# Deam0on/deepEMIA

Hardware: AMD Instinct MI355X
Metric: EM tiles/s (2048x2048, R101-FPN) (higher is better)
Workload: dtype f16x2

## Files before the change

deepemia_amd/_lib.py:

```python
from __future__ import annotations

import ctypes as C
import os
from pathlib import Path

_HERE = Path(__file__).resolve().parent
LIB_PATH = _HERE / "csrc" / ("libdeepemia_hip_dev.so" if os.environ.get("DEEPEMIA_DEV_LIB", "0") == "1" else "libdeepemia_hip.so")

F32, BF16, F32X3, BF16X2, F16X2, P32 = 0, 1, 2, 3, 4, 5
ACT_NONE, ACT_RELU, ACT_SIGMOID = 0, 1, 2
RES_NONE, RES_SAME, RES_UP2 = 0, 1, 2
MOP = {"fill": 1, "dilate": 2, "erode": 3, "drop_multi": 4, "flag_multi": 5, "gate": 6}


class HipExtensionMissing(RuntimeError):
    pass


class HipKernelError(RuntimeError):
    pass


class ConvDesc(C.Structure):
    _fields_ = [
        ("in_", C.c_void_p), ("w", C.c_void_p), ("scale", C.c_void_p), ("bias", C.c_void_p),
        ("residual", C.c_void_p), ("out", C.c_void_p),
        ("N", C.c_int32), ("H", C.c_int32), ("W", C.c_int32), ("Cin", C.c_int32),
        ("Ho", C.c_int32), ("Wo", C.c_int32), ("Cout", C.c_int32), ("CoutPad", C.c_int32),
        ("KH", C.c_int32), ("KW", C.c_int32), ("stride", C.c_int32), ("pad", C.c_int32),
        ("dtype", C.c_int32), ("out_dtype", C.c_int32), ("act", C.c_int32), ("res_mode", C.c_int32),
        ("out_ld", C.c_int32), ("tile_hint", C.c_int32),
        ("amax_in", C.c_void_p), ("amax_out", C.c_void_p),
    ]


class ConvP32Desc(C.Structure):
    _fields_ = [
        ("in_", C.c_void_p), ("in_meta", C.c_void_p), ("w", C.c_void_p), ("scale", C.c_void_p), ("bias", C.c_void_p),
        ("residual", C.c_void_p), ("res_meta", C.c_void_p), ("out", C.c_void_p), ("out_meta", C.c_void_p),
        ("wbound", C.c_float), ("bbound", C.c_float),
        ("N", C.c_int32), ("H", C.c_int32), ("W", C.c_int32), ("Cin", C.c_int32),
        ("Ho", C.c_int32), ("Wo", C.c_int32), ("Cout", C.c_int32), ("CoutPad", C.c_int32),
        ("KH", C.c_int32), ("KW", C.c_int32), ("stride", C.c_int32), ("pad", C.c_int32),
        ("act", C.c_int32), ("res_mode", C.c_int32), ("out_f32", C.c_int32), ("out_ld", C.c_int32), ("tile_hint", C.c_int32),
        ("head_w", C.c_void_p), ("head_b", C.c_void_p), ("head_out", C.c_void_p),
        ("head_n", C.c_int32), ("head_ld", C.c_int32), ("head_act", C.c_int32),
        ("groups", C.c_int32), ("group_rows", C.c_int32), ("row0", C.c_int32), ("single", C.c_int32),
    ]


class RpnDesc(C.Structure):
    _fields_ = [
        ("head", C.c_void_p * 5), ("H", C.c_int32 * 5), ("W", C.c_int32 * 5), ("stride", C.c_int32 * 5),
        ("cell_anchors", C.c_void_p), ("head_ld", C.c_int32), ("N", C.c_int32),
        ("img_h", C.c_int32), ("img_w", C.c_int32), ("pre_topk", C.c_int32), ("post_topk", C.c_int32),
        ("nms_thresh", C.c_float), ("out_boxes", C.c_void_p), ("out_scores", C.c_void_p),
        ("out_count", C.c_void_p), ("workspace", C.c_void_p),
    ]


class RoiAlignDesc(C.Structure):
    _fields_ = [
        ("feat", C.c_void_p * 4), ("H", C.c_int32 * 4), ("W", C.c_int32 * 4),
        ("N", C.c_int32), ("R", C.c_int32), ("C", C.c_int32), ("P", C.c_int32), ("dtype", C.c_int32),
        ("boxes", C.c_void_p), ("count", C.c_void_p), ("out", C.c_void_p),
        ("meta", C.c_void_p * 4), ("out_meta", C.c_void_p), ("groups", C.c_int32), ("single", C.c_int32),
        ("order", C.c_void_p),
    ]


class DetsDesc(C.Structure):
    _fields_ = [
        ("logits", C.c_void_p), ("ld", C.c_int32), ("props", C.c_void_p), ("prop_count", C.c_void_p),
        ("N", C.c_int32), ("R", C.c_int32), ("K", C.c_int32), ("img_h", C.c_int32), ("img_w", C.c_int32),
        ("score_thresh", C.c_float), ("nms_thresh", C.c_float), ("topk", C.c_int32),
        ("det_boxes", C.c_void_p), ("det_scores", C.c_void_p), ("det_classes", C.c_void_p),
        ("det_count", C.c_void_p),
    ]


class PasteDesc(C.Structure):
    _fields_ = [
        ("mask_prob", C.c_void_p), ("ld", C.c_int32), ("det_boxes", C.c_void_p), ("det_classes", C.c_void_p),
        ("det_count", C.c_void_p), ("N", C.c_int32), ("D", C.c_int32), ("img_h", C.c_int32), ("img_w", C.c_int32),
        ("out_h", C.c_int32), ("out_w", C.c_int32), ("out_boxes", C.c_void_p), ("valid", C.c_void_p),
        ("packed", C.c_void_p), ("out_bbox", C.c_void_p), ("prev_bbox", C.c_void_p),
    ]


EXPORTS = {
    "demia_abi_version": (C.c_int, []),
    "demia_conv_f16x2_kstep": (C.c_int, []),
    "demia_last_error": (C.c_char_p, []),
    "demia_build_arch": (C.c_char_p, []),
    "demia_build_flavor": (C.c_char_p, []),
    "demia_stream_create_cu_mask": (C.c_int, [C.c_void_p, C.c_int, C.c_void_p]),
    "demia_stream_destroy": (C.c_int, [C.c_void_p]),
    "demia_conv2d_nhwc": (C.c_int, [C.POINTER(ConvDesc), C.c_void_p]),
    "demia_conv2d_p32": (C.c_int, [C.POINTER(ConvP32Desc), C.c_void_p]),
    "demia_conv2d_p32_single": (C.c_int, [C.POINTER(ConvP32Desc), C.c_void_p]),
    "demia_resize_h_u8": (C.c_int, [C.c_void_p, C.c_void_p, C.c_int, C.c_int, C.c_int, C.c_int, C.c_void_p,
                                     C.c_void_p, C.c_void_p, C.c_int, C.c_void_p]),
    "demia_resize_v_norm": (C.c_int, [C.c_void_p, C.c_void_p, C.c_int, C.c_int, C.c_int, C.c_int, C.c_int, C.c_int,
                                       C.c_void_p, C.c_void_p, C.c_void_p, C.c_int, C.POINTER(C.c_float), C.c_int,
                                       C.c_void_p]),
    "demia_resize_linear_u8": (C.c_int, [C.c_void_p, C.c_void_p, C.c_int, C.c_int, C.c_int, C.c_int, C.c_int, C.c_void_p,
                                          C.c_void_p, C.c_void_p, C.c_void_p, C.c_void_p]),
    "demia_stem_conv": (C.c_int, [C.c_void_p, C.c_void_p, C.c_void_p, C.c_void_p, C.c_void_p, C.c_int, C.c_int,
                                   C.c_int, C.c_int, C.c_void_p]),
    "demia_stem_conv_mfma": (C.c_int, [C.c_void_p, C.c_void_p, C.c_void_p, C.c_void_p, C.c_void_p, C.c_int, C.c_int, C.c_int, C.c_float,
                                        C.c_void_p]),
    "demia_stem_pool_mfma": (C.c_int, [C.c_void_p, C.c_void_p, C.c_void_p, C.c_void_p, C.c_void_p, C.c_void_p, C.c_int, C.c_int, C.c_int,
                                        C.c_float, C.c_float, C.c_int, C.c_int, C.c_void_p]),
    "demia_maxpool3x3s2": (C.c_int, [C.c_void_p, C.c_void_p, C.c_int, C.c_int, C.c_int, C.c_int, C.c_int, C.c_void_p]),
    "demia_maxpool3x3s2_p32": (C.c_int, [C.c_void_p, C.c_void_p, C.c_void_p, C.c_float, C.c_int, C.c_int, C.c_int, C.c_int, C.c_int, C.c_int,
                                          C.c_void_p]),
    "demia_subsample2": (C.c_int, [C.c_void_p, C.c_void_p, C.c_int, C.c_int, C.c_int, C.c_int, C.c_int, C.c_void_p]),
    "demia_rpn_workspace_bytes": (C.c_int64, [C.c_int]),
    "demia_rpn_proposals": (C.c_int, [C.POINTER(RpnDesc), C.c_void_p]),
    "demia_roi_align": (C.c_int, [C.POINTER(RoiAlignDesc), C.c_void_p]),
    "demia_roi_order": (C.c_int, [C.c_void_p, C.c_void_p, C.c_int, C.c_int, C.c_void_p, C.c_void_p]),
    "demia_box_detections": (C.c_int, [C.POINTER(DetsDesc), C.c_void_p]),
    "demia_paste_masks": (C.c_int, [C.POINTER(PasteDesc), C.c_void_p]),
    "demia_unpack_masks": (C.c_int, [C.c_void_p, C.c_void_p, C.c_int64, C.c_int, C.c_int, C.c_void_p]),
    "demia_mask_area_bbox": (C.c_int, [C.c_void_p, C.c_void_p, C.c_void_p, C.c_void_p, C.c_int64, C.c_int, C.c_int, C.c_void_p]),
    "demia_mask_program": (C.c_int, [C.c_void_p, C.c_void_p, C.c_void_p, C.c_void_p, C.c_uint32, C.c_int64, C.c_int, C.c_int,
                                      C.c_void_p, C.c_void_p, C.c_void_p, C.c_void_p]),
    "demia_mask_program_wl": (C.c_int, [C.c_void_p, C.c_void_p, C.c_void_p, C.c_void_p, C.c_uint32, C.c_int64, C.c_int, C.c_int,
                                         C.c_void_p, C.c_void_p, C.c_void_p, C.c_void_p, C.c_void_p]),
    "demia_mask_overlap_prefix": (C.c_int, [C.c_void_p, C.c_void_p, C.c_void_p, C.c_int64, C.c_int, C.c_int, C.c_void_p]),
    "demia_mask_column_counts": (C.c_int, [C.c_void_p, C.c_void_p, C.c_void_p, C.c_int64, C.c_int, C.c_int, C.c_void_p, C.c_void_p]),
    "demia_mask_pair_intersections": (C.c_int, [C.c_void_p, C.c_void_p, C.c_void_p, C.c_void_p, C.c_void_p, C.c_void_p,
                                                 C.c_void_p, C.c_int64, C.c_int, C.c_int, C.c_void_p]),
    "demia_mask_pair_matrix": (C.c_int, [C.c_void_p, C.c_void_p, C.c_void_p, C.c_void_p, C.c_void_p, C.c_void_p, C.c_int64, C.c_int,
                                          C.c_int, C.c_int, C.c_void_p]),
    "demia_host_greedy_keep": (C.c_int, [C.c_void_p, C.c_int, C.c_void_p, C.c_void_p, C.c_void_p, C.c_void_p, C.c_int, C.c_double,
                                          C.c_void_p]),
    "demia_host_dedup_smart": (C.c_int, [C.c_void_p, C.c_int, C.c_void_p, C.c_void_p, C.c_void_p, C.c_void_p, C.c_void_p, C.c_void_p,
                                          C.c_void_p, C.c_int, C.c_double, C.c_void_p, C.c_void_p]),
    "demia_host_repr_rows": (C.c_int64, [C.c_void_p, C.c_int64, C.c_int, C.c_void_p, C.c_int64]),
    "demia_host_rle_text": (C.c_int64, [C.c_void_p, C.c_void_p, C.c_void_p, C.c_int64, C.c_int, C.c_void_p, C.c_int64, C.c_void_p]),
    "demia_mask_place_tiles": (C.c_int, [C.c_void_p, C.c_void_p, C.c_void_p, C.c_void_p, C.c_int64, C.c_int, C.c_int,
                                          C.c_int, C.c_int, C.c_int, C.c_int, C.c_void_p]),
    "demia_mask_crop_pack": (C.c_int, [C.c_void_p, C.c_void_p, C.c_void_p, C.c_int64, C.c_int, C.c_int, C.c_void_p, C.c_void_p]),
    "demia_mask_gather_regions": (C.c_int, [C.c_void_p, C.c_void_p, C.c_void_p, C.c_int64, C.c_int, C.c_int, C.c_void_p, C.c_void_p]),
    "demia_mask_gather_regions_pooled": (C.c_int, [C.c_void_p, C.c_void_p, C.c_void_p, C.c_int64, C.c_int, C.c_int, C.c_void_p, C.c_void_p,
                                                    C.c_int, C.c_void_p]),
    "demia_mask_crop_unpack": (C.c_int, [C.c_void_p, C.c_void_p, C.c_void_p, C.c_int64, C.c_int, C.c_int, C.c_void_p, C.c_void_p]),
    "demia_crop_place_tiles": (C.c_int, [C.c_void_p, C.c_void_p, C.c_void_p, C.c_int64, C.c_int, C.c_int, C.c_int, C.c_int, C.c_int, C.c_int,
                                          C.c_void_p, C.c_void_p, C.c_void_p, C.c_void_p, C.c_void_p, C.c_void_p]),
    "demia_crop_gather": (C.c_int, [C.c_void_p, C.c_void_p, C.c_void_p, C.c_void_p, C.c_void_p, C.c_int64, C.c_void_p, C.c_void_p]),
    "demia_crop_reroom": (C.c_int, [C.c_void_p, C.c_void_p, C.c_void_p, C.c_void_p, C.c_void_p, C.c_void_p, C.c_int64, C.c_int64, C.c_void_p,
                                     C.c_void_p]),
    "demia_crop_pair_matrix": (C.c_int, [C.c_void_p, C.c_void_p, C.c_void_p, C.c_void_p, C.c_void_p, C.c_void_p, C.c_void_p, C.c_void_p,
                                          C.c_int64, C.c_int, C.c_void_p]),
    "demia_crop_pair_intersections": (C.c_int, [C.c_void_p, C.c_void_p, C.c_void_p, C.c_void_p, C.c_void_p, C.c_void_p, C.c_void_p, C.c_void_p,
                                                 C.c_void_p, C.c_void_p, C.c_void_p, C.c_int64, C.c_void_p]),
    "demia_crop_unpack_pooled": (C.c_int, [C.c_void_p, C.c_void_p, C.c_void_p, C.c_void_p, C.c_int64, C.c_int64, C.c_int, C.c_int,
                                            C.c_void_p, C.c_void_p, C.c_int, C.c_void_p]),
    "demia_crop_gray_histogram": (C.c_int, [C.c_void_p, C.c_void_p, C.c_void_p, C.c_void_p, C.c_void_p, C.c_int, C.c_int64, C.c_int, C.c_int,
                                             C.c_void_p, C.c_void_p]),
    "demia_mask_gray_histogram": (C.c_int, [C.c_void_p, C.c_void_p, C.c_void_p, C.c_int, C.c_int64, C.c_int, C.c_int, C.c_void_p, C.c_void_p]),
    "demia_contour_work_ints": (C.c_int64, [C.c_int, C.c_int, C.c_int]),
    "demia_contour_work_floats": (C.c_int64, [C.c_int, C.c_int, C.c_int]),
    "demia_contour_work_doubles": (C.c_int64, [C.c_int, C.c_int, C.c_int]),
    "demia_mask_contours": (C.c_int, [C.c_void_p, C.c_void_p, C.c_void_p, C.c_int, C.c_int, C.c_int, C.c_int, C.c_int,
                                       C.c_void_p, C.c_void_p, C.c_void_p, C.c_void_p, C.c_void_p, C.c_void_p]),
    "demia_mask_contours_wl": (C.c_int, [C.c_void_p, C.c_void_p, C.c_void_p, C.c_int, C.c_int, C.c_int, C.c_int, C.c_int,
                                          C.c_void_p, C.c_void_p, C.c_void_p, C.c_void_p, C.c_void_p, C.c_void_p, C.c_void_p]),
    "demia_crop_contour_scratch": (C.c_int64, [C.c_void_p, C.c_int64, C.c_int, C.c_int, C.c_void_p]),
    "demia_crop_contours_wl": (C.c_int, [C.c_void_p, C.c_void_p, C.c_void_p, C.c_void_p, C.c_int, C.c_int, C.c_int, C.c_int, C.c_int,
                                          C.c_void_p, C.c_void_p, C.c_void_p, C.c_void_p, C.c_void_p, C.c_void_p, C.c_void_p, C.c_void_p,
                                          C.c_void_p]),
    "demia_contour_measure": (C.c_int, [C.c_void_p, C.c_void_p, C.c_void_p, C.c_void_p, C.c_void_p, C.c_int, C.c_int, C.c_int,
                                         C.c_void_p, C.c_void_p, C.c_void_p, C.c_double, C.c_void_p, C.c_int, C.c_void_p]),
    "demia_contour_shape_work_ints": (C.c_int64, [C.c_int, C.c_int, C.c_int]),
    "demia_contour_shape": (C.c_int, [C.c_void_p, C.c_void_p, C.c_void_p, C.c_void_p, C.c_void_p, C.c_int, C.c_int, C.c_int,
                                       C.c_void_p, C.c_double, C.c_void_p, C.c_int, C.c_void_p]),
    "demia_mask_inscribed": (C.c_int, [C.c_void_p, C.c_void_p, C.c_void_p, C.c_void_p, C.c_void_p, C.c_void_p, C.c_int, C.c_int, C.c_int,
                                        C.c_int, C.c_double, C.c_void_p, C.c_int, C.c_void_p]),
    "demia_crop_inscribed": (C.c_int, [C.c_void_p, C.c_void_p, C.c_void_p, C.c_void_p, C.c_void_p, C.c_void_p, C.c_void_p, C.c_int, C.c_int,
                                        C.c_int, C.c_int, C.c_double, C.c_void_p, C.c_int, C.c_void_p, C.c_void_p, C.c_void_p]),
    "demia_mask_skeleton": (C.c_int, [C.c_void_p, C.c_void_p, C.c_void_p, C.c_void_p, C.c_void_p, C.c_void_p, C.c_int, C.c_int, C.c_int,
                                       C.c_int, C.c_double, C.c_void_p, C.c_int, C.c_void_p, C.c_void_p, C.c_void_p]),
    "demia_crop_skeleton_scratch": (C.c_int64, [C.c_void_p, C.c_int64, C.c_int, C.c_int, C.c_void_p]),
    "demia_crop_skeleton": (C.c_int, [C.c_void_p, C.c_void_p, C.c_void_p, C.c_void_p, C.c_void_p, C.c_void_p, C.c_void_p, C.c_int, C.c_int,
                                       C.c_int, C.c_int, C.c_double, C.c_void_p, C.c_int, C.c_void_p, C.c_void_p, C.c_void_p, C.c_void_p,
                                       C.c_void_p, C.c_void_p]),
    "demia_mask_neighbours": (C.c_int, [C.c_void_p, C.c_void_p, C.c_void_p, C.c_int64, C.c_int, C.c_int, C.c_int64, C.c_void_p, C.c_void_p,
                                         C.c_void_p, C.c_void_p, C.c_void_p, C.c_void_p]),
    "demia_crop_neighbours": (C.c_int, [C.c_void_p, C.c_void_p, C.c_void_p, C.c_void_p, C.c_void_p, C.c_int64, C.c_int, C.c_int, C.c_int64,
                                         C.c_void_p, C.c_void_p, C.c_void_p, C.c_void_p, C.c_void_p, C.c_void_p]),
    "demia_poly_rasterize": (C.c_int, [C.c_void_p, C.c_void_p, C.c_void_p, C.c_void_p, C.c_void_p, C.c_void_p, C.c_void_p, C.c_void_p,
                                        C.c_int64, C.c_void_p, C.c_int64, C.c_int, C.c_int, C.c_void_p, C.c_void_p, C.c_void_p,
                                        C.c_void_p]),
    "demia_mask_cross_matrix": (C.c_int, [C.c_void_p, C.c_void_p, C.c_void_p, C.c_void_p, C.c_void_p, C.c_void_p, C.c_void_p, C.c_void_p,
                                           C.c_void_p, C.c_int64, C.c_int, C.c_int, C.c_int, C.c_void_p]),
    "demia_mask_rle_colmajor": (C.c_int, [C.c_void_p, C.c_void_p, C.c_void_p, C.c_void_p, C.c_void_p, C.c_int64, C.c_int, C.c_int,
                                           C.c_void_p]),
    "demia_crop_poly_rasterize": (C.c_int, [C.c_void_p, C.c_void_p, C.c_void_p, C.c_void_p, C.c_void_p, C.c_void_p, C.c_void_p, C.c_void_p,
                                             C.c_int64, C.c_void_p, C.c_int64, C.c_int, C.c_int, C.c_void_p, C.c_void_p, C.c_int64,
                                             C.c_void_p, C.c_void_p, C.c_void_p, C.c_void_p]),
    "demia_crop_cross_matrix": (C.c_int, [C.c_void_p, C.c_void_p, C.c_void_p, C.c_void_p, C.c_void_p, C.c_void_p, C.c_void_p, C.c_void_p,
                                           C.c_void_p, C.c_void_p, C.c_void_p, C.c_void_p, C.c_void_p, C.c_int64, C.c_int, C.c_void_p]),
    "demia_crop_rle_colmajor": (C.c_int, [C.c_void_p, C.c_void_p, C.c_void_p, C.c_void_p, C.c_void_p, C.c_void_p, C.c_void_p, C.c_int64,
                                           C.c_int, C.c_int, C.c_void_p]),
    "demia_host_coco_match": (C.c_int, [C.c_int64, C.c_void_p, C.c_void_p, C.c_void_p, C.c_void_p, C.c_void_p, C.c_void_p, C.c_void_p,
                                         C.c_void_p, C.c_void_p, C.c_void_p, C.c_int, C.c_void_p, C.c_int, C.c_int, C.c_void_p,
                                         C.c_void_p, C.c_void_p, C.c_void_p]),
    "demia_host_rle_string": (C.c_int64, [C.c_void_p, C.c_void_p, C.c_int64, C.c_void_p, C.c_int64, C.c_void_p]),
}

_lib = None


def load() -> C.CDLL:
    global _lib
    if _lib is not None:
        return _lib
    if not LIB_PATH.exists():
        raise HipExtensionMissing(
            f"{LIB_PATH} not found: build it with `python -c 'import __graft_entry__ as g; g.build()'` "
            f"(or `make -C {LIB_PATH.parent}`); there is no CPU fallback for the hot path."
        )
    try:
        lib = C.CDLL(str(LIB_PATH), mode=getattr(os, "RTLD_NOW", 2))
    except OSError as e:
        raise HipExtensionMissing(f"cannot load {LIB_PATH}: {e}") from e
    for name, (res, args) in EXPORTS.items():
        try:
            fn = getattr(lib, name)
        except AttributeError as e:
            raise HipExtensionMissing(f"{LIB_PATH} does not export {name}") from e
        fn.restype = res
        fn.argtypes = args
    _lib = lib
    return lib


def is_dev_build() -> bool:
    return load().demia_build_flavor() == b"dev"


def check(status: int, what: str) -> None:
    if status != 0:
        msg = load().demia_last_error().decode(errors="replace")
        raise HipKernelError(f"{what} failed with status {status}: {msg}")


def ptr(t) -> int:
    return 0 if t is None else int(t.data_ptr())


def cu_masked_stream(device, spec: str):
    import numpy as np
    import torch

    kind, m, k = spec.split(":")
    assert kind == "mod"
    m, k = int(m), int(k)
    bits = np.zeros(256, dtype=np.uint8)
    bits[(np.arange(256) % m) < k] = 1
    words = np.packbits(bits.reshape(8, 32), axis=1, bitorder="little").view(np.uint32).reshape(8).copy()
    handle = C.c_void_p()
    with torch.cuda.device(device):
        check(load().demia_stream_create_cu_mask(words.ctypes.data, 8, C.byref(handle)), "demia_stream_create_cu_mask")
    return torch.cuda.ExternalStream(handle.value, device=device), int(bits.sum())
```

deepemia_amd/csrc/conv_p32.hip:

```cpp
#include <utility>
#include "common.h"
#ifndef P32_ABLATE
#define P32_ABLATE 0
#endif

#ifndef P32_HEAD_DIRECT
#define P32_HEAD_DIRECT 1
#endif
#ifndef P32_SINGLE
#define P32_SINGLE 0
#endif
#ifndef P32_DEV_TILES
#define P32_DEV_TILES 0
#endif
#ifndef P32_ST_AUX
#define P32_ST_AUX 0
#endif
#ifndef P32_RES_AUX
#define P32_RES_AUX 0
#endif
#ifndef P32_A_NT
#define P32_A_NT 0
#endif
#ifndef P32_FRAG_PIPE
#define P32_FRAG_PIPE 0
#endif

namespace {

struct ConvQ {
    const void* in;
    const float* in_meta;
    const void* w;
    const float* scale;
    const float* bias;
    const void* res;
    const float* res_meta;
    void* out;
    float* out_meta;
    float wbound, bbound;
    int N, H, W, Cin, Ho, Wo, Cout, CoutPad, KH, KW, stride, pad;
    int act, res_mode, out_f32, out_ld;
    int M, HoWo, ntn, nwg, ksteps, taps;
    int kloop;
    unsigned in_bytes, w_bytes;
    unsigned out_bytes, res_bytes;
    const float* head_w;
    const float* head_b;
    float* head_out;
    int head_n, head_ld, head_act;
    int groups, group_rows, row0;
    int no_hk;
    int zero_low;
    int stagger_ticks;
    int resident;
};

typedef __attribute__((address_space(3))) void lds_void;

template <int OFF, int WAIT>
__device__ __forceinline__ void ds_read2_b128(f16x8& a, f16x8& b, unsigned addr_a, unsigned addr_b) {
    if constexpr (WAIT >= 0)
        asm volatile("ds_read_b128 %0, %2 offset:%4\n\tds_read_b128 %1, %3 offset:%4\n\ts_waitcnt lgkmcnt(%5)"
                     : "=&v"(a), "=&v"(b) : "v"(addr_a), "v"(addr_b), "n"(OFF), "n"(WAIT) : "memory");
    else
        asm volatile("ds_read_b128 %0, %2 offset:%4\n\tds_read_b128 %1, %3 offset:%4"
                     : "=&v"(a), "=&v"(b) : "v"(addr_a), "v"(addr_b), "n"(OFF) : "memory");
}

template <int... Is, class F>
__device__ __forceinline__ void static_for_impl(std::integer_sequence<int, Is...>, F&& f) { (f(std::integral_constant<int, Is>{}), ...); }
template <int N, class F>
__device__ __forceinline__ void static_for(F&& f) { static_for_impl(std::make_integer_sequence<int, N>{}, static_cast<F&&>(f)); }
typedef int i32x4 __attribute__((ext_vector_type(4)));

__device__ __forceinline__ void dma16(const i32x4 rsrc, unsigned lds_addr, unsigned voff, unsigned soff) {
    unsigned keep;
    asm volatile("s_mov_b32 %0, m0\n\ts_mov_b32 m0, %1\n\ts_nop 0\n\tbuffer_load_dwordx4 %2, %3, %4 offen lds\n\ts_mov_b32 m0, %0"
                 : "=&s"(keep) : "s"(lds_addr), "v"(voff), "s"(rsrc), "s"(soff) : "memory");
}
__device__ __forceinline__ void dma16_nt(const i32x4 rsrc, unsigned lds_addr, unsigned voff, unsigned soff) {
    unsigned keep;
    asm volatile("s_mov_b32 %0, m0\n\ts_mov_b32 m0, %1\n\ts_nop 0\n\tbuffer_load_dwordx4 %2, %3, %4 offen nt lds\n\ts_mov_b32 m0, %0"
                 : "=&s"(keep) : "s"(lds_addr), "v"(voff), "s"(rsrc), "s"(soff) : "memory");
}
__device__ __forceinline__ i32x4 make_rsrc(const void* base, unsigned bytes) {
    const unsigned long long a = reinterpret_cast<unsigned long long>(base);
    i32x4 r;
    r[0] = __builtin_amdgcn_readfirstlane((int)(unsigned)a);
    r[1] = __builtin_amdgcn_readfirstlane((int)((unsigned)(a >> 32) & 0xffffu));
    r[2] = __builtin_amdgcn_readfirstlane((int)bytes);
    r[3] = 0x00020000;
    return r;
}

__device__ __forceinline__ float apply_act_q(float v, int act) {
    if (act == DEMIA_ACT_RELU) return v > 0.f ? v : 0.f;
    if (act == DEMIA_ACT_SIGMOID) return 1.0f / (1.0f + expf(-v));
    return v;
}

__device__ __forceinline__ float plane_scale(float bound) {
    if (!(bound > 0.f) || !(bound < 3.0e38f)) return 1.f;
    int e = 14 - ilogbf(bound);
    e = e < -100 ? -100 : (e > 100 ? 100 : e);
    return ldexpf(1.f, e);
}

template <int TN, int EF>
__device__ __forceinline__ void write_acc32(const f32x16 (&row)[TN], float* e, int lane) {
#pragma unroll
    for (int j = 0; j < TN; ++j)
#pragma unroll
        for (int r = 0; r < 16; ++r)
            e[((r & 3) + 8 * (r >> 2) + 4 * (lane >> 5)) * EF + j * 32 + (lane & 31)] = row[j][r];
}
template <int TN, int EF>
__device__ __forceinline__ void write_acc16(const f32x4 (&r0)[2 * TN], const f32x4 (&r1)[2 * TN], float* e, int lane) {
#pragma unroll
    for (int j = 0; j < 2 * TN; ++j)
#pragma unroll
        for (int r = 0; r < 4; ++r) {
            e[(4 * (lane >> 4) + r) * EF + j * 16 + (lane & 15)] = r0[j][r];
            e[(16 + 4 * (lane >> 4) + r) * EF + j * 16 + (lane & 15)] = r1[j][r];
        }
}

__device__ __forceinline__ float uniform(float v) { return __int_as_float(__builtin_amdgcn_readfirstlane(__float_as_int(v))); }

struct GroupScales {
    int g0, b1, b2;
    float post0, post1, post2, resi0, resi1, resi2, sout0, sout1, sout2;
};

__device__ __forceinline__ void load_group_scale(const ConvQ& p, int gi, bool planes_out, float& post, float& resi, float& sout) {
    gi = min(gi, p.groups - 1);
    const float amax_in = p.in_meta[2 * gi], s_in = p.in_meta[2 * gi + 1];
    float amax_res = 0.f, s_res = 1.f;
    if (p.res_mode != DEMIA_RES_NONE) { amax_res = p.res_meta[2 * gi]; s_res = p.res_meta[2 * gi + 1]; }
    post = uniform(1.0f / s_in);
    resi = uniform(p.res_mode != DEMIA_RES_NONE ? 1.0f / s_res : 0.f);
    sout = uniform(planes_out ? plane_scale(amax_in * p.wbound + p.bbound + amax_res) : 1.f);
}

__device__ __forceinline__ GroupScales load_group_scales(const ConvQ& p, int m0, bool planes_out) {
    GroupScales gs;
    gs.g0 = (m0 + p.row0) / p.group_rows;
    gs.b1 = (gs.g0 + 1) * p.group_rows - p.row0;
    gs.b2 = gs.b1 + p.group_rows;
    load_group_scale(p, gs.g0, planes_out, gs.post0, gs.resi0, gs.sout0);
    load_group_scale(p, gs.g0 + 1, planes_out, gs.post1, gs.resi1, gs.sout1);
    load_group_scale(p, gs.g0 + 2, planes_out, gs.post2, gs.resi2, gs.sout2);
    return gs;
}

template <int WM, int WN, int TM, int TN, bool HEAD, typename WriteRow>
__device__ __forceinline__ void p32_epilogue(const ConvQ& p, const GroupScales& gs, char* smem, WriteRow&& write_tile_row, int wm, int wn, int m0, int n0) {
    constexpr int BN = WN * TN * 32;
    const int tid = threadIdx.x, lane = tid & 63;
    constexpr int EROW = BN * 4 + 16;
    constexpr int GPR = BN / 8, RSTEP = 512 / GPR, ITEMS = WM * 32 / RSTEP;
    static_assert(512 % GPR == 0 && (WM * 32) % RSTEP == 0, "epilogue split");
    constexpr int BM_ = WM * TM * 32;
    static_assert(!HEAD || BN == 256, "the fused head needs a 256-wide tile");
    const bool planes_out = !HEAD && !p.out_f32;
    const int g0 = __builtin_amdgcn_readfirstlane(gs.g0), b1 = __builtin_amdgcn_readfirstlane(gs.b1), b2 = __builtin_amdgcn_readfirstlane(gs.b2);
    const float post0 = uniform(gs.post0), post1 = uniform(gs.post1), post2 = uniform(gs.post2);
    const float resi0 = uniform(gs.resi0), resi1 = uniform(gs.resi1), resi2 = uniform(gs.resi2);
    const float sout0 = uniform(gs.sout0), sout1 = uniform(gs.sout1), sout2 = uniform(gs.sout2);
    if (planes_out && n0 == 0 && tid == 0) {
#pragma unroll
        for (int d = 0; d < 3; ++d) {
            const int first = d == 0 ? g0 * p.group_rows - p.row0 : (d == 1 ? b1 : b2);
            if (g0 + d < p.groups && first >= m0 && first < m0 + BM_ && first < p.M)
                p.out_meta[2 * (g0 + d) + 1] = d == 0 ? sout0 : (d == 1 ? sout1 : sout2);
        }
    }
    const int g = tid % GPR, r_first = tid / GPR;
    const int co = n0 + g * 8;
    float sc[8], bs[8];
#pragma unroll
    for (int q = 0; q < 8; ++q) {
        const bool ok = (co + q) < p.Cout;
        sc[q] = (p.scale && ok) ? p.scale[co + q] : 1.0f;
        bs[q] = (p.bias && ok) ? p.bias[co + q] : 0.0f;
    }
    float vmax3[3] = {0.f, 0.f, 0.f};
    constexpr int HMAX = 4;
    float hw[HMAX][8];
    constexpr bool head_on = HEAD;
    if (head_on) {
#pragma unroll
        for (int j = 0; j < HMAX; ++j)
#pragma unroll
            for (int q = 0; q < 8; ++q) hw[j][q] = j < p.head_n ? p.head_w[j * 256 + g * 8 + q] : 0.f;
    }
    const int tile_n_ = n0 / BN;
    const bool res_on = p.res_mode != DEMIA_RES_NONE, sigmoid_on = p.act == DEMIA_ACT_SIGMOID;
    const float act_lo = p.act == DEMIA_ACT_RELU ? 0.f : -INFINITY;
    const char* resb = reinterpret_cast<const char*>(p.res) + 128;
    char* outb = reinterpret_cast<char*>(p.out) + 128;
    const long cbytes = (long)p.Cout * 4;
    const int gofs = (co >> 5) * 128 + ((co & 31) >> 3) * 16;
    auto row_of = [&](int i, int k) { const int lr = r_first + k * RSTEP; return m0 + (lr >> 5) * (TM * 32) + i * 32 + (lr & 31); };
    auto res_pix = [&](int m) -> long {
        if (p.res_mode == DEMIA_RES_SAME) return m;
        const int n = m / p.HoWo;
        const int rem = m - n * p.HoWo;
        const int ho = rem / p.Wo, wo = rem - ho * p.Wo;
        const int Hr = (p.Ho + 1) >> 1, Wr = (p.Wo + 1) >> 1;
        return ((long)n * Hr + (ho >> 1)) * Wr + (wo >> 1);
    };
    f16x8 rh[ITEMS], rl[ITEMS];
    const bool has_res = p.res_mode != DEMIA_RES_NONE && co < p.Cout;
    auto load_res = [&](int i) {
#pragma unroll
        for (int k = 0; k < ITEMS; ++k) {
            const int m = row_of(i, k);
            if (has_res && m < p.M && !(P32_ABLATE & 32)) {
                const char* rp = resb + res_pix(m) * cbytes + gofs;
                rh[k] = *reinterpret_cast<const f16x8*>(rp);
                rl[k] = *reinterpret_cast<const f16x8*>(rp + 64);
            }
        }
    };
    load_res(0);
#pragma unroll
    for (int i = 0; i < TM; ++i) {
        if (i > 0) __syncthreads();
        write_tile_row(i, reinterpret_cast<float*>(smem) + (wm * 32) * (EROW / 4) + wn * TN * 32);
        __syncthreads();
        f16x8 ch[ITEMS], cl[ITEMS];
#pragma unroll
        for (int k = 0; k < ITEMS; ++k) { ch[k] = rh[k]; cl[k] = rl[k]; }
        if (i + 1 < TM) load_res(i + 1);
        if (co < p.Cout) {
#pragma unroll
            for (int k = 0; k < ITEMS; ++k) {
                const int lr = r_first + k * RSTEP;
                const int m = row_of(i, k);
                if (m >= p.M) continue;
                const float4 x0 = *reinterpret_cast<const float4*>(smem + lr * EROW + g * 32);
                const float4 x1 = *reinterpret_cast<const float4*>(smem + lr * EROW + g * 32 + 16);
                float v[8] = {x0.x, x0.y, x0.z, x0.w, x1.x, x1.y, x1.z, x1.w};
                const int gd = (m >= b1) + (m >= b2);
                const float post = gd == 0 ? post0 : (gd == 1 ? post1 : post2);
#pragma unroll
                for (int q = 0; q < 8; ++q) v[q] = (v[q] * post) * sc[q] + bs[q];
                if (res_on) {
                    const float res_inv = gd == 0 ? resi0 : (gd == 1 ? resi1 : resi2);
#pragma unroll
                    for (int q = 0; q < 8; ++q) v[q] += ((float)ch[k][q] + (float)cl[k][q]) * res_inv;
                }
#pragma unroll
                for (int q = 0; q < 8; ++q) v[q] = fmaxf(v[q], act_lo);
                if (sigmoid_on) {
#pragma unroll
                    for (int q = 0; q < 8; ++q) v[q] = 1.0f / (1.0f + expf(-v[q]));
                }
                if (head_on) {
                    float acc_h[HMAX];
#pragma unroll
                    for (int j = 0; j < HMAX; ++j) {
                        float a = 0.f;
#pragma unroll
                        for (int q = 0; q < 8; ++q) a = fmaf(v[q], hw[j][q], a);
#pragma unroll
                        for (int o = 16; o > 0; o >>= 1) a += __shfl_xor(a, o, 32);
                        acc_h[j] = a;
                    }
                    if (g == 0) {
                        float* o = p.head_out + ((long)m * p.ntn + tile_n_) * p.head_ld;
#pragma unroll
                        for (int j = 0; j < HMAX; ++j)
                            if (j < p.head_n) {
                                const float z = acc_h[j] + p.head_b[j];
                                o[j] = p.head_act == DEMIA_ACT_SIGMOID ? 1.0f / (1.0f + expf(-z)) : (p.head_act == DEMIA_ACT_RELU ? fmaxf(z, 0.f) : z);
                            }
                    }
                } else if (p.out_f32) {
                    float* o = reinterpret_cast<float*>(p.out) + (long)m * p.out_ld + co;
                    if (co + 8 <= p.Cout && (p.out_ld & 3) == 0) {
                        *reinterpret_cast<float4*>(o) = make_float4(v[0], v[1], v[2], v[3]);
                        *reinterpret_cast<float4*>(o + 4) = make_float4(v[4], v[5], v[6], v[7]);
                    } else {
#pragma unroll
                        for (int q = 0; q < 8; ++q)
                            if (co + q < p.Cout) o[q] = v[q];
                    }
                } else {
                    f16x8 h, l;
                    const float s_out = gd == 0 ? sout0 : (gd == 1 ? sout1 : sout2);
                    float vm = 0.f;
#pragma unroll
                    for (int q = 0; q < 8; ++q) {
                        vm = fmaxf(vm, fabsf(v[q]));
                        const float y = v[q] * s_out;
                        h[q] = (_Float16)y;
                        l[q] = (P32_SINGLE && p.zero_low) ? (_Float16)0.f : (_Float16)(y - (float)h[q]);
                    }
                    vmax3[0] = fmaxf(vmax3[0], gd == 0 ? vm : 0.f);
                    vmax3[1] = fmaxf(vmax3[1], gd == 1 ? vm : 0.f);
                    vmax3[2] = fmaxf(vmax3[2], gd == 2 ? vm : 0.f);
                    char* o = outb + (long)m * cbytes + gofs;
                    if (P32_ABLATE & 64) {
                        asm volatile("" :: "v"(h), "v"(l), "v"(o));
                    } else {
                        *reinterpret_cast<f16x8*>(o) = h;
                        *reinterpret_cast<f16x8*>(o + 64) = l;
                    }
                }
            }
        }
    }
    if (planes_out) {
#pragma unroll
        for (int d = 0; d < 3; ++d) {
            if (d > 0 && (d == 1 ? b1 : b2) >= m0 + BM_) break;
            if (g0 + d >= p.groups) break;
            float vmax = vmax3[d];
#pragma unroll
            for (int o = 32; o > 0; o >>= 1) vmax = fmaxf(vmax, __shfl_xor(vmax, o));
            float* slot = p.out_meta + 2 * (g0 + d);
            if (lane == 0 && vmax > *reinterpret_cast<volatile const float*>(slot))
                atomicMax(reinterpret_cast<unsigned int*>(slot), __float_as_uint(vmax));
        }
    }
}

struct NoHook { __device__ __forceinline__ void operator()() const {} };
template <int WM, int WN, int TM, int TN, typename WriteRow, typename Hook = NoHook>
__device__ __forceinline__ void p32_epilogue_planes(const ConvQ& p, const GroupScales& gs, char* smem, WriteRow&& write_tile_row, int wm, int wn,
                                                    int m0, int n0, bool leader = (threadIdx.x == 0), Hook&& hook = NoHook()) {
    constexpr int BM_ = WM * TM * 32;
    const int tid = threadIdx.x, lane = tid & 63;
    constexpr int LDW = TN * 32 + 4;
    constexpr int PPW = 8 / TN, RPI = 2 * PPW, ITEMS = 32 / RPI;
    static_assert(TN == 1 || TN == 2 || TN == 4, "TN");
    char* const wsm = smem + (tid >> 6) * (32 * LDW * 4);
    const int g0 = __builtin_amdgcn_readfirstlane(gs.g0), b1 = __builtin_amdgcn_readfirstlane(gs.b1), b2 = __builtin_amdgcn_readfirstlane(gs.b2);
    const float post0 = uniform(gs.post0), post1 = uniform(gs.post1), post2 = uniform(gs.post2);
    const float resi0 = uniform(gs.resi0), resi1 = uniform(gs.resi1), resi2 = uniform(gs.resi2);
    const float sout0 = uniform(gs.sout0), sout1 = uniform(gs.sout1), sout2 = uniform(gs.sout2);
    if (n0 == 0 && leader) {
#pragma unroll
        for (int d = 0; d < 3; ++d) {
            const int first = d == 0 ? g0 * p.group_rows - p.row0 : (d == 1 ? b1 : b2);
            if (g0 + d < p.groups && first >= m0 && first < m0 + BM_ && first < p.M)
                p.out_meta[2 * (g0 + d) + 1] = d == 0 ? sout0 : (d == 1 ? sout1 : sout2);
        }
    }
    const int cj = lane & 3, rs = (lane >> 2) & 1, lg = lane >> 3;
    const int line = lg % TN;
    const int r_first = (lg / TN) * 2 + rs;
    const int co = n0 + ((wn * TN + line) * 4 + cj) * 8;
    float sc[8], bs[8];
#pragma unroll
    for (int q = 0; q < 8; ++q) {
        sc[q] = p.scale ? p.scale[co + q] : 1.0f;
        bs[q] = p.bias ? p.bias[co + q] : 0.0f;
    }
    const bool sigmoid_on = p.act == DEMIA_ACT_SIGMOID;
    const float act_lo = p.act == DEMIA_ACT_RELU ? 0.f : -INFINITY;
    const bool res_on = p.res_mode != DEMIA_RES_NONE;
    const bool single = P32_SINGLE != 0 && p.zero_low != 0;
    const __amdgpu_buffer_rsrc_t rs_out = __builtin_amdgcn_make_buffer_rsrc(p.out, 0, (int)p.out_bytes, 0x00020000);
    const __amdgpu_buffer_rsrc_t rs_res = __builtin_amdgcn_make_buffer_rsrc(const_cast<void*>(res_on ? p.res : p.out), 0, res_on ? (int)p.res_bytes : 0, 0x00020000);
    const unsigned cbytes = (unsigned)p.Cout * 4u;
    const unsigned lofs = 128u + (unsigned)((co >> 5) * 128 + (lane & 7) * 16);
    auto row_of = [&](int i, int k) { return m0 + wm * (TM * 32) + i * 32 + r_first + k * RPI; };
    auto res_off = [&](int m) -> unsigned {
        if (p.res_mode != DEMIA_RES_UP2 || (P32_ABLATE & 256)) return (unsigned)m * cbytes + lofs;
        const int n = m / p.HoWo;
        const int rem = m - n * p.HoWo;
        const int ho = rem / p.Wo, wo = rem - ho * p.Wo;
        const int Hr = (p.Ho + 1) >> 1, Wr = (p.Wo + 1) >> 1;
        return (unsigned)((n * Hr + (ho >> 1)) * Wr + (wo >> 1)) * cbytes + lofs;
    };
    auto from_below = [&](u32x4 own, u32x4 theirs) -> u32x4 {
        u32x4 r;
#pragma unroll
        for (int c = 0; c < 4; ++c) r[c] = (unsigned)__builtin_amdgcn_update_dpp((int)own[c], (int)theirs[c], 0x114, 0xf, 0xa, false);
        return r;
    };
    auto from_above = [&](u32x4 own, u32x4 theirs) -> u32x4 {
        u32x4 r;
#pragma unroll
        for (int c = 0; c < 4; ++c) r[c] = (unsigned)__builtin_amdgcn_update_dpp((int)own[c], (int)theirs[c], 0x104, 0xf, 0x5, false);
        return r;
    };
    u32x4 rh[ITEMS], rl[ITEMS];
    auto load_res = [&](int i) {
#pragma unroll
        for (int k = 0; k < ITEMS; ++k) {
            const int mp = row_of(i, k) - rs;
            if (P32_ABLATE & 32) { rh[k] = u32x4{0, 0, 0, 0}; rl[k] = rh[k]; continue; }
            rh[k] = __builtin_amdgcn_raw_buffer_load_b128(rs_res, res_off(mp), 0, P32_RES_AUX);
            rl[k] = __builtin_amdgcn_raw_buffer_load_b128(rs_res, res_off(mp + 1), 0, P32_RES_AUX);
        }
    };
    float vmax0 = 0.f, vmax1 = 0.f, vmax2 = 0.f;
    if (P32_ABLATE & 512) return;
    load_res(0);
#pragma unroll
    for (int i = 0; i < TM; ++i) {
        asm volatile("" ::: "memory");
        __builtin_amdgcn_wave_barrier();
        write_tile_row(i, reinterpret_cast<float*>(wsm));
        asm volatile("" ::: "memory");
        __builtin_amdgcn_wave_barrier();
        f16x8 ch[ITEMS], cl[ITEMS];
#pragma unroll
        for (int k = 0; k < ITEMS; ++k) {
            ch[k] = __builtin_bit_cast(f16x8, from_below(rh[k], rl[k]));
            cl[k] = __builtin_bit_cast(f16x8, from_above(rl[k], rh[k]));
        }
        if (i + 1 < TM) load_res(i + 1);
#pragma unroll
        for (int k = 0; k < ITEMS; ++k) {
            const int lr = r_first + k * RPI;
            const int m = row_of(i, k);
            const float4 x0 = *reinterpret_cast<const float4*>(wsm + lr * (LDW * 4) + (line * 4 + cj) * 32);
            const float4 x1 = *reinterpret_cast<const float4*>(wsm + lr * (LDW * 4) + (line * 4 + cj) * 32 + 16);
            typedef float f32x2 __attribute__((ext_vector_type(2)));
            f32x2 v2[4] = {{x0.x, x0.y}, {x0.z, x0.w}, {x1.x, x1.y}, {x1.z, x1.w}};
            const int gd = (m >= b1) + (m >= b2);
            const float post = gd == 0 ? post0 : (gd == 1 ? post1 : post2);
            const float res_inv = gd == 0 ? resi0 : (gd == 1 ? resi1 : resi2);
            const float s_out = gd == 0 ? sout0 : (gd == 1 ? sout1 : sout2);
            float v[8];
#pragma unroll
            for (int q = 0; q < 4; ++q) {
                const f32x2 scq = {sc[2 * q], sc[2 * q + 1]}, bsq = {bs[2 * q], bs[2 * q + 1]};
                const f32x2 t = (v2[q] * post) * scq + bsq;
                v[2 * q] = t.x;
                v[2 * q + 1] = t.y;
            }
#pragma unroll
            for (int q = 0; q < 8; ++q) {
                v[q] = fmaf((float)cl[k][q], res_inv, fmaf((float)ch[k][q], res_inv, v[q]));
                v[q] = fmaxf(v[q], act_lo);
            }
            if (sigmoid_on && !(P32_ABLATE & 256)) {
#pragma unroll
                for (int q = 0; q < 8; ++q) v[q] = 1.0f / (1.0f + expf(-v[q]));
            }
            f16x8 h, l;
            float vm = 0.f;
#pragma unroll
            for (int q = 0; q < 8; q += 2) {
                vm = fmaxf(vm, fmaxf(fabsf(v[q]), fabsf(v[q + 1])));
                const f32x2 y = f32x2{v[q], v[q + 1]} * s_out;
                h[q] = (_Float16)y.x;
                h[q + 1] = (_Float16)y.y;
                l[q] = (_Float16)fmaf(-(float)h[q], 1.0f, y.x);
                l[q + 1] = (_Float16)fmaf(-(float)h[q + 1], 1.0f, y.y);
            }
            if (single) l = f16x8{0, 0, 0, 0, 0, 0, 0, 0};
            vm = m < p.M ? vm : 0.f;
            vmax0 = fmaxf(vmax0, gd == 0 ? vm : 0.f);
            vmax1 = fmaxf(vmax1, gd == 1 ? vm : 0.f);
            vmax2 = fmaxf(vmax2, gd == 2 ? vm : 0.f);
            const u32x4 hu = __builtin_bit_cast(u32x4, h), lu = __builtin_bit_cast(u32x4, l);
            const u32x4 d0 = from_below(hu, lu);
            const u32x4 d1 = from_above(lu, hu);
            const unsigned off = (unsigned)(m - rs) * cbytes + lofs;
            if (P32_ABLATE & 64) {
                asm volatile("" :: "v"(d0), "v"(d1), "v"(off));
            } else {
                __builtin_amdgcn_raw_buffer_store_b128(d0, rs_out, off, 0, P32_ST_AUX);
                __builtin_amdgcn_raw_buffer_store_b128(d1, rs_out, off + cbytes, 0, P32_ST_AUX);
            }
            hook();
        }
    }
#pragma unroll
    for (int d = 0; d < 3; ++d) {
        if (d > 0 && (d == 1 ? b1 : b2) >= m0 + BM_) break;
        if (g0 + d >= p.groups) break;
        float vmax = d == 0 ? vmax0 : (d == 1 ? vmax1 : vmax2);
#pragma unroll
        for (int o = 32; o > 0; o >>= 1) vmax = fmaxf(vmax, __shfl_xor(vmax, o));
        float* slot = p.out_meta + 2 * (g0 + d);
        if (lane == 0 && vmax > *reinterpret_cast<volatile const float*>(slot))
            atomicMax(reinterpret_cast<unsigned int*>(slot), __float_as_uint(vmax));
    }
}

template <int WM, int WN, int TM, int TN, int HN>
__device__ __forceinline__ void p32_epilogue_head_direct(const ConvQ& p, const GroupScales& gs, char* smem, const f32x4 (&acc16)[2 * TM][2 * TN],
                                                         int wm, int wn, int m0, int n0) {
    constexpr int BM = WM * TM * 32, BN = WN * TN * 32;
    static_assert(BN == 256, "the fused head needs a 256-wide tile");
    const int tid = threadIdx.x, lane = tid & 63, c16 = lane & 15, rq = lane >> 4;
    const int b1 = __builtin_amdgcn_readfirstlane(gs.b1), b2 = __builtin_amdgcn_readfirstlane(gs.b2);
    const float post0 = uniform(gs.post0), post1 = uniform(gs.post1), post2 = uniform(gs.post2);
    float sc[2 * TN], bs[2 * TN], hw[HN][2 * TN];
#pragma unroll
    for (int jn = 0; jn < 2 * TN; ++jn) {
        const int cl = wn * TN * 32 + jn * 16 + c16;
        sc[jn] = p.scale ? p.scale[n0 + cl] : 1.0f;
        bs[jn] = p.bias ? p.bias[n0 + cl] : 0.0f;
#pragma unroll
        for (int j = 0; j < HN; ++j) hw[j][jn] = j < p.head_n ? p.head_w[j * 256 + cl] : 0.f;
    }
    const float act_lo = p.act == DEMIA_ACT_RELU ? 0.f : -INFINITY;
    float* part = reinterpret_cast<float*>(smem);
#pragma unroll
    for (int i = 0; i < 2 * TM; ++i) {
#pragma unroll
        for (int r = 0; r < 4; ++r) {
            const int row = wm * TM * 32 + i * 16 + rq * 4 + r;
            const int m = m0 + row;
            const int gd = (m >= b1) + (m >= b2);
            const float post = gd == 0 ? post0 : (gd == 1 ? post1 : post2);
            float a[HN];
#pragma unroll
            for (int j = 0; j < HN; ++j) a[j] = 0.f;
#pragma unroll
            for (int jn = 0; jn < 2 * TN; ++jn) {
                const float v = fmaxf((acc16[i][jn][r] * post) * sc[jn] + bs[jn], act_lo);
#pragma unroll
                for (int j = 0; j < HN; ++j) a[j] = fmaf(v, hw[j][jn], a[j]);
            }
#pragma unroll
            for (int j = 0; j < HN; ++j) {
                a[j] += __int_as_float(__builtin_amdgcn_update_dpp(0, __float_as_int(a[j]), 0x128, 0xf, 0xf, false));
                a[j] += __int_as_float(__builtin_amdgcn_update_dpp(0, __float_as_int(a[j]), 0x124, 0xf, 0xf, false));
                a[j] += __int_as_float(__builtin_amdgcn_update_dpp(0, __float_as_int(a[j]), 0x122, 0xf, 0xf, false));
                a[j] += __int_as_float(__builtin_amdgcn_update_dpp(0, __float_as_int(a[j]), 0x121, 0xf, 0xf, false));
            }
            if (c16 == 0) {
#pragma unroll
                for (int j = 0; j < HN; ++j) part[((long)wn * BM + row) * HN + j] = a[j];
            }
        }
    }
    __syncthreads();
    const int tile_n_ = n0 / BN;
    for (int o = tid; o < BM * HN; o += WM * WN * 64) {
        const int row = o / HN, j = o - row * HN;
        const int m = m0 + row;
        if (m >= p.M || j >= p.head_n) continue;
        float z = 0.f;
#pragma unroll
        for (int w = 0; w < WN; ++w) z += part[((long)w * BM + row) * HN + j];
        z += p.head_b[j];
        p.head_out[((long)m * p.ntn + tile_n_) * p.head_ld + j] =
            p.head_act == DEMIA_ACT_SIGMOID ? 1.0f / (1.0f + expf(-z)) : (p.head_act == DEMIA_ACT_RELU ? fmaxf(z, 0.f) : z);
    }
}


constexpr int EPI_GENERIC = 0, EPI_PLANES = 1, EPI_HEAD = 2;

template <int WM, int WN, int TM, int TN, bool M16 = true, int EPI = EPI_PLANES, int NST = 2, bool HK = false>
__global__ __launch_bounds__(WM * WN * 64, WM * WN == 8 ? 2 : 1) void conv_p32_kernel(const ConvQ p) {
    static_assert(NST == 2 || NST == 3, "two or three LDS stages");
    static_assert(!HK || (P32_SINGLE && M16 && NST == 2), "HK is a variant of the single-plane 16x16x32 kernel");
    static_assert(WM * WN == 8 || (WM * WN == 4 && EPI == EPI_PLANES), "eight waves, or four (planes epilogue only)");
    constexpr int NW = WM * WN;
    constexpr int BM = WM * TM * 32, BN = WN * TN * 32;
    constexpr int STAGE = (BM + BN) * 128;
    constexpr int NIA = BM / 8, NIB = BN / 8;

    extern __shared__ __attribute__((aligned(16))) char smem[];
    const int tid = threadIdx.x, lane = tid & 63;
    const int wave = __builtin_amdgcn_readfirstlane(tid >> 6);
    const int wm = wave / WN, wn = wave % WN;
    const int swz = xcd_remap(blockIdx.x, p.nwg);
    const int tile_n = swz % p.ntn, tile_m = swz / p.ntn;
    const int m0 = tile_m * BM, n0 = tile_n * BN;
#if P32_DEV_TILES
    if (p.stagger_ticks > 0) {
        const int b = blockIdx.x;
        const bool late = p.resident > 256 ? (b >= p.resident / 2 && b < p.resident) : (b < p.resident && ((b >> 3) & 1));
        if (late) {
            const unsigned long long t0 = __builtin_amdgcn_s_memrealtime();
            while (__builtin_amdgcn_s_memrealtime() - t0 < (unsigned long long)p.stagger_ticks) __builtin_amdgcn_s_sleep(32);
        }
    }
#endif

    const i32x4 rsrc_a = make_rsrc(p.in, p.in_bytes), rsrc_b = make_rsrc(p.w, p.w_bytes);
    const unsigned lds0 = (unsigned)(__SIZE_TYPE__)((lds_void*)smem);

    constexpr int QA = (NIA + NW - 1) / NW, QB = NIB / NW;
    constexpr bool A_EVEN = NIA % NW == 0;
    static_assert(NIB % NW == 0, "tile width is a multiple of 64");
    unsigned a_off[QA], a_msk[QA], b_off[QB];
#pragma unroll
    for (int q = 0; q < QA; ++q) {
        const int row = (wave + NW * q) * 8 + (lane >> 3);
        const int csw = (lane & 7) ^ ((row >> 1) & 7);
        const int m = m0 + row;
        const bool vm = m < p.M && row < BM;
        const int mm = vm ? m : 0;
        const int n = mm / p.HoWo;
        const int rem = mm - n * p.HoWo;
        const int ho = rem / p.Wo, wo = rem - ho * p.Wo;
        const int hi0 = ho * p.stride - p.pad, wi0 = wo * p.stride - p.pad;
        const long pix = ((long)n * p.H + hi0) * p.W + wi0;
        a_off[q] = (unsigned)(128 + pix * (long)(p.Cin * 4) + (HK ? (csw >> 2) * 128 + (csw & 3) * 16 : csw * 16));
        unsigned mk = 0;
        for (int t = 0, th = 0, tw = 0; t < p.taps; ++t) {
            if (vm && (unsigned)(hi0 + th) < (unsigned)p.H && (unsigned)(wi0 + tw) < (unsigned)p.W) mk |= 1u << t;
            if (++tw == p.KW) { tw = 0; ++th; }
        }
        a_msk[q] = mk;
    }
#pragma unroll
    for (int q = 0; q < QB; ++q) {
        const int row = (wave + NW * q) * 8 + (lane >> 3);
        const int csw = (lane & 7) ^ ((row >> 1) & 7);
        const int co = n0 + row;
        b_off[q] = (unsigned)(((co >> 6) * p.ksteps) * 8192 + (co & 63) * 128 + (HK ? (csw >> 2) * (p.taps * 8192) + (csw & 3) * 16 : csw * 16));
    }
    int tap = 0, kw = 0, tstep = 0;
    unsigned sdelta = 0, srow = 0, sgrp = 0;
    const bool a_nt = P32_A_NT && p.taps == 1 && p.ntn == 1;
    auto issue = [&](int st, int tp, unsigned sd, unsigned bd) {
        const unsigned sbase = __builtin_amdgcn_readfirstlane(lds0 + st * STAGE + wave * 1024);
        const bool first = bd < 2 * 8192u;
#pragma unroll
        for (int q = 0; q < QA; ++q) {
            if ((P32_ABLATE & 1) && !first) break;
            if (!A_EVEN && q == QA - 1 && wave + NW * q >= NIA) break;
            const bool ok = (a_msk[q] >> tp) & 1u;
            const unsigned vo = ok ? a_off[q] + sd : (a_off[q] & 0x70u);
            if (P32_A_NT && a_nt) dma16_nt(rsrc_a, sbase + q * (NW * 1024), vo, 0u);
            else dma16(rsrc_a, sbase + q * (NW * 1024), vo, 0u);
        }
#pragma unroll
        for (int q = 0; q < QB; ++q) {
            if ((P32_ABLATE & 2) && !first) break;
            dma16(rsrc_b, sbase + BM * 128 + q * (NW * 1024), b_off[q], bd);
        }
    };
    const unsigned pixb = (unsigned)(p.Cin * 4), rowb = (unsigned)(p.W * p.Cin * 4);
#define P32_ADVANCE()                                                                   \
    do {                                                                                \
        ++tstep;                                                                        \
        if (++tap == p.taps) { tap = 0; kw = 0; srow = 0; sgrp += HK ? 256u : 128u; sdelta = sgrp; if (HK) tstep += p.taps; } \
        else if (++kw == p.KW) { kw = 0; srow += rowb; sdelta = srow + sgrp; }          \
        else sdelta += pixb;                                                            \
    } while (0)

    const int fsw = (lane >> 1) & 7, hh = lane >> 5;
    int fa[4], fb[4];
#pragma unroll
    for (int c = 0; c < 4; ++c) {
        const int ch = (((c >> 1) * 4 + (c & 1) * 2 + hh) ^ fsw) * 16;
        fa[c] = (wm * TM * 32 + (lane & 31)) * 128 + ch;
        fb[c] = BM * 128 + (wn * TN * 32 + (lane & 31)) * 128 + ch;
    }

    f32x16 acc[M16 ? 1 : TM][M16 ? 1 : TN];
    f32x4 acc16[M16 ? 2 * TM : 1][M16 ? 2 * TN : 1];
#pragma unroll
    for (int i = 0; i < (M16 ? 1 : TM); ++i)
#pragma unroll
        for (int j = 0; j < (M16 ? 1 : TN); ++j)
#pragma unroll
            for (int r = 0; r < 16; ++r) acc[i][j][r] = 0.f;
#pragma unroll
    for (int i = 0; i < (M16 ? 2 * TM : 1); ++i)
#pragma unroll
        for (int j = 0; j < (M16 ? 2 * TN : 1); ++j)
#pragma unroll
            for (int r = 0; r < 4; ++r) acc16[i][j][r] = 0.f;
    int fa16[2], fb16[2];
#pragma unroll
    for (int pl = 0; pl < 2; ++pl) {
        const int ch = ((pl * 4 + (lane >> 4)) ^ (((lane & 15) >> 1) & 7)) * 16;
        fa16[pl] = (wm * TM * 32 + (lane & 15)) * 128 + ch;
        fb16[pl] = BM * 128 + (wn * TN * 32 + (lane & 15)) * 128 + ch;
    }

    constexpr bool BARRIER_IN_COMPUTE = (P32_FRAG_PIPE == 2) && M16 && NST == 2;
    auto compute1 = [&](int st) {
        const char* sb = smem + st * STAGE;
        if constexpr (M16) {
            f16x8 bh[2 * TN];
#pragma unroll
            for (int j = 0; j < 2 * TN; ++j) bh[j] = *reinterpret_cast<const f16x8*>(sb + fb16[0] + j * 2048);
#pragma unroll
            for (int i = 0; i < 2 * TM; ++i) {
                const f16x8 ah = *reinterpret_cast<const f16x8*>(sb + fa16[0] + i * 2048);
#pragma unroll
                for (int j = 0; j < 2 * TN; ++j) acc16[i][j] = __builtin_amdgcn_mfma_f32_16x16x32_f16(ah, bh[j], acc16[i][j], 0, 0, 0);
            }
        } else {
#pragma unroll
            for (int kk = 0; kk < 2; ++kk) {
                f16x8 bh[TN];
#pragma unroll
                for (int j = 0; j < TN; ++j) bh[j] = *reinterpret_cast<const f16x8*>(sb + fb[kk] + j * 4096);
#pragma unroll
                for (int i = 0; i < TM; ++i) {
                    const f16x8 ah = *reinterpret_cast<const f16x8*>(sb + fa[kk] + i * 4096);
#pragma unroll
                    for (int j = 0; j < TN; ++j) acc[i][j] = __builtin_amdgcn_mfma_f32_32x32x16_f16(ah, bh[j], acc[i][j], 0, 0, 0);
                }
            }
        }
        if (BARRIER_IN_COMPUTE) asm volatile("s_waitcnt vmcnt(0) lgkmcnt(0)\n\ts_barrier" ::: "memory");
    };
    auto compute_hk = [&](int st) {
        const char* sb = smem + st * STAGE;
        f16x8 b0[2 * TN], b1[2 * TN];
#pragma unroll
        for (int j = 0; j < 2 * TN; ++j) {
            b0[j] = *reinterpret_cast<const f16x8*>(sb + fb16[0] + j * 2048);
            b1[j] = *reinterpret_cast<const f16x8*>(sb + fb16[1] + j * 2048);
        }
#pragma unroll
        for (int i = 0; i < 2 * TM; ++i) {
            const f16x8 a0 = *reinterpret_cast<const f16x8*>(sb + fa16[0] + i * 2048);
            const f16x8 a1 = *reinterpret_cast<const f16x8*>(sb + fa16[1] + i * 2048);
#pragma unroll
            for (int j = 0; j < 2 * TN; ++j) {
                f32x4 c = acc16[i][j];
                c = __builtin_amdgcn_mfma_f32_16x16x32_f16(a0, b0[j], c, 0, 0, 0);
                c = __builtin_amdgcn_mfma_f32_16x16x32_f16(a1, b1[j], c, 0, 0, 0);
                acc16[i][j] = c;
            }
        }
    };
    auto compute = [&](int st) {
        if constexpr (HK) { compute_hk(st); return; }
        if constexpr (P32_SINGLE != 0) { compute1(st); return; }
        const char* sb = smem + st * STAGE;
        if constexpr (M16) {
            f16x8 bh[2 * TN], bl[2 * TN];
            f16x8 fake;
#pragma unroll
            for (int q = 0; q < 8; ++q) fake[q] = (_Float16)(float)(lane + q);
#if P32_FRAG_PIPE != 2
#pragma unroll
            for (int j = 0; j < 2 * TN; ++j) {
                bh[j] = (P32_ABLATE & 1024) ? fake : *reinterpret_cast<const f16x8*>(sb + fb16[0] + j * 2048);
                bl[j] = (P32_ABLATE & 1024) ? fake : *reinterpret_cast<const f16x8*>(sb + fb16[1] + j * 2048);
            }
#endif
#if P32_FRAG_PIPE == 2
            const unsigned la0 = (unsigned)(__SIZE_TYPE__)((lds_void*)(smem)) + st * STAGE + fa16[0];
            const unsigned la1 = la0 - fa16[0] + fa16[1];
            const unsigned lb0 = la0 - fa16[0] + fb16[0], lb1 = la0 - fa16[0] + fb16[1];
            f16x8 ahp[2], alp[2];
            ds_read2_b128<0, -1>(ahp[0], alp[0], la0, la1);
            static_for<2 * TN>([&](auto jc) {
                constexpr int j = decltype(jc)::value;
                ds_read2_b128<j * 2048, -1>(bh[j], bl[j], lb0, lb1);
            });
            static_for<2 * TM>([&](auto ic) {
                constexpr int i = decltype(ic)::value;
                const f16x8 ah = ahp[i & 1], al = alp[i & 1];
                if constexpr (i == 0) {
                    ds_read2_b128<2048, -1>(ahp[1], alp[1], la0, la1);
                    static_for<2 * TN>([&](auto jc) {
                        constexpr int j = decltype(jc)::value;
                        asm volatile("s_waitcnt lgkmcnt(%0)" ::"n"(2 * (2 * TN - 1 - j) + 2) : "memory");
                        __builtin_amdgcn_sched_barrier(0);
                        f32x4 c = acc16[0][j];
                        c = __builtin_amdgcn_mfma_f32_16x16x32_f16(ah, bl[j], c, 0, 0, 0);
                        c = __builtin_amdgcn_mfma_f32_16x16x32_f16(al, bh[j], c, 0, 0, 0);
                        c = __builtin_amdgcn_mfma_f32_16x16x32_f16(ah, bh[j], c, 0, 0, 0);
                        acc16[0][j] = c;
                        __builtin_amdgcn_sched_barrier(0);
                    });
                } else {
                    if constexpr (i + 1 < 2 * TM) {
                        ds_read2_b128<(i + 1) * 2048, 2>(ahp[(i + 1) & 1], alp[(i + 1) & 1], la0, la1);
                    } else if constexpr (BARRIER_IN_COMPUTE) {
                        asm volatile("s_waitcnt vmcnt(0) lgkmcnt(0)\n\ts_barrier" ::: "memory");
                    } else {
                        asm volatile("s_waitcnt lgkmcnt(0)" ::: "memory");
                    }
                    __builtin_amdgcn_sched_barrier(0);
#pragma unroll
                    for (int j = 0; j < 2 * TN; ++j) {
                        f32x4 c = acc16[i][j];
                        c = __builtin_amdgcn_mfma_f32_16x16x32_f16(ah, bl[j], c, 0, 0, 0);
                        c = __builtin_amdgcn_mfma_f32_16x16x32_f16(al, bh[j], c, 0, 0, 0);
                        c = __builtin_amdgcn_mfma_f32_16x16x32_f16(ah, bh[j], c, 0, 0, 0);
                        acc16[i][j] = c;
                    }
                    __builtin_amdgcn_sched_barrier(0);
                }
            });
            return;
#elif P32_FRAG_PIPE
            f16x8 ahp[2], alp[2];
            ahp[0] = *reinterpret_cast<const f16x8*>(sb + fa16[0]);
            alp[0] = *reinterpret_cast<const f16x8*>(sb + fa16[1]);
#pragma unroll
            for (int i = 0; i < 2 * TM; ++i) {
                if (i + 1 < 2 * TM) {
                    ahp[(i + 1) & 1] = *reinterpret_cast<const f16x8*>(sb + fa16[0] + (i + 1) * 2048);
                    alp[(i + 1) & 1] = *reinterpret_cast<const f16x8*>(sb + fa16[1] + (i + 1) * 2048);
                }
                const f16x8 ah = ahp[i & 1], al = alp[i & 1];
#pragma unroll
                for (int j = 0; j < 2 * TN; ++j) {
                    f32x4 c = acc16[i][j];
                    c = __builtin_amdgcn_mfma_f32_16x16x32_f16(ah, bl[j], c, 0, 0, 0);
                    c = __builtin_amdgcn_mfma_f32_16x16x32_f16(al, bh[j], c, 0, 0, 0);
                    c = __builtin_amdgcn_mfma_f32_16x16x32_f16(ah, bh[j], c, 0, 0, 0);
                    acc16[i][j] = c;
                }
                if (i + 1 < 2 * TM) __builtin_amdgcn_sched_group_barrier(0x100, 2, 0);
                __builtin_amdgcn_sched_group_barrier(0x008, 6 * TN, 0);
            }
            return;
#else
#pragma unroll
            for (int i = 0; i < 2 * TM; ++i) {
                const f16x8 ah = (P32_ABLATE & 1024) ? fake : *reinterpret_cast<const f16x8*>(sb + fa16[0] + i * 2048);
                const f16x8 al = (P32_ABLATE & 1024) ? fake : *reinterpret_cast<const f16x8*>(sb + fa16[1] + i * 2048);
#pragma unroll
                for (int j = 0; j < 2 * TN; ++j) {
                    f32x4 c = acc16[i][j];
                    if (P32_ABLATE & 4) {
                        asm volatile("" :: "v"(ah), "v"(al), "v"(bh[j]), "v"(bl[j]));
                        continue;
                    }
                    c = __builtin_amdgcn_mfma_f32_16x16x32_f16(ah, bl[j], c, 0, 0, 0);
                    c = __builtin_amdgcn_mfma_f32_16x16x32_f16(al, bh[j], c, 0, 0, 0);
                    c = __builtin_amdgcn_mfma_f32_16x16x32_f16(ah, bh[j], c, 0, 0, 0);
                    acc16[i][j] = c;
                }
            }
            return;
#endif
        }
#pragma unroll
        for (int kk = 0; kk < 2; ++kk) {
            f16x8 bh[TN], bl[TN];
#pragma unroll
            for (int j = 0; j < TN; ++j) {
                bh[j] = *reinterpret_cast<const f16x8*>(sb + fb[kk] + j * 4096);
                bl[j] = *reinterpret_cast<const f16x8*>(sb + fb[2 + kk] + j * 4096);
            }
#pragma unroll
            for (int i = 0; i < TM; ++i) {
                const f16x8 ah = *reinterpret_cast<const f16x8*>(sb + fa[kk] + i * 4096);
                const f16x8 al = *reinterpret_cast<const f16x8*>(sb + fa[2 + kk] + i * 4096);
#pragma unroll
                for (int j = 0; j < TN; ++j) {
                    f32x16 c = acc[i][j];
                    if (P32_ABLATE & 4) {
                        asm volatile("" :: "v"(ah), "v"(al), "v"(bh[j]), "v"(bl[j]));
                        continue;
                    }
                    c = __builtin_amdgcn_mfma_f32_32x32x16_f16(ah, bl[j], c, 0, 0, 0);
                    c = __builtin_amdgcn_mfma_f32_32x32x16_f16(al, bh[j], c, 0, 0, 0);
                    c = __builtin_amdgcn_mfma_f32_32x32x16_f16(ah, bh[j], c, 0, 0, 0);
                    acc[i][j] = c;
                }
            }
        }
    };

    constexpr int N_LAST = QB + QA, N_LAST_SHORT = QB + QA - 1;
    const bool short_wave = !A_EVEN && wave + NW * (QA - 1) >= NIA;
    auto wait_all_but_last_issue = [&]() {
        if (short_wave) asm volatile("s_waitcnt vmcnt(%0)" ::"n"(N_LAST_SHORT) : "memory");
        else asm volatile("s_waitcnt vmcnt(%0)" ::"n"(N_LAST) : "memory");
    };
    issue(0, tap, sdelta, 0u);
    P32_ADVANCE();
    bool two_ahead = false;
    if (NST == 3 && p.kloop > 1 && !(P32_ABLATE & 128)) {
        issue(1, tap, sdelta, (unsigned)tstep * 8192u);
        P32_ADVANCE();
        two_ahead = true;
    }
    constexpr bool HEAD = EPI == EPI_HEAD;
    const GroupScales gs = load_group_scales(p, m0, !HEAD && !p.out_f32);
    if (two_ahead) wait_all_but_last_issue();
    else asm volatile("s_waitcnt vmcnt(0)" ::: "memory");
    __builtin_amdgcn_s_barrier();
    int st = 0;
    for (int t = 0; t < ((P32_ABLATE & 128) ? 1 : p.kloop); ++t) {
        const int st_issue = NST == 2 ? (st ^ 1) : (st == 0 ? 2 : st - 1);
        const bool more = t + NST - 1 < p.kloop;
        if (more) {
            issue(st_issue, tap, sdelta, (unsigned)tstep * 8192u);
            P32_ADVANCE();
        }
        compute(st);
        if (NST == 3 && more) {
            wait_all_but_last_issue();
            asm volatile("s_waitcnt lgkmcnt(0)\n\ts_barrier" ::: "memory");
        } else if (!BARRIER_IN_COMPUTE) {
            asm volatile("s_waitcnt vmcnt(0) lgkmcnt(0)\n\ts_barrier" ::: "memory");
        }
        st = NST == 2 ? (st ^ 1) : (st == 2 ? 0 : st + 1);
    }
#undef P32_ADVANCE

    if constexpr ((P32_ABLATE & 2048) != 0 && M16) {
#pragma unroll
        for (int i = 0; i < 2 * TM; ++i)
#pragma unroll
            for (int j = 0; j < 2 * TN; ++j) asm volatile("" :: "v"(acc16[i][j]));
        return;
    }
    if constexpr (EPI == EPI_PLANES) {
        if constexpr (M16) {
            p32_epilogue_planes<WM, WN, TM, TN>(p, gs, smem, [&](int i, float* e) { write_acc16<TN, TN * 32 + 4>(acc16[2 * i], acc16[2 * i + 1], e, lane); }, wm, wn, m0, n0);
        } else {
            p32_epilogue_planes<WM, WN, TM, TN>(p, gs, smem, [&](int i, float* e) { write_acc32<TN, TN * 32 + 4>(acc[i], e, lane); }, wm, wn, m0, n0);
        }
    } else if constexpr (M16 && HEAD && P32_HEAD_DIRECT) {
        if (p.act != DEMIA_ACT_SIGMOID && p.head_n <= 2)
            p32_epilogue_head_direct<WM, WN, TM, TN, 2>(p, gs, smem, acc16, wm, wn, m0, n0);
        else
            p32_epilogue<WM, WN, TM, TN, HEAD>(p, gs, smem, [&](int i, float* e) { write_acc16<TN, BN + 4>(acc16[2 * i], acc16[2 * i + 1], e, lane); }, wm, wn, m0, n0);
    } else if constexpr (M16) {
        p32_epilogue<WM, WN, TM, TN, HEAD>(p, gs, smem, [&](int i, float* e) { write_acc16<TN, BN + 4>(acc16[2 * i], acc16[2 * i + 1], e, lane); }, wm, wn, m0, n0);
    } else {
        p32_epilogue<WM, WN, TM, TN, HEAD>(p, gs, smem, [&](int i, float* e) { write_acc32<TN, BN + 4>(acc[i], e, lane); }, wm, wn, m0, n0);
    }
}

#if P32_DEV_TILES
#include "conv_p32_dev.inc"
#endif

template <int WM, int WN, int TM, int TN, bool M16 = true, int EPI = EPI_PLANES, int NST = 2, bool HK = false>
int launch_q_(ConvQ p, hipStream_t st) {
    constexpr int BM = WM * TM * 32, BN = WN * TN * 32;
    constexpr int stages = NST * (BM + BN) * 128, image = EPI == EPI_PLANES ? WM * WN * 32 * (TN * 128 + 16) : WM * 32 * (BN * 4 + 16);
    static_assert(stages <= 160 * 1024, "LDS");
    constexpr int smem = stages > image ? stages : image;
    p.ntn = p.CoutPad / BN;
    p.nwg = p.ntn * cdiv(p.M, BM);
    p.resident = 256 * (160 * 1024 / smem >= 2 ? 2 : 1);
    p.kloop = HK ? p.ksteps / 2 : p.ksteps;
    auto k = conv_p32_kernel<WM, WN, TM, TN, M16, EPI, NST, HK>;
    static bool attr_done = false;
    if (!attr_done) {
        (void)hipFuncSetAttribute(reinterpret_cast<const void*>(k), hipFuncAttributeMaxDynamicSharedMemorySize, smem);
        attr_done = true;
    }
    hipLaunchKernelGGL(k, dim3(p.nwg), dim3(WM * WN * 64), smem, st, p);
    DEMIA_CHECK_LAUNCH("conv_p32_kernel");
    return DEMIA_OK;
}
template <int WM, int WN, int TM, int TN, bool M16 = true, int EPI = EPI_PLANES, int NST = 2>
int launch_q(ConvQ p, hipStream_t st) {
#if P32_SINGLE
    if constexpr (M16 && NST == 2) {
        if (p.Cin % 64 == 0 && !p.no_hk) return launch_q_<WM, WN, TM, TN, M16, EPI, NST, true>(p, st);
    }
#endif
    return launch_q_<WM, WN, TM, TN, M16, EPI, NST, false>(p, st);
}

struct TileCfg { int id, bm, bn; };
constexpr TileCfg kTiles[] = {{1, 256, 256}, {2, 128, 256}, {4, 192, 256}, {12, 160, 256}, {13, 224, 256}, {6, 256, 128}, {7, 128, 128}, {9, 256, 64}, {11, 128, 64}};

inline double predict_us(const TileCfg& c, long M, int cout_pad, int ksteps, bool residual) {
    const long tiles = (long)cdiv(M, c.bm) * (cout_pad / c.bn);
    const int smem = 2 * (c.bm + c.bn) * 128;
    const int occ = 160 * 1024 / smem >= 2 ? 2 : 1;
    const double area = (double)c.bm * c.bn / 65536.0;
    const double step = 2.0 * area * (1.0 + 0.2 * (1.0 - area));
    const double edge = 6.0 + 6.0 * area * (residual ? 1.5 : 1.0);
    if (occ == 1) return (double)((tiles + 255) / 256) * (ksteps * step + edge);
    return (double)((tiles + 511) / 512) * (2.0 * ksteps * step + 2.0 * 0.5 * edge);
}

inline int choose_tile(long M, int cout_pad, int ksteps, bool residual, bool need256 = false) {
#if P32_SINGLE
    if (cout_pad % 256 == 0 && (long)cdiv(M, 256) * (cout_pad / 256) >= 512) return 1;
#endif
    int best = 0;
    double best_t = 1e30;
    for (const TileCfg& c : kTiles) {
        if (cout_pad % c.bn || (need256 && c.bn != 256)) continue;
        const double t = predict_us(c, M, cout_pad, ksteps, residual);
        if (t < best_t) { best_t = t; best = c.id; }
    }
    return best;
}

}

#if P32_SINGLE
extern "C" int demia_conv2d_p32_single(const demia_conv_p32_desc* d, void* stream) {
#else
extern "C" int demia_conv2d_p32_single(const demia_conv_p32_desc* d, void* stream);
extern "C" int demia_conv2d_p32(const demia_conv_p32_desc* d, void* stream) {
    if (d && d->single) return demia_conv2d_p32_single(d, stream);
#endif
    DEMIA_REQUIRE(d && d->in && d->in_meta && d->w && (d->out || d->head_n > 0), "null pointer");
    DEMIA_REQUIRE(d->out_f32 || d->out_meta || d->head_n > 0, "P32 output needs out_meta");
    DEMIA_REQUIRE(d->Cin > 0 && d->Cin % 32 == 0, "Cin must be a multiple of 32");
    DEMIA_REQUIRE(d->CoutPad >= d->Cout && d->CoutPad % 64 == 0, "CoutPad must be a multiple of 64");
    DEMIA_REQUIRE(d->out_f32 || d->Cout % 32 == 0, "P32 output needs Cout % 32 == 0");
    DEMIA_REQUIRE(d->KH > 0 && d->KW > 0 && d->KH * d->KW <= 32 && d->stride > 0 && d->pad >= 0, "kernel geometry");
    DEMIA_REQUIRE(d->Ho == (d->H + 2 * d->pad - d->KH) / d->stride + 1, "Ho");
    DEMIA_REQUIRE(d->Wo == (d->W + 2 * d->pad - d->KW) / d->stride + 1, "Wo");
    DEMIA_REQUIRE(d->res_mode == DEMIA_RES_NONE || (d->residual && d->res_meta), "residual pointer");
    DEMIA_REQUIRE((long)d->N * d->Ho * d->Wo < (1L << 31), "M overflow");
    const long in_bytes = 128 + (long)d->N * d->H * d->W * d->Cin * 4;
    DEMIA_REQUIRE(in_bytes < (1L << 32), "input planes must stay below 4 GiB");
    const long w_bytes = (long)d->CoutPad * d->KH * d->KW * d->Cin * 4;
    DEMIA_REQUIRE(w_bytes < (1L << 31), "weight planes must stay below 2 GiB");
    ConvQ p;
    p.in = d->in; p.in_meta = d->in_meta; p.w = d->w; p.scale = d->scale; p.bias = d->bias;
    p.res = d->residual; p.res_meta = d->res_meta; p.out = d->out; p.out_meta = d->out_meta;
    p.wbound = d->wbound; p.bbound = d->bbound;
    p.N = d->N; p.H = d->H; p.W = d->W; p.Cin = d->Cin; p.Ho = d->Ho; p.Wo = d->Wo; p.Cout = d->Cout; p.CoutPad = d->CoutPad;
    p.KH = d->KH; p.KW = d->KW; p.stride = d->stride; p.pad = d->pad;
    p.act = d->act; p.res_mode = d->res_mode; p.out_f32 = d->out_f32;
    p.out_ld = d->out_ld > 0 ? d->out_ld : d->Cout;
    DEMIA_REQUIRE(p.out_ld >= d->Cout, "out_ld");
    p.M = d->N * d->Ho * d->Wo;
    p.HoWo = d->Ho * d->Wo;
    p.taps = d->KH * d->KW;
    p.ksteps = p.taps * (d->Cin / 32);
    p.in_bytes = (unsigned)in_bytes; p.w_bytes = (unsigned)w_bytes;
    p.ntn = p.nwg = 0;
    p.zero_low = d->single == 2;
    {
        static const char* env = getenv("DEMIA_P32_NO_HK");
        p.no_hk = (env && env[0] == '1') ? 1 : 0;
    }
    p.kloop = 0;
    p.resident = 256;
    p.groups = d->groups > 1 ? d->groups : 1;
    p.group_rows = p.groups > 1 ? d->group_rows : (1 << 29);
    p.row0 = p.groups > 1 ? d->row0 : 0;
    DEMIA_REQUIRE(p.groups == 1 || (d->group_rows >= 128 && d->row0 >= 0 && ((long)p.M + d->row0 + d->group_rows - 1) / d->group_rows <= p.groups),
                  "scale groups: group_rows >= 128 and the rows of this call must fall inside `groups` groups");
    p.head_w = d->head_w; p.head_b = d->head_b; p.head_out = d->head_out; p.head_n = d->head_n; p.head_ld = d->head_ld; p.head_act = d->head_act;
    if (d->head_n > 0) {
        DEMIA_REQUIRE(d->head_n <= 4 && d->head_w && d->head_b && d->head_out && d->head_ld >= d->head_n, "fused head: at most 4 rows, pointers, head_ld");
        DEMIA_REQUIRE(d->CoutPad % 256 == 0 && d->Cout == d->CoutPad && !d->out_f32, "fused head needs Cout % 256 == 0 and a planes layer");
    }
    p.stagger_ticks = 0;
#if P32_DEV_TILES
    {
        static const char* env = getenv("DEMIA_P32_STAGGER_US");
        p.stagger_ticks = env ? atoi(env) * 100 : 0;
    }
#endif
    if (p.M == 0) return DEMIA_OK;
    hipStream_t st = reinterpret_cast<hipStream_t>(stream);
    int tile = d->tile_hint ? d->tile_hint : choose_tile(p.M, d->CoutPad, p.ksteps, d->res_mode != DEMIA_RES_NONE, d->head_n > 0);
    const bool n256 = d->CoutPad % 256 == 0, n128 = d->CoutPad % 128 == 0;
    if (d->head_n > 0) {
        switch (tile) {
            case 1: return launch_q<2, 4, 4, 2, true, EPI_HEAD>(p, st);
            case 2: return launch_q<2, 4, 2, 2, true, EPI_HEAD>(p, st);
            default: return launch_q<1, 8, 6, 1, true, EPI_HEAD>(p, st);
        }
    }
    const int tile_bn = (tile == 9 || tile == 10 || tile == 11 || tile == 49) ? 64 : ((tile >= 6 && tile <= 8) || tile == 26 ? 128 : 256);
    const long out_bytes = 128 + (long)p.M * d->Cout * 4;
    long res_bytes = 0;
    if (d->res_mode == DEMIA_RES_SAME) res_bytes = out_bytes;
    if (d->res_mode == DEMIA_RES_UP2) res_bytes = 128 + (long)d->N * ((d->Ho + 1) / 2) * ((d->Wo + 1) / 2) * d->Cout * 4;
    const bool planes = !d->out_f32 && d->Cout % tile_bn == 0 && out_bytes < (1L << 32) - 512 && res_bytes < (1L << 32) - 512 &&
                        (long)(p.M + 256) * d->Cout * 4 + 256 < (1L << 32);
    p.out_bytes = (unsigned)out_bytes; p.res_bytes = (unsigned)res_bytes;
#if !P32_SINGLE && P32_DEV_TILES
    if (tile == 60) {
        DEMIA_REQUIRE(!d->out_f32 && n128 && d->Cout % 128 == 0 && d->KH == 1 && d->KW == 1 && d->stride == 1 && d->pad == 0 &&
                      d->res_mode != DEMIA_RES_UP2 && out_bytes < (1L << 32) - 512 && res_bytes < (1L << 32) - 512 &&
                      (long)(p.M + 256) * d->Cout * 4 + 256 < (1L << 32),
                      "tile 60 (ping-pong) takes 1x1 stride-1 planes layers with Cout % 128 == 0, no nearest-2x residual, buffers below 4 GiB");
        return launch_pp1x1(p, st);
    }
#endif
    if (!planes) {
        if (tile != 7 && tile != 9 && tile != 10 && tile != 11 && tile != 21 && tile != 22 && tile != 26) tile = n128 ? 7 : 11;
        switch (tile) {
            case 7: DEMIA_REQUIRE(n128, "tile needs CoutPad % 128 == 0"); return launch_q<4, 2, 1, 2, true, EPI_GENERIC>(p, st);
            case 9: return launch_q<8, 1, 1, 2, true, EPI_GENERIC>(p, st);
            case 10: return launch_q<4, 2, 2, 1, true, EPI_GENERIC>(p, st);
            case 11: return launch_q<4, 2, 1, 1, true, EPI_GENERIC>(p, st);
            default: break;
        }
    }
    switch (tile) {
        case 1: DEMIA_REQUIRE(n256, "tile needs CoutPad % 256 == 0"); return launch_q<2, 4, 4, 2>(p, st);
        case 2: DEMIA_REQUIRE(n256, "tile needs CoutPad % 256 == 0"); return launch_q<2, 4, 2, 2>(p, st);
        case 4: DEMIA_REQUIRE(n256, "tile needs CoutPad % 256 == 0"); return launch_q<1, 8, 6, 1>(p, st);
        case 6: DEMIA_REQUIRE(n128, "tile needs CoutPad % 128 == 0"); return launch_q<4, 2, 2, 2>(p, st);
        case 7: DEMIA_REQUIRE(n128, "tile needs CoutPad % 128 == 0"); return launch_q<4, 2, 1, 2>(p, st);
        case 9: return launch_q<8, 1, 1, 2>(p, st);
        case 11: return launch_q<4, 2, 1, 1>(p, st);
        case 12: DEMIA_REQUIRE(n256, "tile needs CoutPad % 256 == 0"); return launch_q<1, 8, 5, 1>(p, st);
        case 13: DEMIA_REQUIRE(n256, "tile needs CoutPad % 256 == 0"); return launch_q<1, 8, 7, 1>(p, st);
#if P32_DEV_TILES
        case 3: DEMIA_REQUIRE(n256, "tile needs CoutPad % 256 == 0"); return launch_q<1, 8, 8, 1>(p, st);
        case 5: DEMIA_REQUIRE(n256, "tile needs CoutPad % 256 == 0"); return launch_q<1, 8, 4, 1>(p, st);
        case 8: DEMIA_REQUIRE(n128, "tile needs CoutPad % 128 == 0"); return launch_q<2, 4, 2, 1>(p, st);
        case 10: return launch_q<4, 2, 2, 1>(p, st);
        case 14: DEMIA_REQUIRE(n256, "tile needs CoutPad % 256 == 0"); return launch_q<2, 4, 3, 2>(p, st);
        case 42: DEMIA_REQUIRE(n256, "tile needs CoutPad % 256 == 0"); return launch_q<2, 4, 2, 2, true, EPI_PLANES, 3>(p, st);
        case 52: DEMIA_REQUIRE(n256, "tile needs CoutPad % 256 == 0"); return launch_q<1, 8, 5, 1, true, EPI_PLANES, 3>(p, st);
        case 49: return launch_q<8, 1, 1, 2, true, EPI_PLANES, 3>(p, st);
        case 31: DEMIA_REQUIRE(n256, "tile needs CoutPad % 256 == 0"); return launch_q<2, 4, 4, 2, false>(p, st);
        case 34: DEMIA_REQUIRE(n256, "tile needs CoutPad % 256 == 0"); return launch_q<1, 8, 6, 1, false>(p, st);
        case 21: DEMIA_REQUIRE(n256, "tile needs CoutPad % 256 == 0"); return launch_pp<4, 2>(p, st);
        case 22: DEMIA_REQUIRE(n256, "tile needs CoutPad % 256 == 0"); return launch_pp<2, 2>(p, st);
        case 26: DEMIA_REQUIRE(n128, "tile needs CoutPad % 128 == 0"); return launch_pp<4, 1>(p, st);
#endif
        default: DEMIA_REQUIRE(false, "tile_hint");
    }
    return DEMIA_EINVAL;
}
```

deepemia_amd/engine.py:

```python
from __future__ import annotations

import os

import ctypes as C
import math
from dataclasses import dataclass
from typing import Dict, List, Optional, Sequence, Tuple

import numpy as np
import torch

from . import _lib, p32
from ._lib import ACT_NONE, ACT_RELU, ACT_SIGMOID, BF16, BF16X2, F16X2, F32, F32X3, RES_NONE, RES_SAME, RES_UP2

RES_BLOCKS = {50: (3, 4, 6, 3), 101: (3, 4, 23, 3)}
PIXEL_MEAN = (103.530, 116.280, 123.675)
ANCHOR_SIZES = (32, 64, 128, 256, 512)
ANCHOR_RATIOS = (0.5, 1.0, 2.0)
STRIDES = (4, 8, 16, 32, 64)
DEFAULT_SINGLE_STAGES = ()
MASK_HEAD_STAGES = ("mask_fcn", "deconv")
STAGES = ("res2", "res3", "res4", "res5", "fpn_lateral", "fpn_output", "rpn_conv", "rpn_pred", "fc1", "fc2", "box_pred", "mask_fcn", "deconv")
BN_EPS = 1e-5
PRE_NMS_TOPK = 1000
POST_NMS_TOPK = 1000
RPN_NMS_THRESH = 0.7
DET_NMS_THRESH = 0.5
DETS_PER_IMAGE = 100
MAX_DETS_PER_IMAGE = 1000

EXPECTED_IGNORED_PREFIXES = ("proposal_generator.anchor_generator.", "pixel_mean", "pixel_std")


def check_dets_per_image(value) -> int:
    if isinstance(value, bool) or not isinstance(value, (int, np.integer)) or not 1 <= int(value) <= MAX_DETS_PER_IMAGE:
        raise ValueError(f"dets_per_image = {value!r}: an integer in 1..{MAX_DETS_PER_IMAGE} (the default, Detectron2's "
                         f"TEST.DETECTIONS_PER_IMAGE, is {DETS_PER_IMAGE})")
    return int(value)


def resize_shape(h: int, w: int, short: int = 800, max_size: int = 1333) -> Tuple[int, int]:
    scale = short * 1.0 / min(h, w)
    if h < w:
        newh, neww = short, scale * w
    else:
        newh, neww = scale * h, short
    if max(newh, neww) > max_size:
        s = max_size * 1.0 / max(newh, neww)
        newh, neww = newh * s, neww * s
    return int(newh + 0.5), int(neww + 0.5)


def pil_bilinear_tables(in_size: int, out_size: int):
    if in_size == out_size:
        return (np.arange(out_size, dtype=np.int32), np.ones(out_size, dtype=np.int32),
                np.full((out_size, 1), 1 << 22, dtype=np.int32))
    scale = filterscale = in_size / out_size
    if filterscale < 1.0:
        filterscale = 1.0
    support = 1.0 * filterscale
    ksize = int(math.ceil(support)) * 2 + 1
    xx = np.arange(out_size, dtype=np.float64)
    center = (xx + 0.5) * scale
    xmin = np.maximum((center - support + 0.5).astype(np.int64), 0)
    xmax = np.minimum((center + support + 0.5).astype(np.int64), in_size)
    xsize = xmax - xmin
    j = np.arange(ksize, dtype=np.float64)[None, :]
    arg = (j + xmin[:, None] - center[:, None] + 0.5) * (1.0 / filterscale)
    wgt = np.where(np.abs(arg) < 1.0, 1.0 - np.abs(arg), 0.0)
    wgt = np.where(j < xsize[:, None], wgt, 0.0)
    ww = np.zeros(out_size, dtype=np.float64)
    for c in range(ksize):
        ww = ww + wgt[:, c]
    kk = np.where(ww[:, None] != 0.0, wgt / np.where(ww == 0.0, 1.0, ww)[:, None], wgt)
    ik = np.where(kk < 0, np.trunc(-0.5 + kk * (1 << 22)), np.trunc(0.5 + kk * (1 << 22))).astype(np.int32)
    return xmin.astype(np.int32), xsize.astype(np.int32), np.ascontiguousarray(ik)


def cv_linear_tables(in_size: int, out_size: int, vertical: bool = False):
    inv_scale = float(out_size) / float(in_size)
    scale = 1.0 / inv_scale
    d = np.arange(out_size, dtype=np.float64)
    f = ((d + 0.5) * scale - 0.5).astype(np.float32)
    s = np.floor(f).astype(np.int64)
    f = (f - s.astype(np.float32)).astype(np.float32)
    if vertical:
        s0 = np.clip(s, 0, in_size - 1)
        s1 = np.clip(s + 1, 0, in_size - 1)
    else:
        neg = s < 0
        f[neg] = 0.0
        s[neg] = 0
        hi = s >= in_size - 1
        f[hi] = 0.0
        s[hi] = in_size - 1
        s0, s1 = s, np.minimum(s + 1, in_size - 1)
    ofs = np.stack([s0, s1], axis=1).astype(np.int32)
    c = np.stack([np.float32(1.0) - f, f], axis=1).astype(np.float32) * np.float32(2048.0)
    coef = np.clip(np.rint(c), -32768, 32767).astype(np.int16)
    return np.ascontiguousarray(ofs), np.ascontiguousarray(coef)


def split3_bf16(w: torch.Tensor) -> torch.Tensor:
    w = w.to(torch.float32)
    h = w.to(torch.bfloat16)
    r1 = w - h.to(torch.float32)
    m = r1.to(torch.bfloat16)
    l = (r1 - m.to(torch.float32)).to(torch.bfloat16)
    return torch.stack([h, m, l], dim=0)


def tile_weight_planes(w3: torch.Tensor, bk: int = 32) -> torch.Tensor:
    npl, cout_pad = int(w3.shape[0]), int(w3.shape[1])
    k = w3[0, 0].numel()
    assert cout_pad % 64 == 0 and k % bk == 0, (cout_pad, k, bk)
    return w3.reshape(npl, cout_pad // 64, 64, k // bk, bk).permute(1, 3, 0, 2, 4).contiguous()


def tile_weight_planes_p32(planes: torch.Tensor) -> torch.Tensor:
    _, cout_pad, kh, kw, cin = (int(d) for d in planes.shape)
    assert cout_pad % 64 == 0 and cin % 32 == 0, (cout_pad, cin)
    t = planes.reshape(2, cout_pad // 64, 64, kh * kw, cin // 32, 32)
    return t.permute(1, 4, 3, 2, 0, 5).contiguous()


def split2_f16_scaled(w: torch.Tensor) -> Tuple[torch.Tensor, torch.Tensor]:
    w = w.to(torch.float32)
    amax = w.abs().flatten(1).amax(dim=1)
    _, ex = torch.frexp(amax)
    sw = torch.ldexp(torch.ones_like(amax), 15 - ex)
    ws = w * sw.view(-1, *([1] * (w.dim() - 1)))
    h = ws.to(torch.float16)
    l = (ws - h.to(torch.float32)).to(torch.float16)
    return torch.stack([h, l], dim=0), sw


def stem_weight_planes(w: torch.Tensor) -> Tuple[torch.Tensor, torch.Tensor]:
    w = w.to(torch.float32)
    cout = w.shape[0]
    k = torch.zeros((cout, 7, 8, 4), dtype=torch.float32)
    k[:, :, :7, :3] = w.permute(0, 2, 3, 1)
    planes, sw = split2_f16_scaled(k.reshape(cout, 7 * 32))
    planes = planes.reshape(2, cout, 7, 32).permute(0, 2, 1, 3).contiguous()
    return planes, sw


def cell_anchor_table() -> np.ndarray:
    out = np.zeros((5, 3, 4), dtype=np.float32)
    for l, size in enumerate(ANCHOR_SIZES):
        area = size ** 2.0
        for a, r in enumerate(ANCHOR_RATIOS):
            w = math.sqrt(area / r)
            h = r * w
            out[l, a] = (-w / 2.0, -h / 2.0, w / 2.0, h / 2.0)
    return out


@dataclass
class ConvLayer:
    w: torch.Tensor
    scale: Optional[torch.Tensor]
    bias: Optional[torch.Tensor]
    cin: int
    cout: int
    cout_pad: int
    kh: int
    kw: int
    stride: int
    pad: int
    w3: Optional[torch.Tensor] = None
    scale3: Optional[torch.Tensor] = None
    wbound: float = 0.0
    bbound: float = 0.0
    single: int = 0


@dataclass
class RawDetections:
    boxes: torch.Tensor
    scores: torch.Tensor
    classes: torch.Tensor
    valid: torch.Tensor
    count: torch.Tensor
    packed: torch.Tensor
    height: int
    width: int
    bbox: Optional[torch.Tensor] = None


class MaskRCNNEngine:
    def __init__(self, state_dict: Dict[str, torch.Tensor], depth: int, num_classes: int, score_thresh: float,
                 device: str = "cuda:0", precision: str = "f16x2", min_size_test: int = 800, max_size_test: int = 1333,
                 single_stages: Optional[Sequence[str]] = None, dets_per_image: int = DETS_PER_IMAGE):
        if depth not in RES_BLOCKS:
            raise ValueError(f"unsupported ResNet depth {depth}")
        self.dets_per_image = check_dets_per_image(dets_per_image)
        if not torch.cuda.is_available():
            raise _lib.HipExtensionMissing("no HIP device visible: the deepEMIA hot path has no CPU fallback")
        self.lib = _lib.load()
        self.depth = depth
        self.K = int(num_classes)
        self.score_thresh = float(score_thresh)
        per_row = min(self.K, int(1.0 / self.score_thresh)) if self.score_thresh > 0 else self.K
        if self.score_thresh <= 0 or POST_NMS_TOPK * per_row > 4096:
            raise ValueError(f"{self.K} classes at score threshold {self.score_thresh}: up to {POST_NMS_TOPK} x {per_row} candidates per "
                             f"image exceed the 4096 the detection kernel sorts -- raise --threshold above {1.0 / (4096 // POST_NMS_TOPK + 1):.2f} "
                             f"or use at most {4096 // POST_NMS_TOPK} classes")
        self.device = torch.device(device)
        self.precision = precision
        self.min_size_test, self.max_size_test = int(min_size_test), int(max_size_test)
        if self.min_size_test < 32 or self.max_size_test < self.min_size_test:
            raise ValueError(f"min_size_test / max_size_test = {min_size_test} / {max_size_test}")
        if precision not in ("f32", "f32x3", "f16x2", "f16", "f16x2r", "bf16x2", "bf16"):
            raise ValueError("precision must be 'f16x2' (default: f32-sized error on the fp16 pipe, activations kept as two "
                             "pre-scaled fp16 planes in HBM, LDS-DMA fed kernel), 'f16x2r' (the same arithmetic with f32 "
                             "activations split in the K loop: round 1's kernel), 'f32' (exact-f32 MFMA), 'f32x3' (f32 on the "
                             "bf16 pipe, 3-way split), 'bf16x2' (16-bit operands on the bf16 pipe), 'bf16', or 'f16' (flagged NON-parity: "
                             "the f16x2 path with single-plane fp16 operands, one MFMA per product -- the reference's autocast "
                             "arithmetic, inference.py:1390-1395)")
        if precision not in ("f16x2", "f16", "f32") and not _lib.is_dev_build():
            raise ValueError(f"precision '{precision}' needs the dev build of the library (make -C deepemia_amd/csrc DEV=1, then "
                             f"DEEPEMIA_DEV_LIB=1): the product library computes f16x2 (default), f16 and exact f32 only")
        self.p32 = precision in ("f16x2", "f16")
        self.single_plane = precision == "f16"
        if single_stages is None:
            env = os.environ.get("DEEPEMIA_SINGLE_STAGES")
            single_stages = () if precision != "f16x2" else (DEFAULT_SINGLE_STAGES if env is None else tuple(t for t in env.split(",") if t))
        unknown = set(single_stages) - set(STAGES)
        if unknown or (single_stages and precision != "f16x2"):
            raise ValueError(f"single_stages {sorted(unknown)}: choose from {STAGES}, with precision 'f16x2'")
        self.single_stages = frozenset(single_stages)
        self._amax_buf: Optional[torch.Tensor] = None
        self._amax_i = 0
        self._meta_pool: Optional[torch.Tensor] = None
        self._meta_pools: Dict[tuple, torch.Tensor] = {}
        self._groups = 1
        self._meta_i = 0
        self._graphs: Dict[tuple, dict] = {}
        self._arena: Dict[tuple, list] = {}
        self._arena_key: Optional[tuple] = None
        self._arena_i = 0
        self._paste_static = None
        self.stem_mode = os.environ.get("DEEPEMIA_STEM", "fused") if self.p32 else "valu"
        self.stem_on_mfma = self.stem_mode in ("fused", "mfma")
        self.max_cached_shapes = max(1, int(os.environ.get("DEEPEMIA_MAX_CACHED_SHAPES", "3")))
        self._shape_lru: List[tuple] = []
        self.evictions = 0
        self.dt = BF16 if precision == "bf16" else F32
        self.tdt = torch.bfloat16 if precision == "bf16" else torch.float32
        self._tables: Dict[Tuple[int, int], dict] = {}
        self._cell = cell_anchor_table()
        self.roi_order = os.environ.get("DEEPEMIA_ROI_ORDER", "0") == "1"
        self.conv_events = None
        self.unmatched_keys: List[str] = []
        self._used = set()
        self._pack(state_dict)

    def _get(self, sd, key):
        if key not in sd:
            raise KeyError(f"checkpoint is missing '{key}' (expected Detectron2 0.6 Mask R-CNN R{self.depth}-FPN layout)")
        self._used.add(key)
        return sd[key].detach().to(torch.float32).cpu()

    def _conv(self, sd, prefix, stride=1, pad=0, norm=False, bias=False, weight=None, bias_t=None, stage: str = "") -> ConvLayer:
        w = self._get(sd, prefix + ".weight") if weight is None else weight
        cout, cin, kh, kw = w.shape
        cout_pad = (cout + 63) // 64 * 64 if self.p32 else (cout + 31) // 32 * 32
        wp = torch.zeros((cout_pad, kh, kw, cin), dtype=torch.float32)
        wp[:cout] = w.permute(0, 2, 3, 1)
        scale = b = None
        if norm:
            g = self._get(sd, prefix + ".norm.weight")
            beta = self._get(sd, prefix + ".norm.bias")
            rm = self._get(sd, prefix + ".norm.running_mean")
            rv = self._get(sd, prefix + ".norm.running_var")
            scale = g * (rv + BN_EPS).rsqrt()
            b = beta - rm * scale
        elif bias:
            b = self._get(sd, prefix + ".bias") if bias_t is None else bias_t
        dev = self.device
        if self.p32:
            if cin % 32:
                raise ValueError(f"{prefix or 'layer'}: Cin = {cin} is not a multiple of 32")
            planes, sw = split2_f16_scaled(wp.to(dev))
            if self.single_plane:
                planes[1].zero_()
            base = torch.ones(cout, dtype=torch.float32) if scale is None else scale
            l1 = w.abs().flatten(1).sum(1)
            return ConvLayer(None, None if scale is None else scale.to(dev).contiguous(), None if b is None else b.to(dev).contiguous(),
                             cin, cout, cout_pad, kh, kw, stride, pad, tile_weight_planes_p32(planes),
                             (base.to(dev) / sw[:cout]).contiguous(), float((base.abs() * l1).max()),
                             0.0 if b is None else float(b.abs().max()), 2 if self.single_plane else int(stage in self.single_stages))
        w3 = None
        if self.precision in ("f32x3", "bf16x2") and cout_pad % 64 == 0 and cin % 32 == 0:
            w3 = split3_bf16(wp.to(dev))
            w3 = tile_weight_planes(w3 if self.precision == "f32x3" else w3[:2])
        scale3 = None
        f16_bk = int(self.lib.demia_conv_f16x2_kstep())
        if self.precision == "f16x2r" and cout_pad % 64 == 0 and cin % f16_bk == 0:
            planes, sw = split2_f16_scaled(wp.to(dev))
            w3 = tile_weight_planes(planes, f16_bk)
            base = torch.ones(cout, dtype=torch.float32, device=dev) if scale is None else scale.to(dev)
            scale3 = (base / sw[:cout]).contiguous()
        return ConvLayer(wp.to(dev, self.tdt).contiguous(),
                         None if scale is None else scale.to(dev).contiguous(),
                         None if b is None else b.to(dev).contiguous(), cin, cout, cout_pad, kh, kw, stride, pad, w3, scale3)

    def _pack(self, sd):
        bu = "backbone.bottom_up."
        w = self._get(sd, bu + "stem.conv1.weight")
        ws = torch.zeros((7, 8, 4, 64), dtype=torch.float32)
        ws[:, :7, :3, :] = w.permute(2, 3, 1, 0)
        g = self._get(sd, bu + "stem.conv1.norm.weight")
        beta = self._get(sd, bu + "stem.conv1.norm.bias")
        rm = self._get(sd, bu + "stem.conv1.norm.running_mean")
        rv = self._get(sd, bu + "stem.conv1.norm.running_var")
        sc = g * (rv + BN_EPS).rsqrt()
        self.stem_w = ws.to(self.device).contiguous()
        self.stem_scale = sc.to(self.device).contiguous()
        self.stem_bias = (beta - rm * sc).to(self.device).contiguous()
        self.stem_bound = float(((255.0 - min(PIXEL_MEAN)) * sc.abs() * w.abs().flatten(1).sum(1) + (beta - rm * sc).abs()).max())
        if self.p32:
            planes, sw = stem_weight_planes(w)
            if self.single_plane:
                planes[1].zero_()
            self.stem_planes = planes.to(self.device).contiguous()
            self.stem_s_in = p32.plane_scale(255.0 - min(PIXEL_MEAN))
            self.stem_scale_mfma = (sc / (sw * self.stem_s_in)).to(self.device).contiguous()
        self.blocks = []
        for stage, nblk in zip((2, 3, 4, 5), RES_BLOCKS[self.depth]):
            stage_blocks = []
            for i in range(nblk):
                p = f"{bu}res{stage}.{i}."
                stride = 2 if (i == 0 and stage > 2) else 1
                blk = {}
                if (p + "shortcut.weight") in sd:
                    blk["shortcut"] = self._conv(sd, p + "shortcut", stride=stride, norm=True, stage=f"res{stage}")
                blk["conv1"] = self._conv(sd, p + "conv1", stride=stride, norm=True, stage=f"res{stage}")
                blk["conv2"] = self._conv(sd, p + "conv2", pad=1, norm=True, stage=f"res{stage}")
                blk["conv3"] = self._conv(sd, p + "conv3", norm=True, stage=f"res{stage}")
                stage_blocks.append(blk)
            self.blocks.append(stage_blocks)
        self.fpn_lateral = {l: self._conv(sd, f"backbone.fpn_lateral{l}", bias=True, stage="fpn_lateral") for l in (2, 3, 4, 5)}
        self.fpn_output = {l: self._conv(sd, f"backbone.fpn_output{l}", pad=1, bias=True, stage="fpn_output") for l in (2, 3, 4, 5)}
        rp = "proposal_generator.rpn_head."
        self.rpn_conv = self._conv(sd, rp + "conv", pad=1, bias=True, stage="rpn_conv")
        wobj, wdel = self._get(sd, rp + "objectness_logits.weight"), self._get(sd, rp + "anchor_deltas.weight")
        bobj, bdel = self._get(sd, rp + "objectness_logits.bias"), self._get(sd, rp + "anchor_deltas.bias")
        self.rpn_pred = self._conv(sd, "", bias=True, weight=torch.cat([wobj, wdel], 0), bias_t=torch.cat([bobj, bdel], 0), stage="rpn_pred")
        bh = "roi_heads.box_head."
        w1 = self._get(sd, bh + "fc1.weight")
        w1 = w1.view(w1.shape[0], 256, 7, 7).permute(0, 2, 3, 1).reshape(w1.shape[0], 12544, 1, 1)
        self.fc1 = self._conv(sd, "", bias=True, weight=w1, bias_t=self._get(sd, bh + "fc1.bias"), stage="fc1")
        w2 = self._get(sd, bh + "fc2.weight")
        self.fc2 = self._conv(sd, "", bias=True, weight=w2[:, :, None, None], bias_t=self._get(sd, bh + "fc2.bias"), stage="fc2")
        bp = "roi_heads.box_predictor."
        wc, wb = self._get(sd, bp + "cls_score.weight"), self._get(sd, bp + "bbox_pred.weight")
        bc, bb = self._get(sd, bp + "cls_score.bias"), self._get(sd, bp + "bbox_pred.bias")
        if wc.shape[0] != self.K + 1 or wb.shape[0] != 4 * self.K:
            raise ValueError(f"checkpoint has {wc.shape[0] - 1} classes, dataset metadata says {self.K}")
        self.box_pred = self._conv(sd, "", bias=True, weight=torch.cat([wc, wb], 0)[:, :, None, None],
                                   bias_t=torch.cat([bc, bb], 0), stage="box_pred")
        mh = "roi_heads.mask_head."
        self.mask_fcn = [self._conv(sd, f"{mh}mask_fcn{i}", pad=1, bias=True, stage="mask_fcn") for i in range(1, 5)]
        wd = self._get(sd, mh + "deconv.weight")
        wd = wd.permute(2, 3, 1, 0).reshape(4 * wd.shape[1], wd.shape[0], 1, 1)
        self.deconv = self._conv(sd, "", bias=True, weight=wd, bias_t=self._get(sd, mh + "deconv.bias").repeat(4), stage="deconv")
        self.mask_pred = self._conv(sd, mh + "predictor", bias=True)
        self.mask_pred_w32 = self._get(sd, mh + "predictor.weight").reshape(-1, 256).to(self.device).contiguous()
        self.mask_pred_b32 = self._get(sd, mh + "predictor.bias").to(self.device).contiguous()
        self.unmatched_keys = sorted(k for k in sd if k not in self._used
                                     and not k.startswith(EXPECTED_IGNORED_PREFIXES))

    def _stream(self) -> int:
        return int(torch.cuda.current_stream(self.device).cuda_stream)

    def _begin_forward(self, key: tuple, ph: int, pw: int) -> None:
        self._touch_shape(key)
        self._arena_key, self._arena_i = key, 0
        b = key[0]
        self._groups = b if (b > 1 and ((ph // 32 - 1) // 2 + 1) * ((pw // 32 - 1) // 2 + 1) >= 128) else 1
        pool = self._meta_pools.get(key)
        if pool is None:
            pool = self._meta_pools[key] = torch.zeros((256, self._groups, 2), dtype=torch.float32, device=self.device)
        else:
            pool.zero_()
        self._meta_pool = pool
        self._meta_i = 0

    def _touch_shape(self, key: tuple) -> None:
        lru = self._shape_lru
        if lru and lru[-1] == key:
            return
        if key in lru:
            lru.remove(key)
        lru.append(key)
        while len(lru) > self.max_cached_shapes:
            self._evict_shape(lru.pop(0))

    def _evict_shape(self, key: tuple) -> None:
        torch.cuda.synchronize(self.device)
        self._graphs.pop(key, None)
        self._arena.pop(key, None)
        self._meta_pools.pop(key, None)
        self.evictions += 1

    def release_cached_shapes(self) -> None:
        while self._shape_lru:
            self._evict_shape(self._shape_lru.pop(0))
        self._arena_key = None

    def _scratch(self, numel: int, dtype, zero: bool = False, zero_head: int = 0) -> torch.Tensor:
        if self._arena_key is None:
            t = torch.zeros(numel, dtype=dtype, device=self.device) if zero else torch.empty(numel, dtype=dtype, device=self.device)
            if zero_head and not zero:
                t[:zero_head].zero_()
            return t
        slots = self._arena.setdefault(self._arena_key, [])
        i = self._arena_i
        self._arena_i += 1
        if i < len(slots) and slots[i].numel() == numel and slots[i].dtype == dtype:
            return slots[i]
        t = torch.zeros(numel, dtype=dtype, device=self.device) if zero else torch.empty(numel, dtype=dtype, device=self.device)
        if zero_head and not zero:
            t[:zero_head].zero_()
        if i < len(slots):
            slots[i] = t
        else:
            slots.append(t)
        return t

    def _meta_slot(self, groups: int) -> torch.Tensor:
        if self._arena_key is None:
            return torch.zeros((groups, 2), dtype=torch.float32, device=self.device)
        if groups != self._groups:
            return torch.zeros((groups, 2), dtype=torch.float32, device=self.device)
        if self._meta_i >= self._meta_pool.shape[0]:
            raise RuntimeError("activation meta pool exhausted inside one forward")
        m = self._meta_pool[self._meta_i]
        self._meta_i += 1
        return m

    def new_p32(self, shape, groups: Optional[int] = None) -> p32.P32:
        n = 1
        for d in shape:
            n *= int(d)
        buf = self._scratch(p32.HEADER_HALFS + 2 * n, torch.float16, zero_head=p32.HEADER_HALFS)
        return p32.P32(buf, self._meta_slot(self._groups if groups is None else groups), tuple(int(d) for d in shape))

    def dense(self, x) -> torch.Tensor:
        return p32.to_f32(x) if isinstance(x, p32.P32) else x.float()

    def conv_p32(self, x: p32.P32, L: ConvLayer, act=ACT_NONE, residual: Optional[p32.P32] = None, res_mode=RES_NONE,
                 out_f32: bool = False, out_ld: int = 0, tile_hint: int = 0, head=None):
        n, h, w, cin = x.shape
        assert cin == L.cin, (cin, L.cin)
        ho = (h + 2 * L.pad - L.kh) // L.stride + 1
        wo = (w + 2 * L.pad - L.kw) // L.stride + 1
        hw_ptr = hb_ptr = ho_ptr = hn = hld = hact = 0
        if head is not None:
            hw_t, hb_t, hld, hact = head
            hn = int(hw_t.shape[0])
            out = self._scratch(n * ho * wo * (L.cout // 256) * hld, torch.float32).view(n * ho * wo * (L.cout // 256), hld)
            hw_ptr, hb_ptr, ho_ptr = _lib.ptr(hw_t), _lib.ptr(hb_t), _lib.ptr(out)
            optr, ometa = 0, 0
        elif out_f32:
            ld = out_ld if out_ld > 0 else L.cout
            out = self._scratch(n * ho * wo * ld, torch.float32).view(n, ho, wo, ld)
            optr, ometa = _lib.ptr(out), 0
        else:
            out = self.new_p32((n, ho, wo, L.cout), x.groups)
            optr, ometa = _lib.ptr(out.buf), _lib.ptr(out.meta)
        pix_bytes = cin * 4
        limit = (1 << 32) - (1 << 20)
        chunks = [(0, n)]
        if 128 + n * h * w * pix_bytes >= limit:
            if not (h == 1 and w == 1 and L.kh == 1 and L.kw == 1 and L.pad == 0 and L.stride == 1 and res_mode != RES_UP2):
                raise ValueError(f"{n}x{h}x{w}x{cin} planes exceed 4 GiB: lower the batch size")
            step = (limit - 128) // pix_bytes // 256 * 256
            chunks = [(i, min(step, n - i)) for i in range(0, n, step)]
        ev = self.conv_events
        if ev is not None:
            e0, e1 = torch.cuda.Event(enable_timing=True), torch.cuda.Event(enable_timing=True)
            e0.record(torch.cuda.current_stream(self.device))
        groups = x.groups
        group_rows = (n * ho * wo) // groups
        assert groups == 1 or (group_rows * groups == n * ho * wo and (residual is None or residual.groups == groups)), (x.shape, groups)
        for c0, cn in chunks:
            d = _lib.ConvP32Desc(_lib.ptr(x.buf) + c0 * pix_bytes, _lib.ptr(x.meta), _lib.ptr(L.w3), _lib.ptr(L.scale3), _lib.ptr(L.bias),
                                 0 if residual is None else _lib.ptr(residual.buf) + c0 * L.cout * 4,
                                 0 if residual is None else _lib.ptr(residual.meta),
                                 (optr + c0 * (ld if out_f32 else L.cout) * 4) if optr else 0, ometa, L.wbound, L.bbound, cn, h, w, cin,
                                 ho, wo, L.cout, L.cout_pad, L.kh, L.kw, L.stride, L.pad, act, res_mode, 1 if out_f32 else 0, out_ld,
                                 tile_hint, hw_ptr, hb_ptr, (ho_ptr + c0 * (L.cout // 256) * hld * 4) if ho_ptr else 0, hn, hld, hact,
                                 groups, group_rows, c0, L.single)
            _lib.check(self.lib.demia_conv2d_p32(C.byref(d), self._stream()), "demia_conv2d_p32")
        if ev is not None:
            e1.record(torch.cuda.current_stream(self.device))
            nbytes = (n * h * w * cin * 4 + L.cout_pad * L.kh * L.kw * cin * 4 + n * ho * wo * L.cout * 4 +
                      (0 if residual is None else residual.pixels * residual.channels * 4))
            ev.append((e0, e1, 2.0 * n * ho * wo * L.cout * L.kh * L.kw * cin, "f16" if L.single else self.precision, nbytes))
        return out

    def conv(self, x, L: ConvLayer, act=ACT_NONE, residual=None, res_mode=RES_NONE,
             out_dtype=None, out: Optional[torch.Tensor] = None, out_ld: int = 0, tile_hint: int = 0):
        if self.p32:
            return self.conv_p32(x, L, act, residual, res_mode, out_f32=out_dtype is not None, out_ld=out_ld, tile_hint=tile_hint)
        n, h, w, cin = x.shape
        assert cin == L.cin, (cin, L.cin)
        ho = (h + 2 * L.pad - L.kh) // L.stride + 1
        wo = (w + 2 * L.pad - L.kw) // L.stride + 1
        odt = self.tdt if out_dtype is None else out_dtype
        ld = out_ld if out_ld > 0 else L.cout
        if out is None:
            out = torch.empty((n, ho, wo, ld), dtype=odt, device=self.device)
        use3 = L.w3 is not None and odt == torch.float32
        f16 = use3 and L.w3.dtype == torch.float16
        kind = ("f16x2r" if f16 else ("f32x3" if L.w3.shape[2] == 3 else "bf16x2")) if use3 else ("bf16" if self.dt == BF16 else "f32")
        amax_in = self.amax_of(x) if f16 else None
        amax_out = self._amax_slot() if self.precision == "f16x2r" else None
        d = _lib.ConvDesc(_lib.ptr(x), _lib.ptr(L.w3 if use3 else L.w), _lib.ptr(L.scale3 if f16 else L.scale), _lib.ptr(L.bias),
                          _lib.ptr(residual), _lib.ptr(out), n, h, w, cin, ho, wo, L.cout, L.cout_pad, L.kh, L.kw, L.stride, L.pad,
                          {"f16x2r": F16X2, "f32x3": F32X3, "bf16x2": BF16X2}.get(kind, self.dt), BF16 if odt == torch.bfloat16 else F32,
                          act, res_mode, ld, tile_hint, _lib.ptr(amax_in), _lib.ptr(amax_out))
        if amax_out is not None:
            out._amax = amax_out
        ev = self.conv_events
        if ev is not None:
            e0, e1 = torch.cuda.Event(enable_timing=True), torch.cuda.Event(enable_timing=True)
            e0.record(torch.cuda.current_stream(self.device))
        _lib.check(self.lib.demia_conv2d_nhwc(C.byref(d), self._stream()), "demia_conv2d_nhwc")
        if ev is not None:
            e1.record(torch.cuda.current_stream(self.device))
            esz = 2 if self.dt == BF16 else 4
            osz = 2 if odt == torch.bfloat16 else 4
            nbytes = (n * h * w * cin * esz + L.cout_pad * L.kh * L.kw * cin * (2 * int(L.w3.shape[2]) if use3 else esz) + n * ho * wo * L.cout * osz +
                      (0 if residual is None else residual.numel() * osz))
            ev.append((e0, e1, 2.0 * n * ho * wo * L.cout * L.kh * L.kw * cin, kind, nbytes))
        return out

    def _amax_slot(self) -> torch.Tensor:
        if self._amax_buf is None or self._amax_i >= self._amax_buf.numel():
            self._amax_buf = torch.zeros(512, dtype=torch.float32, device=self.device)
            self._amax_i = 0
        slot = self._amax_buf[self._amax_i:self._amax_i + 1]
        self._amax_i += 1
        return slot

    def amax_of(self, x: torch.Tensor) -> torch.Tensor:
        am = getattr(x, "_amax", None)
        if am is None:
            mn, mx = torch.aminmax(x)
            am = torch.maximum(mx, -mn).to(torch.float32).reshape(1)
            x._amax = am
        return am

    @staticmethod
    def view_as(x, *shape):
        if isinstance(x, p32.P32):
            return x.view(*shape)
        y = x.view(*shape)
        am = getattr(x, "_amax", None)
        if am is not None:
            y._amax = am
        return y

    def _resize_tables(self, h: int, w: int):
        key = (h, w)
        if key not in self._tables:
            newh, neww = resize_shape(h, w, self.min_size_test, self.max_size_test)
            xm, xs, xk = pil_bilinear_tables(w, neww)
            ym, ys, yk = pil_bilinear_tables(h, newh)
            t = lambda a: torch.from_numpy(a).to(self.device)
            self._tables[key] = dict(newh=newh, neww=neww, xm=t(xm), xs=t(xs), xk=t(xk), ksx=xk.shape[1],
                                     ym=t(ym), ys=t(ys), yk=t(yk), ksy=yk.shape[1], need_h=(w != neww))
        return self._tables[key]

    def resize_linear_u8(self, images: torch.Tensor, out_h: int, out_w: int) -> torch.Tensor:
        n, h, w, _ = images.shape
        xo, xa = cv_linear_tables(w, out_w)
        yo, ya = cv_linear_tables(h, out_h, vertical=True)
        t = lambda a: torch.from_numpy(a).to(self.device)
        xo, xa, yo, ya = t(xo), t(xa), t(yo), t(ya)
        out = torch.empty((n, out_h, out_w, 3), dtype=torch.uint8, device=self.device)
        _lib.check(self.lib.demia_resize_linear_u8(_lib.ptr(images.contiguous()), _lib.ptr(out), n, h, w, out_h, out_w, _lib.ptr(xo),
                                                   _lib.ptr(xa), _lib.ptr(yo), _lib.ptr(ya), self._stream()),
                   "demia_resize_linear_u8")
        return out

    def preprocess(self, images: torch.Tensor):
        b, h, w, _ = images.shape
        t = self._resize_tables(h, w)
        newh, neww = t["newh"], t["neww"]
        ph, pw = (newh + 31) // 32 * 32, (neww + 31) // 32 * 32
        if self.p32:
            self._begin_forward((b, h, w), ph, pw)
        st = self._stream()
        if t["need_h"]:
            tmp = (self._scratch(b * h * neww * 3, torch.uint8).view(b, h, neww, 3) if self.p32 else
                   torch.empty((b, h, neww, 3), dtype=torch.uint8, device=self.device))
            _lib.check(self.lib.demia_resize_h_u8(_lib.ptr(images), _lib.ptr(tmp), b, h, w, neww, _lib.ptr(t["xm"]),
                                                  _lib.ptr(t["xs"]), _lib.ptr(t["xk"]), t["ksx"], st), "demia_resize_h_u8")
        else:
            tmp = images
        dst = (self._scratch(b * (ph + 6) * (pw + 8) * 4, torch.float32, zero=True).view(b, ph + 6, pw + 8, 4) if self.p32 else
               torch.zeros((b, ph + 6, pw + 8, 4), dtype=torch.float32, device=self.device))
        mean = (C.c_float * 3)(*PIXEL_MEAN)
        _lib.check(self.lib.demia_resize_v_norm(_lib.ptr(tmp), _lib.ptr(dst), b, h, neww, newh, ph, pw, _lib.ptr(t["ym"]),
                                                _lib.ptr(t["ys"]), _lib.ptr(t["yk"]), t["ksy"], mean, F32, st),
                   "demia_resize_v_norm")
        return dst, newh, neww, ph, pw

    def backbone(self, xin: torch.Tensor, ph: int, pw: int) -> Dict[str, torch.Tensor]:
        b = xin.shape[0]
        st = self._stream()
        if self.p32:
            if self.stem_mode == "fused":
                x = self.new_p32((b, ph // 4, pw // 4, 64))
                _lib.check(self.lib.demia_stem_pool_mfma(_lib.ptr(xin), _lib.ptr(self.stem_planes), _lib.ptr(self.stem_scale_mfma),
                                                         _lib.ptr(self.stem_bias), _lib.ptr(x.buf), _lib.ptr(x.meta), b, ph, pw, self.stem_s_in,
                                                         p32.plane_scale(self.stem_bound), x.groups, int(self.single_plane), st), "demia_stem_pool_mfma")
                mid = None
            else:
                mid = self._scratch(b * (ph // 2) * (pw // 2) * 64, torch.float32)
            if mid is None:
                pass
            elif self.stem_on_mfma:
                _lib.check(self.lib.demia_stem_conv_mfma(_lib.ptr(xin), _lib.ptr(self.stem_planes), _lib.ptr(self.stem_scale_mfma),
                                                         _lib.ptr(self.stem_bias), _lib.ptr(mid), b, ph, pw, self.stem_s_in, st), "demia_stem_conv_mfma")
            else:
                _lib.check(self.lib.demia_stem_conv(_lib.ptr(xin), _lib.ptr(self.stem_w), _lib.ptr(self.stem_scale),
                                                    _lib.ptr(self.stem_bias), _lib.ptr(mid), b, ph, pw, F32, st), "demia_stem_conv")
            if mid is not None:
                x = self.new_p32((b, ph // 4, pw // 4, 64))
                _lib.check(self.lib.demia_maxpool3x3s2_p32(_lib.ptr(mid), _lib.ptr(x.buf), _lib.ptr(x.meta), p32.plane_scale(self.stem_bound),
                                                           b, ph // 2, pw // 2, 64, x.groups, int(self.single_plane), st), "demia_maxpool3x3s2_p32")
        else:
            mid = torch.empty((b, ph // 2, pw // 2, 64), dtype=self.tdt, device=self.device)
            _lib.check(self.lib.demia_stem_conv(_lib.ptr(xin), _lib.ptr(self.stem_w), _lib.ptr(self.stem_scale),
                                                _lib.ptr(self.stem_bias), _lib.ptr(mid), b, ph, pw, self.dt, st), "demia_stem_conv")
            x = torch.empty((b, ph // 4, pw // 4, 64), dtype=self.tdt, device=self.device)
            _lib.check(self.lib.demia_maxpool3x3s2(_lib.ptr(mid), _lib.ptr(x), b, ph // 2, pw // 2, 64, self.dt, st),
                       "demia_maxpool3x3s2")
        feats = {"stem": x}
        for si, stage_blocks in enumerate(self.blocks):
            for blk in stage_blocks:
                sc = self.conv(x, blk["shortcut"]) if "shortcut" in blk else x
                o = self.conv(x, blk["conv1"], act=ACT_RELU)
                o = self.conv(o, blk["conv2"], act=ACT_RELU)
                x = self.conv(o, blk["conv3"], act=ACT_RELU, residual=sc, res_mode=RES_SAME)
            feats[f"res{si + 2}"] = x
        prev = None
        for lvl in (5, 4, 3, 2):
            if prev is None:
                lat = self.conv(feats[f"res{lvl}"], self.fpn_lateral[lvl])
            else:
                lat = self.conv(feats[f"res{lvl}"], self.fpn_lateral[lvl], residual=prev, res_mode=RES_UP2)
            prev = lat
            feats[f"p{lvl}"] = self.conv(lat, self.fpn_output[lvl])
        p5 = feats["p5"]
        h5, w5 = p5.shape[1], p5.shape[2]
        if self.p32:
            p6 = self.new_p32((b, (h5 - 1) // 2 + 1, (w5 - 1) // 2 + 1, 256))
            p6 = p32.P32(p6.buf, p5.meta, p6.shape)
            _lib.check(self.lib.demia_subsample2(_lib.ptr(p5.buf) + 128, _lib.ptr(p6.buf) + 128, b, h5, w5, 256, F32, st), "demia_subsample2")
            feats["p6"] = p6
            return feats
        p6 = torch.empty((b, (h5 - 1) // 2 + 1, (w5 - 1) // 2 + 1, 256), dtype=self.tdt, device=self.device)
        _lib.check(self.lib.demia_subsample2(_lib.ptr(p5), _lib.ptr(p6), b, h5, w5, 256, self.dt, st), "demia_subsample2")
        feats["p6"] = p6
        return feats

    def rpn(self, feats, newh: int, neww: int):
        b = feats["p2"].shape[0]
        heads = []
        for name in ("p2", "p3", "p4", "p5", "p6"):
            t = self.conv(feats[name], self.rpn_conv, act=ACT_RELU)
            heads.append(self.conv(t, self.rpn_pred, out_dtype=torch.float32, out_ld=16))
        boxes = torch.empty((b, POST_NMS_TOPK, 4), dtype=torch.float32, device=self.device)
        scores = torch.empty((b, POST_NMS_TOPK), dtype=torch.float32, device=self.device)
        count = torch.empty((b,), dtype=torch.int32, device=self.device)
        ws = torch.empty((int(self.lib.demia_rpn_workspace_bytes(b)),), dtype=torch.uint8, device=self.device)
        d = _lib.RpnDesc()
        for i, hd in enumerate(heads):
            d.head[i] = _lib.ptr(hd)
            d.H[i], d.W[i], d.stride[i] = hd.shape[1], hd.shape[2], STRIDES[i]
        d.cell_anchors = self._cell.ctypes.data
        d.head_ld, d.N, d.img_h, d.img_w = 16, b, newh, neww
        d.pre_topk, d.post_topk, d.nms_thresh = PRE_NMS_TOPK, POST_NMS_TOPK, RPN_NMS_THRESH
        d.out_boxes, d.out_scores, d.out_count, d.workspace = _lib.ptr(boxes), _lib.ptr(scores), _lib.ptr(count), _lib.ptr(ws)
        _lib.check(self.lib.demia_rpn_proposals(C.byref(d), self._stream()), "demia_rpn_proposals")
        self._dbg_heads = heads
        return boxes, scores, count

    def roi_align(self, feats, boxes: torch.Tensor, count: torch.Tensor, P: int) -> torch.Tensor:
        b, r, _ = boxes.shape
        d = _lib.RoiAlignDesc()
        if self.roi_order and r <= 1024:
            order = torch.empty((b * r,), dtype=torch.int32, device=self.device)
            _lib.check(self.lib.demia_roi_order(_lib.ptr(boxes), _lib.ptr(count), b, r, _lib.ptr(order), self._stream()), "demia_roi_order")
            d.order = _lib.ptr(order)
        if isinstance(feats["p2"], p32.P32):
            out = self.new_p32((b, r, P, P, 256), feats["p2"].groups)
            for i, name in enumerate(("p2", "p3", "p4", "p5")):
                f = feats[name]
                d.feat[i], d.meta[i] = _lib.ptr(f.buf), _lib.ptr(f.meta)
                d.H[i], d.W[i] = f.shape[1], f.shape[2]
            d.N, d.R, d.C, d.P, d.dtype, d.groups, d.single = b, r, 256, P, _lib.P32, out.groups, int(self.single_plane)
            d.boxes, d.count, d.out, d.out_meta = _lib.ptr(boxes), _lib.ptr(count), _lib.ptr(out.buf), _lib.ptr(out.meta)
            _lib.check(self.lib.demia_roi_align(C.byref(d), self._stream()), "demia_roi_align")
            return out
        out = torch.empty((b, r, P, P, 256), dtype=self.tdt, device=self.device)
        for i, name in enumerate(("p2", "p3", "p4", "p5")):
            f = feats[name]
            d.feat[i] = _lib.ptr(f)
            d.H[i], d.W[i] = f.shape[1], f.shape[2]
        d.N, d.R, d.C, d.P, d.dtype = b, r, 256, P, self.dt
        d.boxes, d.count, d.out = _lib.ptr(boxes), _lib.ptr(count), _lib.ptr(out)
        _lib.check(self.lib.demia_roi_align(C.byref(d), self._stream()), "demia_roi_align")
        if self.precision == "f16x2r":
            out._amax = torch.cat([self.amax_of(feats[n]) for n in ("p2", "p3", "p4", "p5")]).amax().reshape(1)
        return out

    def box_head(self, pooled: torch.Tensor) -> torch.Tensor:
        b, r = pooled.shape[:2]
        x = self.view_as(pooled, b * r, 1, 1, 12544)
        x = self.conv(x, self.fc1, act=ACT_RELU)
        x = self.conv(x, self.fc2, act=ACT_RELU)
        ld = (5 * self.K + 1 + 3) // 4 * 4
        return self.conv(x, self.box_pred, out_dtype=torch.float32, out_ld=ld).view(b, r, ld)

    def detections(self, logits, props, prop_count, newh, neww):
        b, r, ld = logits.shape
        D = self.dets_per_image
        det_boxes = torch.empty((b, D, 4), dtype=torch.float32, device=self.device)
        det_scores = torch.empty((b, D), dtype=torch.float32, device=self.device)
        det_classes = torch.empty((b, D), dtype=torch.int32, device=self.device)
        det_count = torch.empty((b,), dtype=torch.int32, device=self.device)
        d = _lib.DetsDesc(_lib.ptr(logits), ld, _lib.ptr(props), _lib.ptr(prop_count), b, r, self.K, newh, neww,
                          self.score_thresh, DET_NMS_THRESH, D, _lib.ptr(det_boxes), _lib.ptr(det_scores),
                          _lib.ptr(det_classes), _lib.ptr(det_count))
        _lib.check(self.lib.demia_box_detections(C.byref(d), self._stream()), "demia_box_detections")
        return det_boxes, det_scores, det_classes, det_count

    def mask_head(self, mpooled: torch.Tensor) -> torch.Tensor:
        b, dd = mpooled.shape[:2]
        x = self.view_as(mpooled, b * dd, 14, 14, 256)
        for L in self.mask_fcn:
            x = self.conv(x, L, act=ACT_RELU)
        ld = (self.K + 3) // 4 * 4
        if self.p32 and self.K <= 4:
            return self.conv_p32(self.view_as(x, b * dd * 196, 1, 1, 256), self.deconv, act=ACT_RELU,
                                 head=(self.mask_pred_w32, self.mask_pred_b32, ld, ACT_SIGMOID)).view(b * dd * 196 * 4, 1, 1, ld)
        x = self.conv(self.view_as(x, b * dd * 196, 1, 1, 256), self.deconv, act=ACT_RELU)
        x = self.conv(self.view_as(x, b * dd * 196 * 4, 1, 1, 256), self.mask_pred, act=ACT_SIGMOID,
                      out_dtype=torch.float32, out_ld=(self.K + 3) // 4 * 4)
        return x

    def paste(self, mask_prob, det_boxes, det_classes, det_count, newh, neww, out_h, out_w):
        b, D = det_boxes.shape[:2]
        out_boxes = torch.empty((b, D, 4), dtype=torch.float32, device=self.device)
        valid = torch.empty((b, D), dtype=torch.uint8, device=self.device)
        bbox = torch.empty((b, D, 4), dtype=torch.int32, device=self.device)
        static = self._paste_static
        if static is not None:
            packed, prev = static
            assert tuple(packed.shape) == (b, D, out_h, (out_w + 31) // 32)
        else:
            packed, prev = torch.empty((b, D, out_h, (out_w + 31) // 32), dtype=torch.int32, device=self.device), None
        d = _lib.PasteDesc(_lib.ptr(mask_prob), mask_prob.shape[-1], _lib.ptr(det_boxes), _lib.ptr(det_classes),
                           _lib.ptr(det_count), b, D, newh, neww, out_h, out_w, _lib.ptr(out_boxes), _lib.ptr(valid),
                           _lib.ptr(packed), _lib.ptr(bbox), _lib.ptr(prev))
        _lib.check(self.lib.demia_paste_masks(C.byref(d), self._stream()), "demia_paste_masks")
        if prev is not None:
            prev.copy_(bbox)
        return out_boxes, valid, packed, bbox

    @torch.no_grad()
    def forward(self, images: torch.Tensor, keep_intermediates: bool = False) -> RawDetections:
        assert images.dtype == torch.uint8 and images.dim() == 4 and images.shape[3] == 3
        images = images.contiguous()
        b, h, w, _ = images.shape
        self._amax_buf = None
        xin, newh, neww, ph, pw = self.preprocess(images)
        feats = self.backbone(xin, ph, pw)
        props, pscores, pcount = self.rpn(feats, newh, neww)
        pooled = self.roi_align(feats, props, pcount, 7)
        logits = self.box_head(pooled)
        det_boxes, det_scores, det_classes, det_count = self.detections(logits, props, pcount, newh, neww)
        mpooled = self.roi_align(feats, det_boxes, det_count, 14)
        mask_prob = self.mask_head(mpooled)
        out_boxes, valid, packed, bbox = self.paste(mask_prob, det_boxes, det_classes, det_count, newh, neww, h, w)
        res = RawDetections(out_boxes, det_scores, det_classes, valid, det_count, packed, h, w, bbox)
        if keep_intermediates:
            res.dbg = dict(xin=xin, feats=feats, props=props, pscores=pscores, pcount=pcount, pooled=pooled,
                           logits=logits, det_boxes=det_boxes, mpooled=mpooled, mask_prob=mask_prob,
                           heads=self._dbg_heads, newh=newh, neww=neww)
        return res

    @torch.no_grad()
    def forward_graphed(self, images: torch.Tensor, slots: int = 2) -> RawDetections:
        if not self.p32:
            return self.forward(images)
        images = images.contiguous()
        key = tuple(int(d) for d in images.shape[:3])
        self._touch_shape(key)
        st = self._graphs.get(key)
        cur = torch.cuda.current_stream(self.device)
        if st is None:
            self.forward(images)
            st = {"graphs": [], "next": 0}
            side = torch.cuda.Stream(device=self.device)
            side.wait_stream(cur)
            with torch.cuda.stream(side):
                for _ in range(slots):
                    static_in = torch.empty_like(images)
                    b, h, w = key
                    planes = torch.zeros((b, self.dets_per_image, h, (w + 31) // 32), dtype=torch.int32, device=self.device)
                    prev = torch.full((b, self.dets_per_image, 4), -1, dtype=torch.int32, device=self.device)
                    g = torch.cuda.CUDAGraph()
                    self._paste_static = (planes, prev)
                    try:
                        with torch.cuda.graph(g, stream=side):
                            out = self.forward(static_in)
                    finally:
                        self._paste_static = None
                    out._slot = (key, len(st["graphs"]))
                    st["graphs"].append((g, static_in, out, planes, prev))
            st["released"] = [None] * len(st["graphs"])
            cur.wait_stream(side)
            self._graphs[key] = st
        slot = st["next"]
        g, static_in, out = st["graphs"][slot][:3]
        st["next"] = (slot + 1) % len(st["graphs"])
        ev = st["released"][slot]
        if ev is not None:
            cur.wait_event(ev)
            st["released"][slot] = None
        static_in.copy_(images, non_blocking=True)
        g.replay()
        return out

    def release_outputs(self, raw: RawDetections) -> None:
        slot = getattr(raw, "_slot", None)
        if slot is None:
            return
        st = self._graphs.get(slot[0])
        if st is not None:
            ev = torch.cuda.Event()
            ev.record(torch.cuda.current_stream(self.device))
            st["released"][slot[1]] = ev

    def unpack(self, packed: torch.Tensor, h: int, w: int) -> torch.Tensor:
        m = packed.shape[0]
        out = torch.empty((m, h, w), dtype=torch.bool, device=self.device)
        _lib.check(self.lib.demia_unpack_masks(_lib.ptr(packed), _lib.ptr(out), m, h, w, self._stream()), "demia_unpack_masks")
        return out

    def area_bbox(self, packed: torch.Tensor, h: int, w: int, hint: Optional[torch.Tensor] = None):
        m = packed.shape[0]
        area = torch.empty((m,), dtype=torch.int32, device=self.device)
        bbox = torch.empty((m, 4), dtype=torch.int32, device=self.device)
        _lib.check(self.lib.demia_mask_area_bbox(_lib.ptr(packed), _lib.ptr(hint), _lib.ptr(area), _lib.ptr(bbox), m, h, w, self._stream()),
                   "demia_mask_area_bbox")
        return area, bbox
```

include/deepemia_hip.h:

```cpp
#ifndef DEEPEMIA_HIP_H
#define DEEPEMIA_HIP_H

#include <stdint.h>

#ifdef __cplusplus
extern "C" {
#endif

#define DEMIA_OK 0
#define DEMIA_EINVAL (-1)
#define DEMIA_ELAUNCH (-2)

#define DEMIA_F32 0
#define DEMIA_BF16 1
#define DEMIA_F32X3 2
#define DEMIA_BF16X2 3
#define DEMIA_F16X2 4
#define DEMIA_P32 5

#define DEMIA_ACT_NONE 0
#define DEMIA_ACT_RELU 1
#define DEMIA_ACT_SIGMOID 2

#define DEMIA_RES_NONE 0
#define DEMIA_RES_SAME 1
#define DEMIA_RES_UP2 2

int demia_abi_version(void);
const char* demia_last_error(void);
const char* demia_build_arch(void);
const char* demia_build_flavor(void);
int demia_stream_create_cu_mask(const uint32_t* mask, int words, void** stream);
int demia_stream_destroy(void* stream);
struct demia_conv_p32_desc;
int demia_conv2d_p32_single(const struct demia_conv_p32_desc* d, void* stream);

typedef struct demia_conv_desc {
    const void* in;
    const void* w;
    const float* scale;
    const float* bias;
    const void* residual;
    void* out;
    int32_t N, H, W, Cin;
    int32_t Ho, Wo, Cout, CoutPad;
    int32_t KH, KW, stride, pad;
    int32_t dtype, out_dtype;
    int32_t act, res_mode;
    int32_t out_ld;
    int32_t tile_hint;
    const float* amax_in;
    float* amax_out;
} demia_conv_desc;
int demia_conv2d_nhwc(const demia_conv_desc* d, void* stream);
int demia_conv_f16x2_kstep(void);

typedef struct demia_conv_p32_desc {
    const void* in;
    const float* in_meta;
    const void* w;
    const float* scale;
    const float* bias;
    const void* residual;
    const float* res_meta;
    void* out;
    float* out_meta;
    float wbound, bbound;
    int32_t N, H, W, Cin;
    int32_t Ho, Wo, Cout, CoutPad;
    int32_t KH, KW, stride, pad;
    int32_t act, res_mode;
    int32_t out_f32;
    int32_t out_ld;
    int32_t tile_hint;
    const float* head_w;
    const float* head_b;
    float* head_out;
    int32_t head_n, head_ld, head_act;
    int32_t groups, group_rows, row0;
    int32_t single;
} demia_conv_p32_desc;
int demia_conv2d_p32(const demia_conv_p32_desc* d, void* stream);

int demia_resize_h_u8(const uint8_t* src, uint8_t* tmp, int N, int H, int W, int newW,
                      const int32_t* xmin, const int32_t* xsize, const int32_t* xk, int ksx, void* stream);
int demia_resize_v_norm(const uint8_t* tmp, void* dst, int N, int H, int newW, int newH, int PH, int PW,
                        const int32_t* ymin, const int32_t* ysize, const int32_t* yk, int ksy,
                        const float* mean3, int dtype, void* stream);

int demia_resize_linear_u8(const uint8_t* src, uint8_t* dst, int N, int H, int W, int out_h, int out_w,
                           const int32_t* xofs, const int16_t* ialpha, const int32_t* yofs, const int16_t* ibeta,
                           void* stream);

int demia_stem_conv(const void* in, const void* w, const float* scale, const float* bias, void* mid,
                    int N, int PH, int PW, int dtype, void* stream);
int demia_stem_conv_mfma(const float* in, const void* w_planes, const float* scale, const float* bias, float* mid, int N,
                         int PH, int PW, float s_in, void* stream);
int demia_stem_pool_mfma(const float* in, const void* w_planes, const float* scale, const float* bias, void* out, float* out_meta,
                         int N, int PH, int PW, float s_in, float s_out, int groups, int single, void* stream);
int demia_maxpool3x3s2(const void* in, void* out, int N, int H, int W, int C, int dtype, void* stream);
int demia_maxpool3x3s2_p32(const float* in, void* out, float* out_meta, float s, int N, int H, int W, int C, int groups, int single,
                           void* stream);
int demia_subsample2(const void* in, void* out, int N, int H, int W, int C, int dtype, void* stream);

typedef struct demia_rpn_desc {
    const float* head[5];
    int32_t H[5], W[5], stride[5];
    const float* cell_anchors;
    int32_t head_ld;
    int32_t N;
    int32_t img_h, img_w;
    int32_t pre_topk, post_topk;
    float nms_thresh;
    float* out_boxes;
    float* out_scores;
    int32_t* out_count;
    void* workspace;
} demia_rpn_desc;
int64_t demia_rpn_workspace_bytes(int N);
int demia_rpn_proposals(const demia_rpn_desc* d, void* stream);

typedef struct demia_roialign_desc {
    const void* feat[4];
    int32_t H[4], W[4];
    int32_t N, R, C, P, dtype;
    const float* boxes;
    const int32_t* count;
    void* out;
    const float* meta[4];
    float* out_meta;
    int32_t groups;
    int32_t single;
    const int32_t* order;
} demia_roialign_desc;
int demia_roi_align(const demia_roialign_desc* d, void* stream);
int demia_roi_order(const float* boxes, const int32_t* count, int N, int R, int32_t* order, void* stream);

typedef struct demia_dets_desc {
    const float* logits;
    int32_t ld;
    const float* props;
    const int32_t* prop_count;
    int32_t N, R, K;
    int32_t img_h, img_w;
    float score_thresh, nms_thresh;
    int32_t topk;
    float* det_boxes;
    float* det_scores;
    int32_t* det_classes;
    int32_t* det_count;
} demia_dets_desc;
int demia_box_detections(const demia_dets_desc* d, void* stream);

typedef struct demia_paste_desc {
    const float* mask_prob;
    int32_t ld;
    const float* det_boxes;
    const int32_t* det_classes;
    const int32_t* det_count;
    int32_t N, D;
    int32_t img_h, img_w;
    int32_t out_h, out_w;
    float* out_boxes;
    uint8_t* valid;
    uint32_t* packed;
    int32_t* out_bbox;
    const int32_t* prev_bbox;
} demia_paste_desc;
int demia_paste_masks(const demia_paste_desc* d, void* stream);
int demia_unpack_masks(const uint32_t* packed, uint8_t* out_bool, int64_t M, int H, int W, void* stream);
int demia_mask_area_bbox(const uint32_t* packed, const int32_t* hint, int32_t* area, int32_t* bbox, int64_t M, int H, int W,
                         void* stream);

enum { DEMIA_MOP_END = 0, DEMIA_MOP_FILL = 1, DEMIA_MOP_DILATE = 2, DEMIA_MOP_ERODE = 3, DEMIA_MOP_DROP_MULTI = 4,
       DEMIA_MOP_FLAG_MULTI = 5, DEMIA_MOP_GATE = 6 };
int demia_mask_program(uint32_t* masks, uint32_t* scratch, const int32_t* bbox, const uint8_t* active, uint32_t program,
                       int64_t M, int H, int W, int32_t* area, int32_t* bbox_out, int32_t* flag, void* stream);
int demia_mask_program_wl(uint32_t* masks, uint32_t* scratch, const int32_t* bbox, const uint8_t* active, uint32_t program,
                          int64_t M, int H, int W, int32_t* area, int32_t* bbox_out, int32_t* flag, int32_t* worklist, void* stream);
int demia_mask_overlap_prefix(uint32_t* masks, const int32_t* seg, const int32_t* bbox, int64_t M, int H, int W, void* stream);
int demia_mask_column_counts(const uint32_t* masks, const int32_t* seg, const int32_t* bbox, int64_t M, int H, int W,
                             int32_t* counts, void* stream);
int demia_mask_pair_intersections(const uint32_t* a, const uint32_t* b, const int32_t* pi, const int32_t* pj,
                                  const int32_t* bbox_a, const int32_t* bbox_b, int32_t* out, int64_t P,
                                  int H, int W, void* stream);
int demia_mask_pair_matrix(const uint32_t* masks, const int32_t* bbox, const int32_t* first, const int32_t* count,
                           const int32_t* label, int32_t* out, int64_t M, int ld, int H, int W, void* stream);
int demia_host_greedy_keep(const int32_t* inter, int ld, const int32_t* row_first, const int64_t* area, const int32_t* seg_first,
                           const int32_t* seg_len, int S, double thr, uint8_t* keep);
int demia_host_dedup_smart(const int32_t* inter, int ld, const int32_t* row_first, const int64_t* area, const int64_t* bbox,
                           const int32_t* items, const double* scores, const int32_t* classes, const int32_t* tile_off, int T,
                           double thr, int32_t* keep_out, int32_t* keep_cnt);
int64_t demia_host_repr_rows(const double* vals, int64_t rows, int cols, char* out, int64_t cap);
int64_t demia_host_rle_text(const uint32_t* payload, const int32_t* bbox, const int64_t* offsets, int64_t M, int H,
                            char* out, int64_t cap, int64_t* text_off);
int demia_mask_place_tiles(const uint32_t* src, uint32_t* dst, const int32_t* x_off, const int32_t* y_off, int64_t T,
                           int src_h, int src_w, int tile_h, int tile_w, int H, int W, void* stream);
int demia_mask_crop_pack(const uint32_t* masks, const int32_t* bbox, const int64_t* offsets, int64_t M, int H, int W,
                         uint32_t* payload, void* stream);
int demia_mask_gather_regions(const uint32_t* src, const int64_t* index, const int32_t* bbox, int64_t M, int H, int W,
                              uint32_t* dst, void* stream);
int demia_mask_gather_regions_pooled(const uint32_t* src, const int64_t* index, const int32_t* bbox, int64_t M, int H, int W,
                                     uint32_t* pool, int32_t* prev, int grow, void* stream);
int demia_mask_crop_unpack(const uint32_t* payload, const int32_t* bbox, const int64_t* offsets, int64_t M, int H, int W,
                           uint32_t* masks, void* stream);

int demia_crop_place_tiles(const uint32_t* src, const int32_t* x_off, const int32_t* y_off, int64_t M, int src_h, int src_w,
                           int tile_h, int tile_w, int H, int W, const int32_t* room, const int64_t* offsets, uint32_t* payload,
                           int32_t* area, int32_t* bbox, void* stream);
int demia_crop_gather(const uint32_t* src, const int64_t* src_offsets, const int64_t* index, const int32_t* dst_room,
                      const int64_t* dst_offsets, int64_t M, uint32_t* dst, void* stream);
int demia_crop_reroom(const uint32_t* src, const int32_t* src_room, const int64_t* src_offsets, const int64_t* index,
                      const int32_t* dst_room, const int64_t* dst_offsets, int64_t M, int64_t max_dst_words, uint32_t* dst, void* stream);
int demia_crop_pair_matrix(const uint32_t* payload, const int32_t* room, const int64_t* offsets, const int32_t* bbox,
                           const int32_t* first, const int32_t* count, const int32_t* label, int32_t* out, int64_t M, int ld,
                           void* stream);
int demia_crop_pair_intersections(const uint32_t* payload_a, const int32_t* room_a, const int64_t* offsets_a, const int32_t* bbox_a,
                                  const uint32_t* payload_b, const int32_t* room_b, const int64_t* offsets_b, const int32_t* bbox_b,
                                  const int32_t* pi, const int32_t* pj, int32_t* out, int64_t P, void* stream);
int demia_crop_unpack_pooled(const uint32_t* payload, const int32_t* room, const int64_t* offsets, const int32_t* bbox,
                             int64_t first, int64_t n, int H, int W, uint32_t* pool, int32_t* prev, int grow, void* stream);
int demia_crop_gray_histogram(const uint32_t* payload, const int32_t* room, const int64_t* offsets, const int32_t* bbox,
                              const uint8_t* image, int channels, int64_t M, int H, int W, int32_t* hist, void* stream);

int demia_mask_gray_histogram(const uint32_t* masks, const int32_t* bbox, const uint8_t* image, int channels,
                              int64_t M, int H, int W, int32_t* hist, void* stream);

int64_t demia_contour_work_ints(int M, int C, int max_points);
int64_t demia_contour_work_floats(int M, int C, int max_points);
int64_t demia_contour_work_doubles(int M, int C, int max_points);
int demia_mask_contours(const uint32_t* masks, uint32_t* scratch, const int32_t* bbox, int M, int H, int W, int C,
                        int max_points, int32_t* count, int32_t* info, double* red, int32_t* points,
                        int32_t* counters, void* stream);
int demia_mask_contours_wl(const uint32_t* masks, uint32_t* scratch, const int32_t* bbox, int M, int H, int W, int C,
                           int max_points, int32_t* count, int32_t* info, double* red, int32_t* points,
                           int32_t* counters, int32_t* worklist, void* stream);
int64_t demia_crop_contour_scratch(const int32_t* room_host, int64_t M, int H, int W, int64_t* scratch_off);
int demia_crop_contours_wl(const uint32_t* payload, const int32_t* room, const int64_t* offsets, const int32_t* bbox, int M, int H,
                           int W, int C, int max_points, int32_t* count, int32_t* info, double* red, int32_t* points,
                           int32_t* counters, int32_t* worklist, uint32_t* scratch, const int64_t* scratch_off, void* stream);
int demia_contour_measure(const int32_t* select , const int32_t* count, const int32_t* info,
                          const double* red, const int32_t* points, int M,
                          int C, int max_points, int32_t* work_i, float* work_f, double* work_d, double um_pix,
                          double* out, int out_c, void* stream);

int64_t demia_contour_shape_work_ints(int M, int C, int max_points);
int demia_contour_shape(const int32_t* select , const int32_t* count, const int32_t* info, const double* red,
                        const int32_t* points, int M, int C, int max_points, int32_t* work_i, double um_pix,
                        double* out , int out_c, void* stream);

int demia_mask_inscribed(const int32_t* select , const uint32_t* masks, uint32_t* scratch, const int32_t* bbox,
                         const int32_t* count, const int32_t* info, int M, int H, int W, int C, double um_pix,
                         double* out , int out_c, void* stream);
int demia_crop_inscribed(const int32_t* select , const uint32_t* payload, const int32_t* room, const int64_t* offsets,
                         const int32_t* bbox, const int32_t* count, const int32_t* info, int M, int H, int W, int C, double um_pix,
                         double* out , int out_c, uint32_t* scratch, const int64_t* scratch_off, void* stream);

int demia_mask_skeleton(const int32_t* select , const uint32_t* masks, uint32_t* scratch, const int32_t* bbox,
                        const int32_t* count, const int32_t* info, int M, int H, int W, int C, double um_pix,
                        double* out , int out_c, uint32_t* scratch2, uint32_t* skel_out, void* stream);
int64_t demia_crop_skeleton_scratch(const int32_t* room_host, int64_t M, int H, int W, int64_t* scratch2_off);
int demia_crop_skeleton(const int32_t* select , const uint32_t* payload, const int32_t* room, const int64_t* offsets,
                        const int32_t* bbox, const int32_t* count, const int32_t* info, int M, int H, int W, int C, double um_pix,
                        double* out , int out_c, uint32_t* scratch, const int64_t* scratch_off, uint32_t* scratch2,
                        const int64_t* scratch2_off, uint32_t* skel_out, void* stream);

int demia_mask_neighbours(const uint32_t* masks, const int32_t* bbox, const int32_t* group , int64_t M, int H, int W,
                          int64_t r2, const int64_t* point_off , uint32_t* points, int32_t* nborder ,
                          int64_t* sums , int64_t* table , void* stream);
int demia_crop_neighbours(const uint32_t* payload, const int32_t* room, const int64_t* offsets, const int32_t* bbox,
                          const int32_t* group , int64_t M, int H, int W, int64_t r2,
                          const int64_t* point_off , uint32_t* points, int32_t* nborder ,
                          int64_t* sums , int64_t* table , void* stream);

int demia_poly_rasterize(const double* xy, const int32_t* vert_off, const int32_t* edge_poly, const int32_t* edge_idx,
                         const int64_t* bnd_off, int32_t* bnd, int32_t* bnd_cnt, int32_t* err, int64_t E,
                         const int32_t* mask_poly, int64_t M, int H, int W, uint32_t* out, int32_t* area, int32_t* bbox,
                         void* stream);
int demia_mask_cross_matrix(const uint32_t* det, const int32_t* det_bbox, const int32_t* det_label, const uint32_t* gt,
                            const int32_t* gt_bbox, const int32_t* gt_label, const int32_t* gt_first, const int32_t* gt_count,
                            int32_t* out, int64_t D, int ld, int H, int W, void* stream);
int demia_mask_rle_colmajor(const uint32_t* masks, const int32_t* bbox, int32_t* n_counts, const int64_t* offsets,
                            uint32_t* counts, int64_t M, int H, int W, void* stream);
int demia_crop_poly_rasterize(const double* xy, const int32_t* vert_off, const int32_t* edge_poly, const int32_t* edge_idx,
                              const int64_t* bnd_off, int32_t* bnd, int32_t* bnd_cnt, int32_t* err, int64_t E,
                              const int32_t* mask_poly, int64_t M, int H, int W, const int32_t* room, const int64_t* offsets,
                              int64_t max_room_words, uint32_t* payload, int32_t* area, int32_t* bbox, void* stream);
int demia_crop_cross_matrix(const uint32_t* det_payload, const int32_t* det_room, const int64_t* det_offsets,
                            const int32_t* det_bbox, const int32_t* det_label, const uint32_t* gt_payload, const int32_t* gt_room,
                            const int64_t* gt_offsets, const int32_t* gt_bbox, const int32_t* gt_label, const int32_t* gt_first,
                            const int32_t* gt_count, int32_t* out, int64_t D, int ld, void* stream);
int demia_crop_rle_colmajor(const uint32_t* payload, const int32_t* room, const int64_t* room_offsets, const int32_t* bbox,
                            int32_t* n_counts, const int64_t* offsets, uint32_t* counts, int64_t M, int H, int W, void* stream);
int demia_host_coco_match(int64_t G, const int64_t* dt_off, const int64_t* gt_off, const double* dt_score,
                          const double* dt_area, const int64_t* dt_row, const double* gt_area, const uint8_t* gt_crowd,
                          const int64_t* gt_col, const double* iou, const double* area_rng, int A, const double* thr, int T,
                          int max_det, int32_t* dt_rank, uint8_t* dt_matched, uint8_t* dt_ignore, uint8_t* gt_ignore);
int64_t demia_host_rle_string(const uint32_t* counts, const int64_t* offsets, int64_t M, char* out, int64_t cap,
                              int64_t* text_off);

#ifdef __cplusplus
}
#endif
#endif
```

Before: 731.4.

## Fuse res2 bottleneck conv2 3x3 and conv3 1x1 into one chained P32 kernel

Adds a chained kernel that runs the 3x3 64->64 conv and the 1x1 64->256 conv with residual and ReLU inside one launch, keeping the 64-channel intermediate in LDS. The Python path routes qualifying bottleneck blocks (64-channel mid, f16x2 P32 precision) to it by default. It also moves the shared device helpers into a header. The goal is to avoid writing and re-reading the intermediate activation in global memory and to save one launch per block. The cost is higher LDS use per workgroup, which may lower occupancy, plus new per-group scale handling that must match the unfused path.

```diff
diff --git a/deepemia_amd/_lib.py b/deepemia_amd/_lib.py
--- a/deepemia_amd/_lib.py
+++ b/deepemia_amd/_lib.py
@@ -46,6 +46,19 @@
         ("head_w", C.c_void_p), ("head_b", C.c_void_p), ("head_out", C.c_void_p),
         ("head_n", C.c_int32), ("head_ld", C.c_int32), ("head_act", C.c_int32),
         ("groups", C.c_int32), ("group_rows", C.c_int32), ("row0", C.c_int32), ("single", C.c_int32),
+    ]
+
+
+class ConvP32ChainDesc(C.Structure):
+    _fields_ = [
+        ("in_", C.c_void_p), ("in_meta", C.c_void_p),
+        ("w2", C.c_void_p), ("scale2", C.c_void_p), ("bias2", C.c_void_p), ("wbound2", C.c_float), ("bbound2", C.c_float),
+        ("w3", C.c_void_p), ("scale3", C.c_void_p), ("bias3", C.c_void_p), ("wbound3", C.c_float), ("bbound3", C.c_float),
+        ("residual", C.c_void_p), ("res_meta", C.c_void_p), ("out", C.c_void_p), ("out_meta", C.c_void_p),
+        ("w_next", C.c_void_p), ("scale_next", C.c_void_p), ("bias_next", C.c_void_p),
+        ("wbound_next", C.c_float), ("bbound_next", C.c_float), ("out_next", C.c_void_p), ("next_meta", C.c_void_p),
+        ("N", C.c_int32), ("H", C.c_int32), ("W", C.c_int32), ("mid", C.c_int32), ("Cout", C.c_int32), ("stride", C.c_int32),
+        ("groups", C.c_int32), ("group_rows", C.c_int32), ("row0", C.c_int32),
     ]
 
 
@@ -99,6 +112,7 @@
     "demia_conv2d_nhwc": (C.c_int, [C.POINTER(ConvDesc), C.c_void_p]),
     "demia_conv2d_p32": (C.c_int, [C.POINTER(ConvP32Desc), C.c_void_p]),
     "demia_conv2d_p32_single": (C.c_int, [C.POINTER(ConvP32Desc), C.c_void_p]),
+    "demia_conv_p32_chain": (C.c_int, [C.POINTER(ConvP32ChainDesc), C.c_void_p]),
     "demia_resize_h_u8": (C.c_int, [C.c_void_p, C.c_void_p, C.c_int, C.c_int, C.c_int, C.c_int, C.c_void_p,
                                      C.c_void_p, C.c_void_p, C.c_int, C.c_void_p]),
     "demia_resize_v_norm": (C.c_int, [C.c_void_p, C.c_void_p, C.c_int, C.c_int, C.c_int, C.c_int, C.c_int, C.c_int,
diff --git a/deepemia_amd/csrc/conv_p32.hip b/deepemia_amd/csrc/conv_p32.hip
--- a/deepemia_amd/csrc/conv_p32.hip
+++ b/deepemia_amd/csrc/conv_p32.hip
@@ -26,133 +26,9 @@
 #define P32_FRAG_PIPE 0
 #endif
 
+#include "conv_p32_device.h"
+
 namespace {
-
-struct ConvQ {
-    const void* in;
-    const float* in_meta;
-    const void* w;
-    const float* scale;
-    const float* bias;
-    const void* res;
-    const float* res_meta;
-    void* out;
-    float* out_meta;
-    float wbound, bbound;
-    int N, H, W, Cin, Ho, Wo, Cout, CoutPad, KH, KW, stride, pad;
-    int act, res_mode, out_f32, out_ld;
-    int M, HoWo, ntn, nwg, ksteps, taps;
-    int kloop;
-    unsigned in_bytes, w_bytes;
-    unsigned out_bytes, res_bytes;
-    const float* head_w;
-    const float* head_b;
-    float* head_out;
-    int head_n, head_ld, head_act;
-    int groups, group_rows, row0;
-    int no_hk;
-    int zero_low;
-    int stagger_ticks;
-    int resident;
-};
-
-typedef __attribute__((address_space(3))) void lds_void;
-
-template <int OFF, int WAIT>
-__device__ __forceinline__ void ds_read2_b128(f16x8& a, f16x8& b, unsigned addr_a, unsigned addr_b) {
-    if constexpr (WAIT >= 0)
-        asm volatile("ds_read_b128 %0, %2 offset:%4\n\tds_read_b128 %1, %3 offset:%4\n\ts_waitcnt lgkmcnt(%5)"
-                     : "=&v"(a), "=&v"(b) : "v"(addr_a), "v"(addr_b), "n"(OFF), "n"(WAIT) : "memory");
-    else
-        asm volatile("ds_read_b128 %0, %2 offset:%4\n\tds_read_b128 %1, %3 offset:%4"
-                     : "=&v"(a), "=&v"(b) : "v"(addr_a), "v"(addr_b), "n"(OFF) : "memory");
-}
-
-template <int... Is, class F>
-__device__ __forceinline__ void static_for_impl(std::integer_sequence<int, Is...>, F&& f) { (f(std::integral_constant<int, Is>{}), ...); }
-template <int N, class F>
-__device__ __forceinline__ void static_for(F&& f) { static_for_impl(std::make_integer_sequence<int, N>{}, static_cast<F&&>(f)); }
-typedef int i32x4 __attribute__((ext_vector_type(4)));
-
-__device__ __forceinline__ void dma16(const i32x4 rsrc, unsigned lds_addr, unsigned voff, unsigned soff) {
-    unsigned keep;
-    asm volatile("s_mov_b32 %0, m0\n\ts_mov_b32 m0, %1\n\ts_nop 0\n\tbuffer_load_dwordx4 %2, %3, %4 offen lds\n\ts_mov_b32 m0, %0"
-                 : "=&s"(keep) : "s"(lds_addr), "v"(voff), "s"(rsrc), "s"(soff) : "memory");
-}
-__device__ __forceinline__ void dma16_nt(const i32x4 rsrc, unsigned lds_addr, unsigned voff, unsigned soff) {
-    unsigned keep;
-    asm volatile("s_mov_b32 %0, m0\n\ts_mov_b32 m0, %1\n\ts_nop 0\n\tbuffer_load_dwordx4 %2, %3, %4 offen nt lds\n\ts_mov_b32 m0, %0"
-                 : "=&s"(keep) : "s"(lds_addr), "v"(voff), "s"(rsrc), "s"(soff) : "memory");
-}
-__device__ __forceinline__ i32x4 make_rsrc(const void* base, unsigned bytes) {
-    const unsigned long long a = reinterpret_cast<unsigned long long>(base);
-    i32x4 r;
-    r[0] = __builtin_amdgcn_readfirstlane((int)(unsigned)a);
-    r[1] = __builtin_amdgcn_readfirstlane((int)((unsigned)(a >> 32) & 0xffffu));
-    r[2] = __builtin_amdgcn_readfirstlane((int)bytes);
-    r[3] = 0x00020000;
-    return r;
-}
-
-__device__ __forceinline__ float apply_act_q(float v, int act) {
-    if (act == DEMIA_ACT_RELU) return v > 0.f ? v : 0.f;
-    if (act == DEMIA_ACT_SIGMOID) return 1.0f / (1.0f + expf(-v));
-    return v;
-}
-
-__device__ __forceinline__ float plane_scale(float bound) {
-    if (!(bound > 0.f) || !(bound < 3.0e38f)) return 1.f;
-    int e = 14 - ilogbf(bound);
-    e = e < -100 ? -100 : (e > 100 ? 100 : e);
-    return ldexpf(1.f, e);
-}
-
-template <int TN, int EF>
-__device__ __forceinline__ void write_acc32(const f32x16 (&row)[TN], float* e, int lane) {
-#pragma unroll
-    for (int j = 0; j < TN; ++j)
-#pragma unroll
-        for (int r = 0; r < 16; ++r)
-            e[((r & 3) + 8 * (r >> 2) + 4 * (lane >> 5)) * EF + j * 32 + (lane & 31)] = row[j][r];
-}
-template <int TN, int EF>
-__device__ __forceinline__ void write_acc16(const f32x4 (&r0)[2 * TN], const f32x4 (&r1)[2 * TN], float* e, int lane) {
-#pragma unroll
-    for (int j = 0; j < 2 * TN; ++j)
-#pragma unroll
-        for (int r = 0; r < 4; ++r) {
-            e[(4 * (lane >> 4) + r) * EF + j * 16 + (lane & 15)] = r0[j][r];
-            e[(16 + 4 * (lane >> 4) + r) * EF + j * 16 + (lane & 15)] = r1[j][r];
-        }
-}
-
-__device__ __forceinline__ float uniform(float v) { return __int_as_float(__builtin_amdgcn_readfirstlane(__float_as_int(v))); }
-
-struct GroupScales {
-    int g0, b1, b2;
-    float post0, post1, post2, resi0, resi1, resi2, sout0, sout1, sout2;
-};
-
-__device__ __forceinline__ void load_group_scale(const ConvQ& p, int gi, bool planes_out, float& post, float& resi, float& sout) {
-    gi = min(gi, p.groups - 1);
-    const float amax_in = p.in_meta[2 * gi], s_in = p.in_meta[2 * gi + 1];
-    float amax_res = 0.f, s_res = 1.f;
-    if (p.res_mode != DEMIA_RES_NONE) { amax_res = p.res_meta[2 * gi]; s_res = p.res_meta[2 * gi + 1]; }
-    post = uniform(1.0f / s_in);
-    resi = uniform(p.res_mode != DEMIA_RES_NONE ? 1.0f / s_res : 0.f);
-    sout = uniform(planes_out ? plane_scale(amax_in * p.wbound + p.bbound + amax_res) : 1.f);
-}
-
-__device__ __forceinline__ GroupScales load_group_scales(const ConvQ& p, int m0, bool planes_out) {
-    GroupScales gs;
-    gs.g0 = (m0 + p.row0) / p.group_rows;
-    gs.b1 = (gs.g0 + 1) * p.group_rows - p.row0;
-    gs.b2 = gs.b1 + p.group_rows;
-    load_group_scale(p, gs.g0, planes_out, gs.post0, gs.resi0, gs.sout0);
-    load_group_scale(p, gs.g0 + 1, planes_out, gs.post1, gs.resi1, gs.sout1);
-    load_group_scale(p, gs.g0 + 2, planes_out, gs.post2, gs.resi2, gs.sout2);
-    return gs;
-}
 
 template <int WM, int WN, int TM, int TN, bool HEAD, typename WriteRow>
 __device__ __forceinline__ void p32_epilogue(const ConvQ& p, const GroupScales& gs, char* smem, WriteRow&& write_tile_row, int wm, int wn, int m0, int n0) {
@@ -325,165 +201,6 @@
             if (lane == 0 && vmax > *reinterpret_cast<volatile const float*>(slot))
                 atomicMax(reinterpret_cast<unsigned int*>(slot), __float_as_uint(vmax));
         }
-    }
-}
-
-struct NoHook { __device__ __forceinline__ void operator()() const {} };
-template <int WM, int WN, int TM, int TN, typename WriteRow, typename Hook = NoHook>
-__device__ __forceinline__ void p32_epilogue_planes(const ConvQ& p, const GroupScales& gs, char* smem, WriteRow&& write_tile_row, int wm, int wn,
-                                                    int m0, int n0, bool leader = (threadIdx.x == 0), Hook&& hook = NoHook()) {
-    constexpr int BM_ = WM * TM * 32;
-    const int tid = threadIdx.x, lane = tid & 63;
-    constexpr int LDW = TN * 32 + 4;
-    constexpr int PPW = 8 / TN, RPI = 2 * PPW, ITEMS = 32 / RPI;
-    static_assert(TN == 1 || TN == 2 || TN == 4, "TN");
-    char* const wsm = smem + (tid >> 6) * (32 * LDW * 4);
-    const int g0 = __builtin_amdgcn_readfirstlane(gs.g0), b1 = __builtin_amdgcn_readfirstlane(gs.b1), b2 = __builtin_amdgcn_readfirstlane(gs.b2);
-    const float post0 = uniform(gs.post0), post1 = uniform(gs.post1), post2 = uniform(gs.post2);
-    const float resi0 = uniform(gs.resi0), resi1 = uniform(gs.resi1), resi2 = uniform(gs.resi2);
-    const float sout0 = uniform(gs.sout0), sout1 = uniform(gs.sout1), sout2 = uniform(gs.sout2);
-    if (n0 == 0 && leader) {
-#pragma unroll
-        for (int d = 0; d < 3; ++d) {
-            const int first = d == 0 ? g0 * p.group_rows - p.row0 : (d == 1 ? b1 : b2);
-            if (g0 + d < p.groups && first >= m0 && first < m0 + BM_ && first < p.M)
-                p.out_meta[2 * (g0 + d) + 1] = d == 0 ? sout0 : (d == 1 ? sout1 : sout2);
-        }
-    }
-    const int cj = lane & 3, rs = (lane >> 2) & 1, lg = lane >> 3;
-    const int line = lg % TN;
-    const int r_first = (lg / TN) * 2 + rs;
-    const int co = n0 + ((wn * TN + line) * 4 + cj) * 8;
-    float sc[8], bs[8];
-#pragma unroll
-    for (int q = 0; q < 8; ++q) {
-        sc[q] = p.scale ? p.scale[co + q] : 1.0f;
-        bs[q] = p.bias ? p.bias[co + q] : 0.0f;
-    }
-    const bool sigmoid_on = p.act == DEMIA_ACT_SIGMOID;
-    const float act_lo = p.act == DEMIA_ACT_RELU ? 0.f : -INFINITY;
-    const bool res_on = p.res_mode != DEMIA_RES_NONE;
-    const bool single = P32_SINGLE != 0 && p.zero_low != 0;
-    const __amdgpu_buffer_rsrc_t rs_out = __builtin_amdgcn_make_buffer_rsrc(p.out, 0, (int)p.out_bytes, 0x00020000);
-    const __amdgpu_buffer_rsrc_t rs_res = __builtin_amdgcn_make_buffer_rsrc(const_cast<void*>(res_on ? p.res : p.out), 0, res_on ? (int)p.res_bytes : 0, 0x00020000);
-    const unsigned cbytes = (unsigned)p.Cout * 4u;
-    const unsigned lofs = 128u + (unsigned)((co >> 5) * 128 + (lane & 7) * 16);
-    auto row_of = [&](int i, int k) { return m0 + wm * (TM * 32) + i * 32 + r_first + k * RPI; };
-    auto res_off = [&](int m) -> unsigned {
-        if (p.res_mode != DEMIA_RES_UP2 || (P32_ABLATE & 256)) return (unsigned)m * cbytes + lofs;
-        const int n = m / p.HoWo;
-        const int rem = m - n * p.HoWo;
-        const int ho = rem / p.Wo, wo = rem - ho * p.Wo;
-        const int Hr = (p.Ho + 1) >> 1, Wr = (p.Wo + 1) >> 1;
-        return (unsigned)((n * Hr + (ho >> 1)) * Wr + (wo >> 1)) * cbytes + lofs;
-    };
-    auto from_below = [&](u32x4 own, u32x4 theirs) -> u32x4 {
-        u32x4 r;
-#pragma unroll
-        for (int c = 0; c < 4; ++c) r[c] = (unsigned)__builtin_amdgcn_update_dpp((int)own[c], (int)theirs[c], 0x114, 0xf, 0xa, false);
-        return r;
-    };
-    auto from_above = [&](u32x4 own, u32x4 theirs) -> u32x4 {
-        u32x4 r;
-#pragma unroll
-        for (int c = 0; c < 4; ++c) r[c] = (unsigned)__builtin_amdgcn_update_dpp((int)own[c], (int)theirs[c], 0x104, 0xf, 0x5, false);
-        return r;
-    };
-    u32x4 rh[ITEMS], rl[ITEMS];
-    auto load_res = [&](int i) {
-#pragma unroll
-        for (int k = 0; k < ITEMS; ++k) {
-            const int mp = row_of(i, k) - rs;
-            if (P32_ABLATE & 32) { rh[k] = u32x4{0, 0, 0, 0}; rl[k] = rh[k]; continue; }
-            rh[k] = __builtin_amdgcn_raw_buffer_load_b128(rs_res, res_off(mp), 0, P32_RES_AUX);
-            rl[k] = __builtin_amdgcn_raw_buffer_load_b128(rs_res, res_off(mp + 1), 0, P32_RES_AUX);
-        }
-    };
-    float vmax0 = 0.f, vmax1 = 0.f, vmax2 = 0.f;
-    if (P32_ABLATE & 512) return;
-    load_res(0);
-#pragma unroll
-    for (int i = 0; i < TM; ++i) {
-        asm volatile("" ::: "memory");
-        __builtin_amdgcn_wave_barrier();
-        write_tile_row(i, reinterpret_cast<float*>(wsm));
-        asm volatile("" ::: "memory");
-        __builtin_amdgcn_wave_barrier();
-        f16x8 ch[ITEMS], cl[ITEMS];
-#pragma unroll
-        for (int k = 0; k < ITEMS; ++k) {
-            ch[k] = __builtin_bit_cast(f16x8, from_below(rh[k], rl[k]));
-            cl[k] = __builtin_bit_cast(f16x8, from_above(rl[k], rh[k]));
-        }
-        if (i + 1 < TM) load_res(i + 1);
-#pragma unroll
-        for (int k = 0; k < ITEMS; ++k) {
-            const int lr = r_first + k * RPI;
-            const int m = row_of(i, k);
-            const float4 x0 = *reinterpret_cast<const float4*>(wsm + lr * (LDW * 4) + (line * 4 + cj) * 32);
-            const float4 x1 = *reinterpret_cast<const float4*>(wsm + lr * (LDW * 4) + (line * 4 + cj) * 32 + 16);
-            typedef float f32x2 __attribute__((ext_vector_type(2)));
-            f32x2 v2[4] = {{x0.x, x0.y}, {x0.z, x0.w}, {x1.x, x1.y}, {x1.z, x1.w}};
-            const int gd = (m >= b1) + (m >= b2);
-            const float post = gd == 0 ? post0 : (gd == 1 ? post1 : post2);
-            const float res_inv = gd == 0 ? resi0 : (gd == 1 ? resi1 : resi2);
-            const float s_out = gd == 0 ? sout0 : (gd == 1 ? sout1 : sout2);
-            float v[8];
-#pragma unroll
-            for (int q = 0; q < 4; ++q) {
-                const f32x2 scq = {sc[2 * q], sc[2 * q + 1]}, bsq = {bs[2 * q], bs[2 * q + 1]};
-                const f32x2 t = (v2[q] * post) * scq + bsq;
-                v[2 * q] = t.x;
-                v[2 * q + 1] = t.y;
-            }
-#pragma unroll
-            for (int q = 0; q < 8; ++q) {
-                v[q] = fmaf((float)cl[k][q], res_inv, fmaf((float)ch[k][q], res_inv, v[q]));
-                v[q] = fmaxf(v[q], act_lo);
-            }
-            if (sigmoid_on && !(P32_ABLATE & 256)) {
-#pragma unroll
-                for (int q = 0; q < 8; ++q) v[q] = 1.0f / (1.0f + expf(-v[q]));
-            }
-            f16x8 h, l;
-            float vm = 0.f;
-#pragma unroll
-            for (int q = 0; q < 8; q += 2) {
-                vm = fmaxf(vm, fmaxf(fabsf(v[q]), fabsf(v[q + 1])));
-                const f32x2 y = f32x2{v[q], v[q + 1]} * s_out;
-                h[q] = (_Float16)y.x;
-                h[q + 1] = (_Float16)y.y;
-                l[q] = (_Float16)fmaf(-(float)h[q], 1.0f, y.x);
-                l[q + 1] = (_Float16)fmaf(-(float)h[q + 1], 1.0f, y.y);
-            }
-            if (single) l = f16x8{0, 0, 0, 0, 0, 0, 0, 0};
-            vm = m < p.M ? vm : 0.f;
-            vmax0 = fmaxf(vmax0, gd == 0 ? vm : 0.f);
-            vmax1 = fmaxf(vmax1, gd == 1 ? vm : 0.f);
-            vmax2 = fmaxf(vmax2, gd == 2 ? vm : 0.f);
-            const u32x4 hu = __builtin_bit_cast(u32x4, h), lu = __builtin_bit_cast(u32x4, l);
-            const u32x4 d0 = from_below(hu, lu);
-            const u32x4 d1 = from_above(lu, hu);
-            const unsigned off = (unsigned)(m - rs) * cbytes + lofs;
-            if (P32_ABLATE & 64) {
-                asm volatile("" :: "v"(d0), "v"(d1), "v"(off));
-            } else {
-                __builtin_amdgcn_raw_buffer_store_b128(d0, rs_out, off, 0, P32_ST_AUX);
-                __builtin_amdgcn_raw_buffer_store_b128(d1, rs_out, off + cbytes, 0, P32_ST_AUX);
-            }
-            hook();
-        }
-    }
-#pragma unroll
-    for (int d = 0; d < 3; ++d) {
-        if (d > 0 && (d == 1 ? b1 : b2) >= m0 + BM_) break;
-        if (g0 + d >= p.groups) break;
-        float vmax = d == 0 ? vmax0 : (d == 1 ? vmax1 : vmax2);
-#pragma unroll
-        for (int o = 32; o > 0; o >>= 1) vmax = fmaxf(vmax, __shfl_xor(vmax, o));
-        float* slot = p.out_meta + 2 * (g0 + d);
-        if (lane == 0 && vmax > *reinterpret_cast<volatile const float*>(slot))
-            atomicMax(reinterpret_cast<unsigned int*>(slot), __float_as_uint(vmax));
     }
 }
 
diff --git a/deepemia_amd/csrc/conv_p32_chain.hip b/deepemia_amd/csrc/conv_p32_chain.hip
--- /dev/null
+++ b/deepemia_amd/csrc/conv_p32_chain.hip
@@ -0,0 +1,290 @@
+#include "conv_p32_device.h"
+
+namespace {
+
+struct ChainQ {
+    ConvQ c2;
+    ConvQ c3;
+};
+
+constexpr int CH_BM = 256, CH_MID = 64, CH_OUT = 256;
+constexpr int CH_STAGE = (CH_BM + CH_MID) * 128;
+constexpr int CH_PIECE = 32 * (2 * 32 + 4) * 4;
+constexpr int CH_KLOOP = 18;
+constexpr int CH_PIECES = 2 * CH_STAGE;
+constexpr int CH_TAB = CH_PIECES + 8 * CH_PIECE;
+constexpr int CH_SMEM = CH_TAB + 2 * CH_OUT * 4;
+static_assert(CH_KLOOP % 3 == 0 && CH_OUT * 128 <= CH_STAGE && CH_SMEM <= 160 * 1024, "LDS");
+
+__device__ __forceinline__ void chain_group_scale(const ChainQ& q, int gi, float& post2, float& sb, float& post3, float& resi, float& sout) {
+    gi = min(gi, q.c2.groups - 1);
+    const float amax_a = q.c2.in_meta[2 * gi], s_a = q.c2.in_meta[2 * gi + 1];
+    const float amax_x = q.c3.res_meta[2 * gi], s_x = q.c3.res_meta[2 * gi + 1];
+    const float bound_b = amax_a * q.c2.wbound + q.c2.bbound;
+    post2 = uniform(1.0f / s_a);
+    sb = uniform(plane_scale(bound_b));
+    post3 = uniform(1.0f / sb);
+    resi = uniform(1.0f / s_x);
+    sout = uniform(plane_scale(bound_b * q.c3.wbound + q.c3.bbound + amax_x));
+}
+
+__global__ __launch_bounds__(512, 2) void conv_p32_chain_kernel(const ChainQ q) {
+    const ConvQ& p = q.c2;
+    constexpr int NW = 8, QA = CH_BM / 8 / NW;
+    extern __shared__ __attribute__((aligned(16))) char smem[];
+    const int tid = threadIdx.x, lane = tid & 63;
+    const int wave = __builtin_amdgcn_readfirstlane(tid >> 6);
+    const int m0 = xcd_remap(blockIdx.x, p.nwg) * CH_BM;
+    const i32x4 rsrc_a = make_rsrc(p.in, p.in_bytes), rsrc_b = make_rsrc(p.w, p.w_bytes), rsrc_w3 = make_rsrc(q.c3.w, q.c3.w_bytes);
+    const unsigned lds0 = (unsigned)(__SIZE_TYPE__)((lds_void*)smem);
+
+    unsigned a_off[QA], a_msk[QA], b_off;
+#pragma unroll
+    for (int k = 0; k < QA; ++k) {
+        const int row = (wave + NW * k) * 8 + (lane >> 3);
+        const int csw = (lane & 7) ^ ((row >> 1) & 7);
+        const int m = m0 + row;
+        const bool vm = m < p.M;
+        const int mm = vm ? m : 0;
+        const int n = mm / p.HoWo;
+        const int rem = mm - n * p.HoWo;
+        const int ho = rem / p.Wo, wo = rem - ho * p.Wo;
+        const int hi0 = ho - p.pad, wi0 = wo - p.pad;
+        const long pix = ((long)n * p.H + hi0) * p.W + wi0;
+        a_off[k] = (unsigned)(128 + pix * (long)(p.Cin * 4) + csw * 16);
+        unsigned mk = 0;
+        for (int t = 0, th = 0, tw = 0; t < p.taps; ++t) {
+            if (vm && (unsigned)(hi0 + th) < (unsigned)p.H && (unsigned)(wi0 + tw) < (unsigned)p.W) mk |= 1u << t;
+            if (++tw == p.KW) { tw = 0; ++th; }
+        }
+        a_msk[k] = mk;
+    }
+    {
+        const int row = wave * 8 + (lane >> 3);
+        const int csw = (lane & 7) ^ ((row >> 1) & 7);
+        b_off = (unsigned)(row * 128 + csw * 16);
+    }
+    int tap = 0, kw = 0, tstep = 0;
+    unsigned sdelta = 0, srow = 0, sgrp = 0;
+    auto issue = [&](int st, int tp, unsigned sd, unsigned bd) {
+        const unsigned sbase = __builtin_amdgcn_readfirstlane(lds0 + st * CH_STAGE + wave * 1024);
+#pragma unroll
+        for (int k = 0; k < QA; ++k) {
+            const bool ok = (a_msk[k] >> tp) & 1u;
+            const unsigned vo = ok ? a_off[k] + sd : (a_off[k] & 0x70u);
+            dma16(rsrc_a, sbase + k * (NW * 1024), vo, 0u);
+        }
+        dma16(rsrc_b, sbase + CH_BM * 128, b_off, bd);
+    };
+    auto issue_w3 = [&](int ks) {
+#pragma unroll
+        for (int r = 0; r < 4; ++r) {
+            const int piece = wave + NW * r;
+            const int row = piece * 8 + (lane >> 3);
+            const int csw = (lane & 7) ^ ((row >> 1) & 7);
+            const unsigned vo = (unsigned)(((row >> 6) * 2 + ks) * 8192 + (row & 63) * 128 + csw * 16);
+            dma16(rsrc_w3, __builtin_amdgcn_readfirstlane(lds0 + ks * CH_STAGE + piece * 1024), vo, 0u);
+        }
+    };
+    const unsigned pixb = (unsigned)(p.Cin * 4), rowb = (unsigned)(p.W * p.Cin * 4);
+#define CHAIN_ADVANCE()                                                                 \
+    do {                                                                                \
+        ++tstep;                                                                        \
+        if (++tap == p.taps) { tap = 0; kw = 0; srow = 0; sgrp += 128u; sdelta = sgrp; } \
+        else if (++kw == p.KW) { kw = 0; srow += rowb; sdelta = srow + sgrp; }          \
+        else sdelta += pixb;                                                            \
+    } while (0)
+
+    int frag[2];
+#pragma unroll
+    for (int pl = 0; pl < 2; ++pl) frag[pl] = (lane & 15) * 128 + ((pl * 4 + (lane >> 4)) ^ (((lane & 15) >> 1) & 7)) * 16;
+
+    f32x4 acc16[2][4];
+#pragma unroll
+    for (int i = 0; i < 2; ++i)
+#pragma unroll
+        for (int j = 0; j < 4; ++j) acc16[i][j] = f32x4{0.f, 0.f, 0.f, 0.f};
+    auto compute = [&](int st) {
+        const char* sa = smem + st * CH_STAGE + wave * 32 * 128, *sb = smem + st * CH_STAGE + CH_BM * 128;
+        f16x8 bh[4], bl[4];
+#pragma unroll
+        for (int j = 0; j < 4; ++j) {
+            bh[j] = *reinterpret_cast<const f16x8*>(sb + frag[0] + j * 2048);
+            bl[j] = *reinterpret_cast<const f16x8*>(sb + frag[1] + j * 2048);
+        }
+#pragma unroll
+        for (int i = 0; i < 2; ++i) {
+            const f16x8 ah = *reinterpret_cast<const f16x8*>(sa + frag[0] + i * 2048);
+            const f16x8 al = *reinterpret_cast<const f16x8*>(sa + frag[1] + i * 2048);
+#pragma unroll
+            for (int j = 0; j < 4; ++j) {
+                f32x4 c = acc16[i][j];
+                c = __builtin_amdgcn_mfma_f32_16x16x32_f16(ah, bl[j], c, 0, 0, 0);
+                c = __builtin_amdgcn_mfma_f32_16x16x32_f16(al, bh[j], c, 0, 0, 0);
+                c = __builtin_amdgcn_mfma_f32_16x16x32_f16(ah, bh[j], c, 0, 0, 0);
+                acc16[i][j] = c;
+            }
+        }
+    };
+
+    reinterpret_cast<float*>(smem + CH_TAB)[tid] = tid < CH_OUT ? (q.c3.scale ? q.c3.scale[tid] : 1.0f) : (q.c3.bias ? q.c3.bias[tid - CH_OUT] : 0.0f);
+    issue(0, tap, sdelta, 0u);
+    CHAIN_ADVANCE();
+    issue(1, tap, sdelta, (unsigned)tstep * 8192u);
+    CHAIN_ADVANCE();
+    GroupScales gs;
+    gs.g0 = (m0 + p.row0) / p.group_rows;
+    gs.b1 = (gs.g0 + 1) * p.group_rows - p.row0;
+    gs.b2 = gs.b1 + p.group_rows;
+    float post2_0, post2_1, post2_2, sb0, sb1, sb2;
+    chain_group_scale(q, gs.g0, post2_0, sb0, gs.post0, gs.resi0, gs.sout0);
+    chain_group_scale(q, gs.g0 + 1, post2_1, sb1, gs.post1, gs.resi1, gs.sout1);
+    chain_group_scale(q, gs.g0 + 2, post2_2, sb2, gs.post2, gs.resi2, gs.sout2);
+    asm volatile("s_waitcnt vmcnt(%0)" ::"n"(QA + 1) : "memory");
+    __builtin_amdgcn_s_barrier();
+    int st = 0;
+    for (int t = 0; t < CH_KLOOP; ++t) {
+        const int st_issue = st == 0 ? 2 : st - 1;
+        const bool more = t + 2 < CH_KLOOP;
+        if (more) {
+            issue(st_issue, tap, sdelta, (unsigned)tstep * 8192u);
+            CHAIN_ADVANCE();
+        } else {
+            issue_w3(t - (CH_KLOOP - 2));
+        }
+        compute(st);
+        if (more) asm volatile("s_waitcnt vmcnt(%0) lgkmcnt(0)\n\ts_barrier" ::"n"(QA + 1) : "memory");
+        else if (t + 1 < CH_KLOOP) asm volatile("s_waitcnt vmcnt(4) lgkmcnt(0)\n\ts_barrier" ::: "memory");
+        else asm volatile("s_waitcnt vmcnt(0) lgkmcnt(0)\n\ts_barrier" ::: "memory");
+        st = st == 2 ? 0 : st + 1;
+    }
+#undef CHAIN_ADVANCE
+    char* const piece = smem + CH_PIECES + wave * CH_PIECE;
+
+    {
+        const int b1 = __builtin_amdgcn_readfirstlane(gs.b1), b2 = __builtin_amdgcn_readfirstlane(gs.b2);
+        const float act_lo = p.act == DEMIA_ACT_RELU ? 0.f : -INFINITY;
+        float sc2[4], bs2[4];
+#pragma unroll
+        for (int j = 0; j < 4; ++j) {
+            sc2[j] = p.scale ? p.scale[j * 16 + (lane & 15)] : 1.0f;
+            bs2[j] = p.bias ? p.bias[j * 16 + (lane & 15)] : 0.0f;
+        }
+#pragma unroll
+        for (int i = 0; i < 2; ++i)
+#pragma unroll
+            for (int r = 0; r < 4; ++r) {
+                const int row = i * 16 + 4 * (lane >> 4) + r;
+                const int m = m0 + wave * 32 + row;
+                const int gd = (m >= b1) + (m >= b2);
+                const float post = gd == 0 ? post2_0 : (gd == 1 ? post2_1 : post2_2);
+                const float sb = gd == 0 ? sb0 : (gd == 1 ? sb1 : sb2);
+                const int sw = (row >> 1) & 7;
+#pragma unroll
+                for (int j = 0; j < 4; ++j) {
+                    const float v = fmaxf((acc16[i][j][r] * post) * sc2[j] + bs2[j], act_lo);
+                    const float y = v * sb;
+                    const _Float16 h = (_Float16)y;
+                    const _Float16 l = (_Float16)fmaf(-(float)h, 1.0f, y);
+                    const int cc = (j & 1) * 16 + (lane & 15);
+                    char* line = piece + (j >> 1) * 4096 + row * 128 + (cc & 7) * 2;
+                    *reinterpret_cast<_Float16*>(line + (((cc >> 3) ^ sw) * 16)) = h;
+                    *reinterpret_cast<_Float16*>(line + (((4 + (cc >> 3)) ^ sw) * 16)) = l;
+                }
+            }
+    }
+    asm volatile("" ::: "memory");
+    __builtin_amdgcn_wave_barrier();
+
+    f32x4 acc3[4][2][4];
+#pragma unroll
+    for (int c = 0; c < 4; ++c)
+#pragma unroll
+        for (int i = 0; i < 2; ++i)
+#pragma unroll
+            for (int j = 0; j < 4; ++j) acc3[c][i][j] = f32x4{0.f, 0.f, 0.f, 0.f};
+#pragma unroll
+    for (int ks = 0; ks < 2; ++ks) {
+        f16x8 ah[2], al[2];
+#pragma unroll
+        for (int i = 0; i < 2; ++i) {
+            ah[i] = *reinterpret_cast<const f16x8*>(piece + ks * 4096 + i * 2048 + frag[0]);
+            al[i] = *reinterpret_cast<const f16x8*>(piece + ks * 4096 + i * 2048 + frag[1]);
+        }
+#pragma unroll
+        for (int c = 0; c < 4; ++c) {
+            const char* wb = smem + ks * CH_STAGE + c * (64 * 128);
+            f16x8 bh[4], bl[4];
+#pragma unroll
+            for (int j = 0; j < 4; ++j) {
+                bh[j] = *reinterpret_cast<const f16x8*>(wb + j * 2048 + frag[0]);
+                bl[j] = *reinterpret_cast<const f16x8*>(wb + j * 2048 + frag[1]);
+            }
+#pragma unroll
+            for (int i = 0; i < 2; ++i)
+#pragma unroll
+                for (int j = 0; j < 4; ++j) {
+                    f32x4 a = acc3[c][i][j];
+                    a = __builtin_amdgcn_mfma_f32_16x16x32_f16(ah[i], bl[j], a, 0, 0, 0);
+                    a = __builtin_amdgcn_mfma_f32_16x16x32_f16(al[i], bh[j], a, 0, 0, 0);
+                    a = __builtin_amdgcn_mfma_f32_16x16x32_f16(ah[i], bh[j], a, 0, 0, 0);
+                    acc3[c][i][j] = a;
+                }
+        }
+    }
+
+    auto write_pass = [&](int c, float* e) { write_acc16<2, 2 * 32 + 4>(acc3[c][0], acc3[c][1], e, lane); };
+    p32_epilogue_planes<8, 1, 4, 2, decltype(write_pass)&, NoHook, true>(q.c3, gs, smem + CH_PIECES, write_pass, wave, 0, m0, 0, tid == 0, NoHook(), smem + CH_TAB);
+}
+
+}
+
+extern "C" int demia_conv_p32_chain(const demia_conv_p32_chain_desc* d, void* stream) {
+    DEMIA_REQUIRE(d && d->in && d->in_meta && d->w2 && d->w3 && d->residual && d->res_meta && d->out && d->out_meta, "null pointer");
+    DEMIA_REQUIRE(d->mid == 64 && d->Cout == 256, "the chain takes mid width 64 and 256 output channels");
+    DEMIA_REQUIRE(d->stride == 1, "the chain takes stride 1");
+    DEMIA_REQUIRE(d->N > 0 && d->H > 0 && d->W > 0 && (long)d->N * d->H * d->W < (1L << 31), "geometry");
+    const long M = (long)d->N * d->H * d->W;
+    const int groups = d->groups > 1 ? d->groups : 1;
+    DEMIA_REQUIRE(d->group_rows >= 128 && d->row0 >= 0 && (groups == 1 || (M + d->row0 + d->group_rows - 1) / d->group_rows <= groups),
+                  "scale groups: group_rows >= 128 and the rows of this call must fall inside `groups` groups");
+    DEMIA_REQUIRE(!d->w_next || (d->out_next && d->next_meta), "next conv1: output pointers");
+    const long in_bytes = 128 + M * 64 * 4, out_bytes = 128 + M * 256 * 4;
+    DEMIA_REQUIRE(out_bytes < (1L << 32) - 512 && (M + 256) * 256 * 4 + 256 < (1L << 32), "planes must stay below 4 GiB");
+
+    ChainQ q{};
+    ConvQ& c2 = q.c2;
+    c2.in = d->in; c2.in_meta = d->in_meta; c2.w = d->w2; c2.scale = d->scale2; c2.bias = d->bias2;
+    c2.wbound = d->wbound2; c2.bbound = d->bbound2;
+    c2.N = d->N; c2.H = d->H; c2.W = d->W; c2.Cin = 64; c2.Ho = d->H; c2.Wo = d->W; c2.Cout = 64; c2.CoutPad = 64;
+    c2.KH = c2.KW = 3; c2.stride = 1; c2.pad = 1; c2.act = DEMIA_ACT_RELU; c2.res_mode = DEMIA_RES_NONE;
+    c2.M = (int)M; c2.HoWo = d->H * d->W; c2.ntn = 1; c2.nwg = cdiv(M, CH_BM); c2.taps = 9; c2.ksteps = c2.kloop = CH_KLOOP;
+    c2.in_bytes = (unsigned)in_bytes; c2.w_bytes = 64u * 9 * 64 * 4;
+    c2.groups = groups; c2.group_rows = groups > 1 ? d->group_rows : (1 << 29); c2.row0 = groups > 1 ? d->row0 : 0; c2.resident = 256;
+    ConvQ& c3 = q.c3;
+    c3 = c2;
+    c3.in = nullptr; c3.in_meta = nullptr;
+    c3.w = d->w3; c3.w_bytes = 256u * 64 * 4; c3.scale = d->scale3; c3.bias = d->bias3; c3.wbound = d->wbound3; c3.bbound = d->bbound3;
+    c3.res = d->residual; c3.res_meta = d->res_meta; c3.out = d->out; c3.out_meta = d->out_meta;
+    c3.Cin = 64; c3.Cout = c3.CoutPad = 256; c3.KH = c3.KW = 1; c3.pad = 0; c3.taps = 1; c3.ksteps = c3.kloop = 2;
+    c3.act = DEMIA_ACT_RELU; c3.res_mode = DEMIA_RES_SAME;
+    c3.out_bytes = c3.res_bytes = (unsigned)out_bytes;
+
+    hipStream_t st = reinterpret_cast<hipStream_t>(stream);
+    static bool attr_done = false;
+    if (!attr_done) {
+        (void)hipFuncSetAttribute(reinterpret_cast<const void*>(conv_p32_chain_kernel), hipFuncAttributeMaxDynamicSharedMemorySize, CH_SMEM);
+        attr_done = true;
+    }
+    hipLaunchKernelGGL(conv_p32_chain_kernel, dim3(c2.nwg), dim3(512), CH_SMEM, st, q);
+    DEMIA_CHECK_LAUNCH("conv_p32_chain_kernel");
+    if (!d->w_next) return DEMIA_OK;
+
+    demia_conv_p32_desc n{};
+    n.in = d->out; n.in_meta = d->out_meta; n.w = d->w_next; n.scale = d->scale_next; n.bias = d->bias_next;
+    n.out = d->out_next; n.out_meta = d->next_meta; n.wbound = d->wbound_next; n.bbound = d->bbound_next;
+    n.N = d->N; n.H = d->H; n.W = d->W; n.Cin = 256; n.Ho = d->H; n.Wo = d->W; n.Cout = 64; n.CoutPad = 64;
+    n.KH = n.KW = 1; n.stride = 1; n.pad = 0; n.act = DEMIA_ACT_RELU; n.res_mode = DEMIA_RES_NONE;
+    n.groups = d->groups; n.group_rows = d->group_rows; n.row0 = d->row0;
+    return demia_conv2d_p32(&n, stream);
+}
diff --git a/deepemia_amd/csrc/conv_p32_device.h b/deepemia_amd/csrc/conv_p32_device.h
--- /dev/null
+++ b/deepemia_amd/csrc/conv_p32_device.h
@@ -0,0 +1,315 @@
+#pragma once
+#include <utility>
+#include "common.h"
+#ifndef P32_ABLATE
+#define P32_ABLATE 0
+#endif
+#ifndef P32_SINGLE
+#define P32_SINGLE 0
+#endif
+#ifndef P32_ST_AUX
+#define P32_ST_AUX 0
+#endif
+#ifndef P32_RES_AUX
+#define P32_RES_AUX 0
+#endif
+
+namespace {
+
+struct ConvQ {
+    const void* in;
+    const float* in_meta;
+    const void* w;
+    const float* scale;
+    const float* bias;
+    const void* res;
+    const float* res_meta;
+    void* out;
+    float* out_meta;
+    float wbound, bbound;
+    int N, H, W, Cin, Ho, Wo, Cout, CoutPad, KH, KW, stride, pad;
+    int act, res_mode, out_f32, out_ld;
+    int M, HoWo, ntn, nwg, ksteps, taps;
+    int kloop;
+    unsigned in_bytes, w_bytes;
+    unsigned out_bytes, res_bytes;
+    const float* head_w;
+    const float* head_b;
+    float* head_out;
+    int head_n, head_ld, head_act;
+    int groups, group_rows, row0;
+    int no_hk;
+    int zero_low;
+    int stagger_ticks;
+    int resident;
+};
+
+typedef __attribute__((address_space(3))) void lds_void;
+
+template <int OFF, int WAIT>
+__device__ __forceinline__ void ds_read2_b128(f16x8& a, f16x8& b, unsigned addr_a, unsigned addr_b) {
+    if constexpr (WAIT >= 0)
+        asm volatile("ds_read_b128 %0, %2 offset:%4\n\tds_read_b128 %1, %3 offset:%4\n\ts_waitcnt lgkmcnt(%5)"
+                     : "=&v"(a), "=&v"(b) : "v"(addr_a), "v"(addr_b), "n"(OFF), "n"(WAIT) : "memory");
+    else
+        asm volatile("ds_read_b128 %0, %2 offset:%4\n\tds_read_b128 %1, %3 offset:%4"
+                     : "=&v"(a), "=&v"(b) : "v"(addr_a), "v"(addr_b), "n"(OFF) : "memory");
+}
+
+template <int... Is, class F>
+__device__ __forceinline__ void static_for_impl(std::integer_sequence<int, Is...>, F&& f) { (f(std::integral_constant<int, Is>{}), ...); }
+template <int N, class F>
+__device__ __forceinline__ void static_for(F&& f) { static_for_impl(std::make_integer_sequence<int, N>{}, static_cast<F&&>(f)); }
+typedef int i32x4 __attribute__((ext_vector_type(4)));
+
+__device__ __forceinline__ void dma16(const i32x4 rsrc, unsigned lds_addr, unsigned voff, unsigned soff) {
+    unsigned keep;
+    asm volatile("s_mov_b32 %0, m0\n\ts_mov_b32 m0, %1\n\ts_nop 0\n\tbuffer_load_dwordx4 %2, %3, %4 offen lds\n\ts_mov_b32 m0, %0"
+                 : "=&s"(keep) : "s"(lds_addr), "v"(voff), "s"(rsrc), "s"(soff) : "memory");
+}
+__device__ __forceinline__ void dma16_nt(const i32x4 rsrc, unsigned lds_addr, unsigned voff, unsigned soff) {
+    unsigned keep;
+    asm volatile("s_mov_b32 %0, m0\n\ts_mov_b32 m0, %1\n\ts_nop 0\n\tbuffer_load_dwordx4 %2, %3, %4 offen nt lds\n\ts_mov_b32 m0, %0"
+                 : "=&s"(keep) : "s"(lds_addr), "v"(voff), "s"(rsrc), "s"(soff) : "memory");
+}
+__device__ __forceinline__ i32x4 make_rsrc(const void* base, unsigned bytes) {
+    const unsigned long long a = reinterpret_cast<unsigned long long>(base);
+    i32x4 r;
+    r[0] = __builtin_amdgcn_readfirstlane((int)(unsigned)a);
+    r[1] = __builtin_amdgcn_readfirstlane((int)((unsigned)(a >> 32) & 0xffffu));
+    r[2] = __builtin_amdgcn_readfirstlane((int)bytes);
+    r[3] = 0x00020000;
+    return r;
+}
+
+__device__ __forceinline__ float apply_act_q(float v, int act) {
+    if (act == DEMIA_ACT_RELU) return v > 0.f ? v : 0.f;
+    if (act == DEMIA_ACT_SIGMOID) return 1.0f / (1.0f + expf(-v));
+    return v;
+}
+
+__device__ __forceinline__ float plane_scale(float bound) {
+    if (!(bound > 0.f) || !(bound < 3.0e38f)) return 1.f;
+    int e = 14 - ilogbf(bound);
+    e = e < -100 ? -100 : (e > 100 ? 100 : e);
+    return ldexpf(1.f, e);
+}
+
+template <int TN, int EF>
+__device__ __forceinline__ void write_acc32(const f32x16 (&row)[TN], float* e, int lane) {
+#pragma unroll
+    for (int j = 0; j < TN; ++j)
+#pragma unroll
+        for (int r = 0; r < 16; ++r)
+            e[((r & 3) + 8 * (r >> 2) + 4 * (lane >> 5)) * EF + j * 32 + (lane & 31)] = row[j][r];
+}
+template <int TN, int EF>
+__device__ __forceinline__ void write_acc16(const f32x4 (&r0)[2 * TN], const f32x4 (&r1)[2 * TN], float* e, int lane) {
+#pragma unroll
+    for (int j = 0; j < 2 * TN; ++j)
+#pragma unroll
+        for (int r = 0; r < 4; ++r) {
+            e[(4 * (lane >> 4) + r) * EF + j * 16 + (lane & 15)] = r0[j][r];
+            e[(16 + 4 * (lane >> 4) + r) * EF + j * 16 + (lane & 15)] = r1[j][r];
+        }
+}
+
+__device__ __forceinline__ float uniform(float v) { return __int_as_float(__builtin_amdgcn_readfirstlane(__float_as_int(v))); }
+
+struct GroupScales {
+    int g0, b1, b2;
+    float post0, post1, post2, resi0, resi1, resi2, sout0, sout1, sout2;
+};
+
+__device__ __forceinline__ void load_group_scale(const ConvQ& p, int gi, bool planes_out, float& post, float& resi, float& sout) {
+    gi = min(gi, p.groups - 1);
+    const float amax_in = p.in_meta[2 * gi], s_in = p.in_meta[2 * gi + 1];
+    float amax_res = 0.f, s_res = 1.f;
+    if (p.res_mode != DEMIA_RES_NONE) { amax_res = p.res_meta[2 * gi]; s_res = p.res_meta[2 * gi + 1]; }
+    post = uniform(1.0f / s_in);
+    resi = uniform(p.res_mode != DEMIA_RES_NONE ? 1.0f / s_res : 0.f);
+    sout = uniform(planes_out ? plane_scale(amax_in * p.wbound + p.bbound + amax_res) : 1.f);
+}
+
+__device__ __forceinline__ GroupScales load_group_scales(const ConvQ& p, int m0, bool planes_out) {
+    GroupScales gs;
+    gs.g0 = (m0 + p.row0) / p.group_rows;
+    gs.b1 = (gs.g0 + 1) * p.group_rows - p.row0;
+    gs.b2 = gs.b1 + p.group_rows;
+    load_group_scale(p, gs.g0, planes_out, gs.post0, gs.resi0, gs.sout0);
+    load_group_scale(p, gs.g0 + 1, planes_out, gs.post1, gs.resi1, gs.sout1);
+    load_group_scale(p, gs.g0 + 2, planes_out, gs.post2, gs.resi2, gs.sout2);
+    return gs;
+}
+
+struct NoHook { __device__ __forceinline__ void operator()() const {} };
+template <int WM, int WN, int TM, int TN, typename WriteRow, typename Hook = NoHook, bool COLS = false>
+__device__ __forceinline__ void p32_epilogue_planes(const ConvQ& p, const GroupScales& gs, char* smem, WriteRow&& write_tile_row, int wm, int wn,
+                                                    int m0, int n0, bool leader = (threadIdx.x == 0), Hook&& hook = NoHook(), const char* cols_tab = nullptr) {
+    constexpr int BM_ = COLS ? WM * 32 : WM * TM * 32;
+    const int tid = threadIdx.x, lane = tid & 63;
+    constexpr int LDW = TN * 32 + 4;
+    constexpr int PPW = 8 / TN, RPI = 2 * PPW, ITEMS = 32 / RPI;
+    static_assert(TN == 1 || TN == 2 || TN == 4, "TN");
+    char* const wsm = smem + (tid >> 6) * (32 * LDW * 4);
+    const int g0 = __builtin_amdgcn_readfirstlane(gs.g0), b1 = __builtin_amdgcn_readfirstlane(gs.b1), b2 = __builtin_amdgcn_readfirstlane(gs.b2);
+    const float post0 = uniform(gs.post0), post1 = uniform(gs.post1), post2 = uniform(gs.post2);
+    const float resi0 = uniform(gs.resi0), resi1 = uniform(gs.resi1), resi2 = uniform(gs.resi2);
+    const float sout0 = uniform(gs.sout0), sout1 = uniform(gs.sout1), sout2 = uniform(gs.sout2);
+    if (n0 == 0 && leader) {
+#pragma unroll
+        for (int d = 0; d < 3; ++d) {
+            const int first = d == 0 ? g0 * p.group_rows - p.row0 : (d == 1 ? b1 : b2);
+            if (g0 + d < p.groups && first >= m0 && first < m0 + BM_ && first < p.M)
+                p.out_meta[2 * (g0 + d) + 1] = d == 0 ? sout0 : (d == 1 ? sout1 : sout2);
+        }
+    }
+    const int cj = lane & 3, rs = (lane >> 2) & 1, lg = lane >> 3;
+    const int line = lg % TN;
+    const int r_first = (lg / TN) * 2 + rs;
+    const int co = n0 + ((wn * TN + line) * 4 + cj) * 8;
+    float sc[8], bs[8];
+#pragma unroll
+    for (int q = 0; q < 8; ++q) {
+        if (COLS) continue;
+        sc[q] = p.scale ? p.scale[co + q] : 1.0f;
+        bs[q] = p.bias ? p.bias[co + q] : 0.0f;
+    }
+    const bool sigmoid_on = p.act == DEMIA_ACT_SIGMOID;
+    const float act_lo = p.act == DEMIA_ACT_RELU ? 0.f : -INFINITY;
+    const bool res_on = p.res_mode != DEMIA_RES_NONE;
+    const bool single = P32_SINGLE != 0 && p.zero_low != 0;
+    const __amdgpu_buffer_rsrc_t rs_out = __builtin_amdgcn_make_buffer_rsrc(p.out, 0, (int)p.out_bytes, 0x00020000);
+    const __amdgpu_buffer_rsrc_t rs_res = __builtin_amdgcn_make_buffer_rsrc(const_cast<void*>(res_on ? p.res : p.out), 0, res_on ? (int)p.res_bytes : 0, 0x00020000);
+    const unsigned cbytes = (unsigned)p.Cout * 4u;
+    const unsigned lofs = 128u + (unsigned)((co >> 5) * 128 + (lane & 7) * 16);
+    auto row_of = [&](int i, int k) { return COLS ? m0 + wm * 32 + r_first + k * RPI : m0 + wm * (TM * 32) + i * 32 + r_first + k * RPI; };
+    auto col_off = [&](int i) -> unsigned { return COLS ? (unsigned)(i * TN * 128) : 0u; };
+    auto res_off = [&](int m) -> unsigned {
+        if (p.res_mode != DEMIA_RES_UP2 || (P32_ABLATE & 256)) return (unsigned)m * cbytes + lofs;
+        const int n = m / p.HoWo;
+        const int rem = m - n * p.HoWo;
+        const int ho = rem / p.Wo, wo = rem - ho * p.Wo;
+        const int Hr = (p.Ho + 1) >> 1, Wr = (p.Wo + 1) >> 1;
+        return (unsigned)((n * Hr + (ho >> 1)) * Wr + (wo >> 1)) * cbytes + lofs;
+    };
+    auto from_below = [&](u32x4 own, u32x4 theirs) -> u32x4 {
+        u32x4 r;
+#pragma unroll
+        for (int c = 0; c < 4; ++c) r[c] = (unsigned)__builtin_amdgcn_update_dpp((int)own[c], (int)theirs[c], 0x114, 0xf, 0xa, false);
+        return r;
+    };
+    auto from_above = [&](u32x4 own, u32x4 theirs) -> u32x4 {
+        u32x4 r;
+#pragma unroll
+        for (int c = 0; c < 4; ++c) r[c] = (unsigned)__builtin_amdgcn_update_dpp((int)own[c], (int)theirs[c], 0x104, 0xf, 0x5, false);
+        return r;
+    };
+    u32x4 rh[ITEMS], rl[ITEMS];
+    auto load_res = [&](int i) {
+#pragma unroll
+        for (int k = 0; k < ITEMS; ++k) {
+            const int mp = row_of(i, k) - rs;
+            if (P32_ABLATE & 32) { rh[k] = u32x4{0, 0, 0, 0}; rl[k] = rh[k]; continue; }
+            rh[k] = __builtin_amdgcn_raw_buffer_load_b128(rs_res, res_off(mp) + col_off(i), 0, P32_RES_AUX);
+            rl[k] = __builtin_amdgcn_raw_buffer_load_b128(rs_res, res_off(mp + 1) + col_off(i), 0, P32_RES_AUX);
+        }
+    };
+    auto table_scale_bias = [&](int i) {
+        const float* t = reinterpret_cast<const float*>(cols_tab) + co + i * TN * 32;
+#pragma unroll
+        for (int q = 0; q < 8; ++q) {
+            sc[q] = t[q];
+            bs[q] = t[TM * TN * 32 + q];
+        }
+    };
+    float vmax0 = 0.f, vmax1 = 0.f, vmax2 = 0.f;
+    if (P32_ABLATE & 512) return;
+    load_res(0);
+#pragma unroll
+    for (int i = 0; i < TM; ++i) {
+        asm volatile("" ::: "memory");
+        __builtin_amdgcn_wave_barrier();
+        write_tile_row(i, reinterpret_cast<float*>(wsm));
+        asm volatile("" ::: "memory");
+        __builtin_amdgcn_wave_barrier();
+        if (COLS) table_scale_bias(i);
+        f16x8 ch[ITEMS], cl[ITEMS];
+#pragma unroll
+        for (int k = 0; k < ITEMS; ++k) {
+            ch[k] = __builtin_bit_cast(f16x8, from_below(rh[k], rl[k]));
+            cl[k] = __builtin_bit_cast(f16x8, from_above(rl[k], rh[k]));
+        }
+        if (i + 1 < TM) load_res(i + 1);
+#pragma unroll
+        for (int k = 0; k < ITEMS; ++k) {
+            const int lr = r_first + k * RPI;
+            const int m = row_of(i, k);
+            const float4 x0 = *reinterpret_cast<const float4*>(wsm + lr * (LDW * 4) + (line * 4 + cj) * 32);
+            const float4 x1 = *reinterpret_cast<const float4*>(wsm + lr * (LDW * 4) + (line * 4 + cj) * 32 + 16);
+            typedef float f32x2 __attribute__((ext_vector_type(2)));
+            f32x2 v2[4] = {{x0.x, x0.y}, {x0.z, x0.w}, {x1.x, x1.y}, {x1.z, x1.w}};
+            const int gd = (m >= b1) + (m >= b2);
+            const float post = gd == 0 ? post0 : (gd == 1 ? post1 : post2);
+            const float res_inv = gd == 0 ? resi0 : (gd == 1 ? resi1 : resi2);
+            const float s_out = gd == 0 ? sout0 : (gd == 1 ? sout1 : sout2);
+            float v[8];
+#pragma unroll
+            for (int q = 0; q < 4; ++q) {
+                const f32x2 scq = {sc[2 * q], sc[2 * q + 1]}, bsq = {bs[2 * q], bs[2 * q + 1]};
+                const f32x2 t = (v2[q] * post) * scq + bsq;
+                v[2 * q] = t.x;
+                v[2 * q + 1] = t.y;
+            }
+#pragma unroll
+            for (int q = 0; q < 8; ++q) {
+                v[q] = fmaf((float)cl[k][q], res_inv, fmaf((float)ch[k][q], res_inv, v[q]));
+                v[q] = fmaxf(v[q], act_lo);
+            }
+            if (sigmoid_on && !(P32_ABLATE & 256)) {
+#pragma unroll
+                for (int q = 0; q < 8; ++q) v[q] = 1.0f / (1.0f + expf(-v[q]));
+            }
+            f16x8 h, l;
+            float vm = 0.f;
+#pragma unroll
+            for (int q = 0; q < 8; q += 2) {
+                vm = fmaxf(vm, fmaxf(fabsf(v[q]), fabsf(v[q + 1])));
+                const f32x2 y = f32x2{v[q], v[q + 1]} * s_out;
+                h[q] = (_Float16)y.x;
+                h[q + 1] = (_Float16)y.y;
+                l[q] = (_Float16)fmaf(-(float)h[q], 1.0f, y.x);
+                l[q + 1] = (_Float16)fmaf(-(float)h[q + 1], 1.0f, y.y);
+            }
+            if (single) l = f16x8{0, 0, 0, 0, 0, 0, 0, 0};
+            vm = m < p.M ? vm : 0.f;
+            vmax0 = fmaxf(vmax0, gd == 0 ? vm : 0.f);
+            vmax1 = fmaxf(vmax1, gd == 1 ? vm : 0.f);
+            vmax2 = fmaxf(vmax2, gd == 2 ? vm : 0.f);
+            const u32x4 hu = __builtin_bit_cast(u32x4, h), lu = __builtin_bit_cast(u32x4, l);
+            const u32x4 d0 = from_below(hu, lu);
+            const u32x4 d1 = from_above(lu, hu);
+            const unsigned off = (unsigned)(m - rs) * cbytes + lofs + col_off(i);
+            if (P32_ABLATE & 64) {
+                asm volatile("" :: "v"(d0), "v"(d1), "v"(off));
+            } else {
+                __builtin_amdgcn_raw_buffer_store_b128(d0, rs_out, off, 0, P32_ST_AUX);
+                __builtin_amdgcn_raw_buffer_store_b128(d1, rs_out, off + cbytes, 0, P32_ST_AUX);
+            }
+            hook();
+        }
+    }
+#pragma unroll
+    for (int d = 0; d < 3; ++d) {
+        if (d > 0 && (d == 1 ? b1 : b2) >= m0 + BM_) break;
+        if (g0 + d >= p.groups) break;
+        float vmax = d == 0 ? vmax0 : (d == 1 ? vmax1 : vmax2);
+#pragma unroll
+        for (int o = 32; o > 0; o >>= 1) vmax = fmaxf(vmax, __shfl_xor(vmax, o));
+        float* slot = p.out_meta + 2 * (g0 + d);
+        if (lane == 0 && vmax > *reinterpret_cast<volatile const float*>(slot))
+            atomicMax(reinterpret_cast<unsigned int*>(slot), __float_as_uint(vmax));
+    }
+}
+
+}
diff --git a/deepemia_amd/engine.py b/deepemia_amd/engine.py
--- a/deepemia_amd/engine.py
+++ b/deepemia_amd/engine.py
@@ -251,6 +251,7 @@
         self._tables: Dict[Tuple[int, int], dict] = {}
         self._cell = cell_anchor_table()
         self.roi_order = os.environ.get("DEEPEMIA_ROI_ORDER", "0") == "1"
+        self.res2_chain = os.environ.get("DEEPEMIA_RES2_CHAIN", "1") != "0"
         self.conv_events = None
         self.unmatched_keys: List[str] = []
         self._used = set()
@@ -502,6 +503,43 @@
             ev.append((e0, e1, 2.0 * n * ho * wo * L.cout * L.kh * L.kw * cin, "f16" if L.single else self.precision, nbytes))
         return out
 
+    def chain_qualifies(self, a, L2: ConvLayer, L3: ConvLayer) -> bool:
+        if not (self.res2_chain and self.precision == "f16x2" and isinstance(a, p32.P32)):
+            return False
+        n, h, w, cin = a.shape
+        rows = n * h * w
+        return (cin == 64 and L2.cin == 64 and L2.cout == 64 and L2.kh == 3 and L2.kw == 3 and L2.stride == 1 and L2.pad == 1 and
+                L3.cin == 64 and L3.cout == 256 and L3.kh == 1 and L3.kw == 1 and L3.stride == 1 and L3.pad == 0 and
+                L2.single == 0 and L3.single == 0 and rows % a.groups == 0 and rows // a.groups >= 128 and
+                (rows + 256) * 256 * 4 + 256 < (1 << 32))
+
+    def conv_p32_chain(self, a: p32.P32, L2: ConvLayer, L3: ConvLayer, residual: p32.P32, next_conv1: Optional[ConvLayer] = None):
+        n, h, w, _ = a.shape
+        assert residual.shape == (n, h, w, L3.cout) and residual.groups == a.groups, (a.shape, residual.shape)
+        out = self.new_p32((n, h, w, L3.cout), a.groups)
+        L1, nxt = next_conv1, None
+        if L1 is not None:
+            assert L1.cin == L3.cout and L1.cout == 64 and L1.kh == 1 and L1.stride == 1 and L1.single == 0, L1
+            nxt = self.new_p32((n, h, w, L1.cout), a.groups)
+        ev = self.conv_events
+        if ev is not None:
+            e0, e1 = torch.cuda.Event(enable_timing=True), torch.cuda.Event(enable_timing=True)
+            e0.record(torch.cuda.current_stream(self.device))
+        d = _lib.ConvP32ChainDesc(_lib.ptr(a.buf), _lib.ptr(a.meta), _lib.ptr(L2.w3), _lib.ptr(L2.scale3), _lib.ptr(L2.bias), L2.wbound, L2.bbound,
+                                  _lib.ptr(L3.w3), _lib.ptr(L3.scale3), _lib.ptr(L3.bias), L3.wbound, L3.bbound,
+                                  _lib.ptr(residual.buf), _lib.ptr(residual.meta), _lib.ptr(out.buf), _lib.ptr(out.meta),
+                                  0 if L1 is None else _lib.ptr(L1.w3), 0 if L1 is None else _lib.ptr(L1.scale3), 0 if L1 is None else _lib.ptr(L1.bias),
+                                  0.0 if L1 is None else L1.wbound, 0.0 if L1 is None else L1.bbound,
+                                  0 if nxt is None else _lib.ptr(nxt.buf), 0 if nxt is None else _lib.ptr(nxt.meta),
+                                  n, h, w, L2.cout, L3.cout, 1, a.groups, (n * h * w) // a.groups, 0)
+        _lib.check(self.lib.demia_conv_p32_chain(C.byref(d), self._stream()), "demia_conv_p32_chain")
+        if ev is not None:
+            e1.record(torch.cuda.current_stream(self.device))
+            m = n * h * w
+            nbytes = m * 64 * 4 + 2 * m * 256 * 4 + (L2.cout_pad * 9 * 64 + L3.cout_pad * 64) * 4
+            ev.append((e0, e1, 2.0 * m * (64 * 9 * 64 + 256 * 64), self.precision, nbytes))
+        return out if nxt is None else (out, nxt)
+
     def conv(self, x, L: ConvLayer, act=ACT_NONE, residual=None, res_mode=RES_NONE,
              out_dtype=None, out: Optional[torch.Tensor] = None, out_ld: int = 0, tile_hint: int = 0):
         if self.p32:
@@ -647,6 +685,9 @@
             for blk in stage_blocks:
                 sc = self.conv(x, blk["shortcut"]) if "shortcut" in blk else x
                 o = self.conv(x, blk["conv1"], act=ACT_RELU)
+                if self.p32 and self.chain_qualifies(o, blk["conv2"], blk["conv3"]):
+                    x = self.conv_p32_chain(o, blk["conv2"], blk["conv3"], sc)
+                    continue
                 o = self.conv(o, blk["conv2"], act=ACT_RELU)
                 x = self.conv(o, blk["conv3"], act=ACT_RELU, residual=sc, res_mode=RES_SAME)
             feats[f"res{si + 2}"] = x
diff --git a/include/deepemia_hip.h b/include/deepemia_hip.h
--- a/include/deepemia_hip.h
+++ b/include/deepemia_hip.h
@@ -81,6 +81,34 @@
     int32_t single;
 } demia_conv_p32_desc;
 int demia_conv2d_p32(const demia_conv_p32_desc* d, void* stream);
+
+typedef struct demia_conv_p32_chain_desc {
+    const void* in;
+    const float* in_meta;
+    const void* w2;
+    const float* scale2;
+    const float* bias2;
+    float wbound2, bbound2;
+    const void* w3;
+    const float* scale3;
+    const float* bias3;
+    float wbound3, bbound3;
+    const void* residual;
+    const float* res_meta;
+    void* out;
+    float* out_meta;
+    const void* w_next;
+    const float* scale_next;
+    const float* bias_next;
+    float wbound_next, bbound_next;
+    void* out_next;
+    float* next_meta;
+    int32_t N, H, W;
+    int32_t mid, Cout;
+    int32_t stride;
+    int32_t groups, group_rows, row0;
+} demia_conv_p32_chain_desc;
+int demia_conv_p32_chain(const demia_conv_p32_chain_desc* d, void* stream);
 
 int demia_resize_h_u8(const uint8_t* src, uint8_t* tmp, int N, int H, int W, int newW,
                       const int32_t* xmin, const int32_t* xsize, const int32_t* xk, int ksx, void* stream);
```

New measurement: 737.2, median of 6. No clear change (+0.8%).
